# ErrorTzy/unpaper-gpu

Hardware: AMD Instinct MI355X
Metric: pages/sec + Mpixel/s, 1000-page GRAY8 A4@300dpi batch, 1/2/4/8 GPU (higher is better)
Workload: dtype u8; 1 GPU; 1000 synthetic GRAY8 A4@300dpi pages (2480x3508) per GPU, default pipeline, inputs and outputs resident in HBM; pages_per_gpu=1000, sheets_per_batch=64, streams=16, hw_queues=24, parallelism=one runner thread per device, pages sharded, no collective

## Files before the change

unpaper-gpu_amd/csrc/common.h:

```cpp
#pragma once

#include <hip/hip_runtime.h>
#include <stdint.h>
#include <stdlib.h>

#include <mutex>
#include <set>
#include <utility>

#include "unpaper_hip.h"

#define UPH_HD __host__ __device__ __forceinline__

namespace uph {

inline void allow_dynamic_lds(const void* kernel, size_t bytes) {
  if (bytes <= 64 * 1024) return;
  static std::mutex mu;
  static std::set<std::pair<int, const void*>> done;
  int dev = 0;
  (void)hipGetDevice(&dev);
  std::lock_guard<std::mutex> lk(mu);
  if (done.insert({dev, kernel}).second)
    (void)hipFuncSetAttribute(kernel, hipFuncAttributeMaxDynamicSharedMemorySize, 160 * 1024);
}


enum Fmt : int32_t {
  F_GRAY8 = UPHIP_FMT_GRAY8,
  F_Y400A = UPHIP_FMT_Y400A,
  F_RGB24 = UPHIP_FMT_RGB24,
  F_MONOWHITE = UPHIP_FMT_MONOWHITE,
  F_MONOBLACK = UPHIP_FMT_MONOBLACK,
};

UPH_HD int bytes_per_pixel(int fmt) {
  return fmt == F_GRAY8 ? 1 : fmt == F_Y400A ? 2 : fmt == F_RGB24 ? 3 : 0;
}
UPH_HD bool is_mono(int fmt) { return fmt == F_MONOWHITE || fmt == F_MONOBLACK; }
UPH_HD int64_t row_bytes(int32_t w, int fmt) {
  return is_mono(fmt) ? ((int64_t)w + 7) / 8 : (int64_t)w * bytes_per_pixel(fmt);
}
UPH_HD int64_t round_pitch(int64_t bytes) { return (bytes + 255) & ~(int64_t)255; }

struct Rect {
  int32_t x0, y0, x1, y1;
};

UPH_HD Rect to_rect(UphipRectangle r) {
  return Rect{r.vertex[0].x, r.vertex[0].y, r.vertex[1].x, r.vertex[1].y};
}
UPH_HD UphipRectangle from_rect(Rect r) {
  UphipRectangle o;
  o.vertex[0].x = r.x0;
  o.vertex[0].y = r.y0;
  o.vertex[1].x = r.x1;
  o.vertex[1].y = r.y1;
  return o;
}
UPH_HD int32_t imin(int32_t a, int32_t b) { return a < b ? a : b; }
UPH_HD int32_t imax(int32_t a, int32_t b) { return a > b ? a : b; }
UPH_HD int32_t iabs(int32_t a) { return a < 0 ? -a : a; }
UPH_HD Rect normalize(Rect r) {
  return Rect{imin(r.x0, r.x1), imin(r.y0, r.y1), imax(r.x0, r.x1), imax(r.y0, r.y1)};
}
UPH_HD Rect clip(Rect r, int32_t W, int32_t H) {
  Rect n = normalize(r);
  return Rect{imax(n.x0, 0), imax(n.y0, 0), imin(n.x1, W - 1), imin(n.y1, H - 1)};
}
UPH_HD uint64_t count_pixels(Rect r) {
  return (uint64_t)(uint32_t)((iabs(r.x0 - r.x1) + 1) * (iabs(r.y0 - r.y1) + 1));
}
UPH_HD bool point_in(int32_t x, int32_t y, Rect in) {
  Rect a = normalize(in);
  return x >= a.x0 && x <= a.x1 && y >= a.y0 && y <= a.y1;
}
UPH_HD Rect rect_from_size(int32_t x, int32_t y, int32_t w, int32_t h) {
  return Rect{x, y, x + w - 1, y + h - 1};
}
UPH_HD bool rects_overlap(Rect a_in, Rect b_in) {
  Rect a = normalize(a_in), b = normalize(b_in);
  return point_in(a.x0, a.y0, b) || point_in(a.x1, a.y1, b);
}

struct Px {
  uint8_t r, g, b;
};
UPH_HD uint8_t gray_of(Px p) { return (uint8_t)(((int)p.r + p.g + p.b) / 3); }
UPH_HD uint8_t light_of(Px p) {
  uint8_t m = p.r < p.g ? p.r : p.g;
  return m < p.b ? m : p.b;
}
UPH_HD uint8_t dark_of(Px p) {
  uint8_t m = p.r > p.g ? p.r : p.g;
  return m > p.b ? m : p.b;
}

template <int FMT>
__device__ __forceinline__ Px load_px_row(const uint8_t* row, int32_t x) {
  if (FMT == F_GRAY8) {
    uint8_t v = row[x];
    return Px{v, v, v};
  } else if (FMT == F_Y400A) {
    uint8_t v = row[2 * x];
    return Px{v, v, v};
  } else {
    const uint8_t* q = row + 3 * x;
    return Px{q[0], q[1], q[2]};
  }
}

template <int FMT>
__device__ __forceinline__ void store_px_row(uint8_t* row, int32_t x, Px p) {
  if (FMT == F_GRAY8) {
    row[x] = gray_of(p);
  } else if (FMT == F_Y400A) {
    row[2 * x] = gray_of(p);
    row[2 * x + 1] = 0xFF;
  } else {
    uint8_t* q = row + 3 * x;
    q[0] = p.r;
    q[1] = p.g;
    q[2] = p.b;
  }
}

__device__ __forceinline__ Px load_px_any(const uint8_t* base, int64_t pitch, int fmt,
                                          int32_t W, int32_t H, int32_t x, int32_t y) {
  if (x < 0 || y < 0 || x >= W || y >= H) return Px{255, 255, 255};
  const uint8_t* row = base + (int64_t)y * pitch;
  switch (fmt) {
    case F_GRAY8: return load_px_row<F_GRAY8>(row, x);
    case F_Y400A: return load_px_row<F_Y400A>(row, x);
    case F_RGB24: return load_px_row<F_RGB24>(row, x);
    case F_MONOWHITE: return (row[x >> 3] & (128 >> (x & 7))) ? Px{0, 0, 0} : Px{255, 255, 255};
    default: return (row[x >> 3] & (128 >> (x & 7))) ? Px{255, 255, 255} : Px{0, 0, 0};
  }
}

__device__ __forceinline__ void xcd_block(int* bx, int* by, int* bz) {
  const int gx = gridDim.x, gy = gridDim.y;
  const int nblk = gx * gy * gridDim.z;
  const int lin = blockIdx.x + gx * (blockIdx.y + gy * blockIdx.z);
  const int q = nblk >> 3, rr = nblk & 7, xcd = lin & 7;
  const int t = xcd * q + (xcd < rr ? xcd : rr) + (lin >> 3);
  *bz = t / (gx * gy);
  const int rem = t - *bz * gx * gy;
  *by = rem / gx;
  *bx = rem - *by * gx;
}

inline uint32_t div_magic(uint32_t d) { return d > 1 ? (uint32_t)(0xFFFFFFFFull / d + 1) : 0u; }
__device__ __forceinline__ int div_by_magic(int n, uint32_t m) {
  return m ? (int)__umulhi((uint32_t)n, m) : n;
}
__device__ __forceinline__ void xcd_block_m(uint32_t m_gxy, uint32_t m_gx, int* bx, int* by,
                                            int* bz) {
  const int gx = gridDim.x, gy = gridDim.y;
  const int nblk = gx * gy * gridDim.z;
  const int lin = blockIdx.x + gx * (blockIdx.y + gy * blockIdx.z);
  const int q = nblk >> 3, rr = nblk & 7, xcd = lin & 7;
  const int t = xcd * q + (xcd < rr ? xcd : rr) + (lin >> 3);
  *bz = div_by_magic(t, m_gxy);
  const int rem = t - *bz * gx * gy;
  *by = div_by_magic(rem, m_gx);
  *bx = rem - *by * gx;
}

struct Planes {
  uint8_t* base[2];
  int64_t pitch;
  int64_t stride;
  int32_t W, H;
  int32_t fmt;
  int32_t count;
};

struct SheetCtl {
  int32_t cur;
  int32_t status;
  int32_t point_count;
  int32_t mask_count;
  UphipPoint points[UPHIP_MAX_POINTS];
  UphipRectangle masks[UPHIP_MAX_POINTS];
  UphipRectangle border_masks[UPHIP_MAX_PAGES];
  float rotation[UPHIP_MAX_PAGES];
  int32_t rot_index[UPHIP_MAX_PAGES][4];
  int32_t op_active;
  int32_t op_i[8];
  float op_f[4];
  UphipRectangle op_rect[4];
};

enum : int32_t {
  STATUS_FLOOD_OVERFLOW = 1 << 0,
  STATUS_NOISE_OVERFLOW = 1 << 1,
  STATUS_EDGE_GUARD = 1 << 2,
  STATUS_SORT_OVERFLOW = 1 << 3,
};

__device__ __forceinline__ uint8_t* sheet_plane(const Planes& P, int s, int k) {
  return P.base[k] + (int64_t)s * P.stride;
}

#ifdef UPHIP_DIAG
inline int diag_env(const char* name) {
  const char* v = getenv(name);
  return v ? atoi(v) : 0;
}
inline int diag_skip() {
  static const int v = diag_env("UPHIP_DIAG_SKIP");
  return v;
}
inline int diag_double() {
  static const int v = diag_env("UPHIP_DIAG_DOUBLE");
  return v;
}
inline int diag_noise() {
  static const int v = diag_env("UPHIP_DIAG_NOISE");
  return v;
}
#define UPH_DIAG_BITS(d, m) ((d) & (m))
#define UPH_LAUNCH_DIAG(bit, ...)                              \
  do {                                                         \
    hipLaunchKernelGGL(__VA_ARGS__);                           \
    if (::uph::diag_double() & (bit)) hipLaunchKernelGGL(__VA_ARGS__); \
  } while (0)
#else
constexpr int diag_skip() { return 0; }
constexpr int diag_double() { return 0; }
constexpr int diag_noise() { return 0; }
#define UPH_DIAG_BITS(d, m) 0
#define UPH_LAUNCH_DIAG(bit, ...) hipLaunchKernelGGL(__VA_ARGS__)
#endif

}
```

unpaper-gpu_amd/csrc/kernels.h:

```cpp
#pragma once

#include "common.h"

namespace uph {

struct PlaneRef {
  Planes P;
  const SheetCtl* ctl;
  int32_t which;
};

__device__ __forceinline__ uint8_t* plane_ptr(const PlaneRef& R, int s) {
  int k = R.which;
  if (R.ctl) k = R.which ? 1 - R.ctl[s].cur : R.ctl[s].cur;
  return R.P.base[k] + (int64_t)s * R.P.stride;
}

inline PlaneRef cur_ref(const Planes& P, const SheetCtl* ctl) { return PlaneRef{P, ctl, 0}; }
inline PlaneRef other_ref(const Planes& P, const SheetCtl* ctl) { return PlaneRef{P, ctl, 1}; }
inline PlaneRef fixed_ref(const Planes& P, int k) { return PlaneRef{P, nullptr, k}; }

struct FillArgs {
  Rect r;
  uint8_t color[3];
  int32_t active;
};

struct CopyArgs {
  Rect a;
  int32_t tx, ty;
  int32_t active;
};

struct MaskArgs {
  int32_t n;
  uint8_t color[3];
  Rect m[UPHIP_MAX_MASKS];
};

struct MoveArgs {
  Rect area;
  int32_t tx, ty;
  uint8_t bg[3];
  int32_t active;
};

struct RotateArgs {
  Rect mask;
  float sinval, cosval;
  int32_t active;
};

void launch_fill_thr(const PlaneRef& dst, const FillArgs* args, int count, int rows_hint,
                     uint8_t thr, hipStream_t st);
void launch_copy_thr(const PlaneRef& src, const PlaneRef& dst, const CopyArgs* args, int count,
                     int rows_hint, uint8_t thr, hipStream_t st);
void launch_apply_masks_thr(const PlaneRef& dst, const MaskArgs* args, int count, uint8_t thr,
                            hipStream_t st);
void launch_mirror_oop(const PlaneRef& src, const PlaneRef& dst, bool h, bool v, uint8_t thr,
                       int count, hipStream_t st);
void launch_rotate90_thr(const PlaneRef& src, const PlaneRef& dst, int direction, uint8_t thr,
                         int count, hipStream_t st);
void launch_stretch_thr(const PlaneRef& src, const PlaneRef& dst, int interp, uint8_t thr,
                        int count, hipStream_t st);
void launch_shift(const PlaneRef& src, const PlaneRef& dst, int dx, int dy, const uint8_t bg[3],
                  uint8_t thr, int count, hipStream_t st);
void launch_flip_if_active(SheetCtl* ctl, const int32_t* active, int64_t stride_bytes,
                           int count, hipStream_t st);

void launch_move_rect(const PlaneRef& src, const PlaneRef& dst, const MoveArgs* args,
                      int count, hipStream_t st);
struct MoveExtra {
  const MaskArgs* masks;
  uint32_t* rows;
  int64_t rows_stride;
  int32_t rx0, rx1;
  uint8_t thr;
  bool dry;
  int32_t ya0, ya1, yb0, yb1;
  const int32_t* only;
};
bool launch_move_chain(const PlaneRef& src, const PlaneRef& dst, const MoveArgs* center,
                       const MaskArgs* masks, const MoveArgs* align, int count, hipStream_t st);
bool launch_move_rect_fused(const PlaneRef& src, const PlaneRef& dst, const MoveArgs* args,
                            const MoveExtra& x, int count, hipStream_t st);

bool launch_rotate_mask(const PlaneRef& src, const PlaneRef& dst, const RotateArgs* args,
                        int interp, int count, hipStream_t st, float max_abs_angle,
                        uint32_t* colsum = nullptr, int64_t cs_stride = 0);
struct LinWindow {
  int32_t cols, rows, stride;
};
bool launch_rotate_linear(const PlaneRef& src, const PlaneRef& dst, const RotateArgs* args,
                          int nmask, int64_t mstride, const int32_t* indep, int count,
                          hipStream_t st, float max_abs_angle);

}
```

unpaper-gpu_amd/csrc/kernels_rotate.hip:

```cpp
#include <type_traits>

#include "blit_common.h"
#include "interp.h"
#include "kernels.h"

namespace uph {

constexpr int kRotTW = 64, kRotTH = 16;
constexpr int kRotCap = 4096;

template <int FMT>
struct LdsSrc {
  const uint8_t* lds;
  int32_t x0, y0, w, h;
  int32_t W, H;
  Src<FMT> g;
  __device__ __forceinline__ Px at(int32_t x, int32_t y) const {
    const int32_t u = x - x0, v = y - y0;
    if (u < 0 || v < 0 || u >= w || v >= h) return g.at(x, y);
    if (FMT == F_RGB24) {
      const uint8_t* q = lds + 3 * (v * w + u);
      return Px{q[0], q[1], q[2]};
    }
    const uint8_t q = lds[v * w + u];
    return Px{q, q, q};
  }
};

template <int FMT>
__global__ void __launch_bounds__(kThreads) k_rotate_mask(PlaneRef src, PlaneRef dst,
                                                          const RotateArgs* args, int interp) {
  constexpr int CH = FMT == F_RGB24 ? 3 : 1;
  __shared__ uint8_t stage[kRotCap * CH];
  const int s = blockIdx.z;
  const RotateArgs a = args[s];
  if (!a.active) return;
  const Planes& P = src.P;
  const uint8_t* sbase = plane_ptr(src, s);
  uint8_t* dbase = plane_ptr(dst, s);
  const Rect nm = normalize(a.mask);
  const int32_t sw = nm.x1 - nm.x0 + 1, sh = nm.y1 - nm.y0 + 1;
  const float scx = nm.x0 + sw / 2.0f, scy = nm.y0 + sh / 2.0f;
  const float tcx = 0 + sw / 2.0f, tcy = 0 + sh / 2.0f;
  const Src<FMT> S{sbase, P.pitch, P.W, P.H};
  const int32_t tx0 = blockIdx.x * kRotTW, ty0 = blockIdx.y * kRotTH;
  const int32_t u0 = imax(tx0, 0) - a.mask.x0, u1 = imin(tx0 + kRotTW, P.W) - 1 - a.mask.x0;
  const int32_t v0 = imax(ty0, 0) - a.mask.y0, v1 = imin(ty0 + kRotTH, P.H) - 1 - a.mask.y0;
  const int32_t cu0 = imax(u0, 0), cu1 = imin(u1, sw - 1);
  const int32_t cv0 = imax(v0, 0), cv1 = imin(v1, sh - 1);
  const bool any_in = cu0 <= cu1 && cv0 <= cv1;
  int32_t bx0 = 0, by0 = 0, bw = 0, bh = 0;
  bool staged = false;
  if (any_in) {
    float mnx = 3.0e38f, mxx = -3.0e38f, mny = 3.0e38f, mxy = -3.0e38f;
#pragma unroll
    for (int c = 0; c < 4; c++) {
      const int32_t u = c & 1 ? cu1 : cu0, v = c & 2 ? cv1 : cv0;
      const float X = scx + (u - tcx) * a.cosval + (v - tcy) * a.sinval;
      const float Y = scy + (v - tcy) * a.cosval - (u - tcx) * a.sinval;
      mnx = fminf(mnx, X);
      mxx = fmaxf(mxx, X);
      mny = fminf(mny, Y);
      mxy = fmaxf(mxy, Y);
    }
    bx0 = (int32_t)floorf(mnx) - 3;
    by0 = (int32_t)floorf(mny) - 3;
    bw = (int32_t)floorf(mxx) + 4 - bx0 + 1;
    bh = (int32_t)floorf(mxy) + 4 - by0 + 1;
    staged = bw > 0 && bh > 0 && (int64_t)bw * bh <= kRotCap;
  }
  if (staged) {
    const int n = bw * bh;
    for (int base = 0; base < n; base += 8 * kThreads) {
      uint8_t v[8][CH];
#pragma unroll
      for (int k = 0; k < 8; k++) {
        const int i = base + k * kThreads + threadIdx.x;
        const int32_t x = bx0 + i % bw, y = by0 + i / bw;
#pragma unroll
        for (int c = 0; c < CH; c++) v[k][c] = 255;
        if (i < n && x >= 0 && y >= 0 && x < P.W && y < P.H) {
          const Px p = load_px_row<FMT>(sbase + (int64_t)y * P.pitch, x);
          v[k][0] = p.r;
          if (CH == 3) {
            v[k][1] = p.g;
            v[k][2] = p.b;
          }
        }
      }
#pragma unroll
      for (int k = 0; k < 8; k++) {
        const int i = base + k * kThreads + threadIdx.x;
        if (i < n) {
#pragma unroll
          for (int c = 0; c < CH; c++) stage[i * CH + c] = v[k][c];
        }
      }
    }
  }
  __syncthreads();
  const LdsSrc<FMT> L{stage, bx0, by0, bw, bh, P.W, P.H, S};
  const int lane = threadIdx.x & 63, w = threadIdx.x >> 6;
  const int32_t x = tx0 + lane;
  if (x >= P.W) return;
  const int32_t u = x - a.mask.x0;
#pragma unroll
  for (int k = 0; k < kRotTH / 4; k++) {
    const int32_t y = ty0 + w + 4 * k;
    if (y >= P.H) break;
    uint8_t* drow = dbase + (int64_t)y * P.pitch;
    const int32_t v = y - a.mask.y0;
    if (u >= 0 && u < sw && v >= 0 && v < sh) {
      const float srcX = scx + (u - tcx) * a.cosval + (v - tcy) * a.sinval;
      const float srcY = scy + (v - tcy) * a.cosval - (u - tcx) * a.sinval;
      if (FMT != F_RGB24 && staged && interp == UPHIP_INTERP_CUBIC) {
        const int ix = (int)srcX, iy = (int)srcY;
        const uint8_t* t = stage + (iy - 1 - by0) * bw + (ix - 1 - bx0);
        const float fx = srcX - ix;
        uint8_t col[4];
#pragma unroll
        for (int r = 0; r < 4; r++, t += bw) col[r] = cubic_scale(fx, t[0], t[1], t[2], t[3]);
        const uint8_t o = cubic_scale(srcY - iy, col[0], col[1], col[2], col[3]);
        store_px_row<FMT>(drow, x, Px{o, o, o});
        continue;
      }
      const Px o = staged ? interpolate<FMT>(L, srcX, srcY, interp)
                          : interpolate<FMT>(S, srcX, srcY, interp);
      store_px_row<FMT>(drow, x, o);
    } else {
      copy_px_raw<FMT>(drow, x, sbase + (int64_t)y * P.pitch, x);
    }
  }
}

__device__ __forceinline__ uint8_t cubic_int(float f, float h, int a, int b, int c, int d) {
  const float s2 = (float)(3 * (b - c) + d - a);
  const float s1 = (float)(2 * a - 5 * b + 4 * c - d);
  const float u = s1 + f * s2;
  const float v = (float)(c - a) + f * u;
  const int r = (int)((float)b + h * v);
  return (uint8_t)(r < 0 ? 0 : (r > 255 ? 255 : r));
}

constexpr int kRotGH = 32;
constexpr int kRotGCap = 6144;

template <int FMT>
__global__ void __launch_bounds__(kThreads) k_rotate_cubic_gray(PlaneRef src, PlaneRef dst,
                                                                const RotateArgs* args) {
  __shared__ uint32_t stage32[kRotGCap / 4];
  uint8_t* stage = reinterpret_cast<uint8_t*>(stage32);
  int txi, tyi, s;
  xcd_block(&txi, &tyi, &s);
  const RotateArgs a = args[s];
  if (!a.active) return;
  const Planes& P = src.P;
  const uint8_t* sbase = plane_ptr(src, s);
  uint8_t* dbase = plane_ptr(dst, s);
  const Rect nm = normalize(a.mask);
  const int32_t sw = nm.x1 - nm.x0 + 1, sh = nm.y1 - nm.y0 + 1;
  const float scx = nm.x0 + sw / 2.0f, scy = nm.y0 + sh / 2.0f;
  const float tcx = 0 + sw / 2.0f, tcy = 0 + sh / 2.0f;
  const int32_t tx0 = txi * kRotTW, ty0 = tyi * kRotGH;
  const int32_t u0 = imax(tx0, 0) - a.mask.x0, u1 = imin(tx0 + kRotTW, P.W) - 1 - a.mask.x0;
  const int32_t v0 = imax(ty0, 0) - a.mask.y0, v1 = imin(ty0 + kRotGH, P.H) - 1 - a.mask.y0;
  const int32_t cu0 = imax(u0, 0), cu1 = imin(u1, sw - 1);
  const int32_t cv0 = imax(v0, 0), cv1 = imin(v1, sh - 1);
  int32_t bx0 = 0, by0 = 0, bw = 0, bh = 0;
  bool staged = false;
  if (cu0 <= cu1 && cv0 <= cv1) {
    float mnx = 3.0e38f, mxx = -3.0e38f, mny = 3.0e38f, mxy = -3.0e38f;
#pragma unroll
    for (int c = 0; c < 4; c++) {
      const int32_t u = c & 1 ? cu1 : cu0, v = c & 2 ? cv1 : cv0;
      const float X = scx + (u - tcx) * a.cosval + (v - tcy) * a.sinval;
      const float Y = scy + (v - tcy) * a.cosval - (u - tcx) * a.sinval;
      mnx = fminf(mnx, X);
      mxx = fmaxf(mxx, X);
      mny = fminf(mny, Y);
      mxy = fmaxf(mxy, Y);
    }
    bx0 = (int32_t)floorf(mnx) - 3;
    by0 = (int32_t)floorf(mny) - 3;
    bw = (int32_t)floorf(mxx) + 4 - bx0 + 1;
    bh = (int32_t)floorf(mxy) + 4 - by0 + 1;
    staged = bw > 0 && bh > 0;
  }
  const int32_t xa = bx0 >= 0 ? (bx0 & ~3) : -((-bx0 + 3) & ~3);
  const int lead = FMT == F_GRAY8 ? bx0 - xa : 0;
  const int nd = (lead + bw + 3) >> 2;
  const int sstride = FMT == F_GRAY8 ? 4 * nd : bw;
  staged = staged && (int64_t)sstride * bh <= kRotGCap;
  if (staged && FMT == F_GRAY8) {
    const int n = nd * bh;
    for (int b0 = 0; b0 < n; b0 += 8 * kThreads) {
      uint32_t v[8];
#pragma unroll
      for (int k = 0; k < 8; k++) {
        const int i = b0 + k * kThreads + threadIdx.x;
        const int r = i / nd;
        const int32_t xd = xa + 4 * (i - r * nd), y = by0 + r;
        const bool row_ok = (y >= 0) & (y < P.H);
        const uint8_t* row = sbase + (int64_t)imin(imax(y, 0), P.H - 1) * P.pitch;
        v[k] = *reinterpret_cast<const uint32_t*>(row + imin(imax(xd, 0), (int32_t)P.pitch - 4));
        if (!row_ok) v[k] = 0xFFFFFFFFu;
      }
#pragma unroll
      for (int k = 0; k < 8; k++) {
        const int i = b0 + k * kThreads + threadIdx.x;
        if (i >= n) continue;
        const int r = i / nd;
        const int32_t xd = xa + 4 * (i - r * nd), y = by0 + r;
        uint32_t w4 = v[k];
        if ((y >= 0) & (y < P.H) & ((xd < 0) | (xd + 3 >= P.W))) {
          const uint8_t* row = sbase + (int64_t)y * P.pitch;
          w4 = 0;
#pragma unroll
          for (int j = 0; j < 4; j++) {
            const int32_t x = xd + j;
            const uint32_t b = (x >= 0 && x < P.W) ? row[x] : 255u;
            w4 |= b << (8 * j);
          }
        }
        stage32[i] = w4;
      }
    }
  } else if (staged) {
    const int n = bw * bh;
    for (int b0 = 0; b0 < n; b0 += 8 * kThreads) {
      uint8_t v[8];
#pragma unroll
      for (int k = 0; k < 8; k++) {
        const int i = b0 + k * kThreads + threadIdx.x;
        const int r = i / bw;
        const int32_t x = bx0 + (i - r * bw), y = by0 + r;
        const bool ok = (x >= 0) & (y >= 0) & (x < P.W) & (y < P.H);
        const uint8_t q = load_px_row<FMT>(sbase + (int64_t)imin(imax(y, 0), P.H - 1) * P.pitch,
                                           imin(imax(x, 0), P.W - 1)).r;
        v[k] = ok ? q : (uint8_t)255;
      }
#pragma unroll
      for (int k = 0; k < 8; k++) {
        const int i = b0 + k * kThreads + threadIdx.x;
        if (i < n) stage[i] = v[k];
      }
    }
  }
  __syncthreads();
  const Src<FMT> S{sbase, P.pitch, P.W, P.H};
  const int lane = threadIdx.x & 63, w = threadIdx.x >> 6;
  const int32_t x = tx0 + lane;
  if (x >= P.W) return;
  const int32_t u = x - a.mask.x0;
#pragma unroll
  for (int k = 0; k < kRotGH / 4; k++) {
    const int32_t y = ty0 + w + 4 * k;
    if (y >= P.H) break;
    uint8_t* drow = dbase + (int64_t)y * P.pitch;
    const int32_t v = y - a.mask.y0;
    if (u >= 0 && u < sw && v >= 0 && v < sh) {
      const float srcX = scx + (u - tcx) * a.cosval + (v - tcy) * a.sinval;
      const float srcY = scy + (v - tcy) * a.cosval - (u - tcx) * a.sinval;
      uint8_t o;
      if (staged) {
        const int ix = (int)srcX, iy = (int)srcY;
        const float fx = srcX - ix, fy = srcY - iy;
        const float hx = 0.5f * fx, hy = 0.5f * fy;
        const uint8_t* t = stage + (iy - 1 - by0) * sstride + lead + (ix - 1 - bx0);
        int col[4];
#pragma unroll
        for (int r = 0; r < 4; r++, t += sstride)
          col[r] = cubic_int(fx, hx, t[0], t[1], t[2], t[3]);
        o = cubic_int(fy, hy, col[0], col[1], col[2], col[3]);
      } else {
        o = interp_bicubic(S, srcX, srcY).r;
      }
      store_px_row<FMT>(drow, x, Px{o, o, o});
    } else {
      copy_px_raw<FMT>(drow, x, sbase + (int64_t)y * P.pitch, x);
    }
  }
}

typedef float f2 __attribute__((ext_vector_type(2)));
constexpr int kRQW = 256;
constexpr int kRQH = 32;
constexpr int kRQStride = 72;
constexpr int kRQRows = 84;
constexpr int kRQWords = kRQStride * kRQRows + 2;

__device__ __forceinline__ f2 fma2(f2 a, f2 b, f2 c) { return __builtin_elementwise_fma(a, b, c); }
__device__ __forceinline__ f2 splat2(float v) { return f2{v, v}; }

__device__ __forceinline__ void cubic_terms(f2 a, f2 b, f2 c, f2 d, f2& ca, f2& s1, f2& s2) {
  const f2 e = d - a, g = b - c;
  ca = c - a;
  s2 = fma2(splat2(3.0f), g, e);
  s1 = fma2(splat2(-5.0f), g, -(e + ca));
}

__device__ __forceinline__ f2 cubic2(f2 f, f2 h, f2 a, f2 b, f2 c, f2 d) {
  f2 ca, s1, s2;
  cubic_terms(a, b, c, d, ca, s1, s2);
  const f2 u = s1 + f * s2;
  const f2 v = ca + f * u;
  const f2 r = b + h * v;
  return f2{__builtin_amdgcn_fmed3f(__builtin_truncf(r.x), 0.0f, 255.0f),
            __builtin_amdgcn_fmed3f(__builtin_truncf(r.y), 0.0f, 255.0f)};
}

template <int K>
__device__ __forceinline__ float ubyte_f(uint32_t w) {
  float r;
  if constexpr (K == 0) asm("v_cvt_f32_ubyte0 %0, %1" : "=v"(r) : "v"(w));
  else if constexpr (K == 1) asm("v_cvt_f32_ubyte1 %0, %1" : "=v"(r) : "v"(w));
  else if constexpr (K == 2) asm("v_cvt_f32_ubyte2 %0, %1" : "=v"(r) : "v"(w));
  else asm("v_cvt_f32_ubyte3 %0, %1" : "=v"(r) : "v"(w));
  return r;
}
template <int K>
__device__ __forceinline__ f2 tap2(uint32_t p, uint32_t q) {
  return f2{ubyte_f<K>(p), ubyte_f<K>(q)};
}

__global__ void __launch_bounds__(kThreads) k_rotate_cubic_g8(PlaneRef src, PlaneRef dst,
                                                              const RotateArgs* args) {
  __shared__ uint32_t win[kRQWords];
  int txi, tyi, s;
  xcd_block(&txi, &tyi, &s);
  const RotateArgs a = args[s];
  if (!a.active) return;
  const Planes& P = src.P;
  const uint8_t* sbase = plane_ptr(src, s);
  uint8_t* dbase = plane_ptr(dst, s);
  const Rect nm = normalize(a.mask);
  const int32_t sw = nm.x1 - nm.x0 + 1, sh = nm.y1 - nm.y0 + 1;
  const float scx = nm.x0 + sw / 2.0f, scy = nm.y0 + sh / 2.0f;
  const float tcx = 0 + sw / 2.0f, tcy = 0 + sh / 2.0f;
  const int32_t tx0 = txi * kRQW, ty0 = tyi * kRQH;
  const int32_t u0 = imax(tx0, 0) - a.mask.x0, u1 = imin(tx0 + kRQW, P.W) - 1 - a.mask.x0;
  const int32_t v0 = imax(ty0, 0) - a.mask.y0, v1 = imin(ty0 + kRQH, P.H) - 1 - a.mask.y0;
  const int32_t cu0 = imax(u0, 0), cu1 = imin(u1, sw - 1);
  const int32_t cv0 = imax(v0, 0), cv1 = imin(v1, sh - 1);
  int32_t bx0 = 0, by0 = 0, bw = 0, bh = 0;
  if (cu0 <= cu1 && cv0 <= cv1) {
    float mnx = 3.0e38f, mxx = -3.0e38f, mny = 3.0e38f, mxy = -3.0e38f;
#pragma unroll
    for (int c = 0; c < 4; c++) {
      const int32_t u = c & 1 ? cu1 : cu0, v = c & 2 ? cv1 : cv0;
      const float X = scx + (u - tcx) * a.cosval + (v - tcy) * a.sinval;
      const float Y = scy + (v - tcy) * a.cosval - (u - tcx) * a.sinval;
      mnx = fminf(mnx, X);
      mxx = fmaxf(mxx, X);
      mny = fminf(mny, Y);
      mxy = fmaxf(mxy, Y);
    }
    bx0 = (int32_t)floorf(mnx) - 3;
    by0 = (int32_t)floorf(mny) - 3;
    bw = (int32_t)floorf(mxx) + 4 - bx0 + 1;
    bh = (int32_t)floorf(mxy) + 4 - by0 + 1;
  }
  const int32_t xa = bx0 >= 0 ? (bx0 & ~3) : -((-bx0 + 3) & ~3);
  const int lead = bx0 - xa;
  const int nd = (lead + bw + 3) >> 2;
  const bool staged = bw > 0 && bh > 0 && nd < kRQStride && bh <= kRQRows;
  if (staged) {
    const uint32_t m = nd > 1 ? (uint32_t)((0xFFFFFFFFull / (uint32_t)nd) + 1) : 0u;
    const int n = nd * bh;
    for (int b0 = 0; b0 < n; b0 += 8 * kThreads) {
      uint32_t v[8];
#pragma unroll
      for (int k = 0; k < 8; k++) {
        const int i = b0 + k * kThreads + threadIdx.x;
        const int r = nd > 1 ? (int)__umulhi((uint32_t)i, m) : i;
        const int32_t xd = xa + 4 * (i - r * nd), y = by0 + r;
        const uint8_t* row = sbase + (int64_t)imin(imax(y, 0), P.H - 1) * P.pitch;
        v[k] = *reinterpret_cast<const uint32_t*>(row + imin(imax(xd, 0), (int32_t)P.pitch - 4));
        if ((y < 0) | (y >= P.H)) v[k] = 0xFFFFFFFFu;
      }
#pragma unroll
      for (int k = 0; k < 8; k++) {
        const int i = b0 + k * kThreads + threadIdx.x;
        if (i >= n) continue;
        const int r = nd > 1 ? (int)__umulhi((uint32_t)i, m) : i;
        const int j = i - r * nd;
        const int32_t xd = xa + 4 * j, y = by0 + r;
        uint32_t w4 = v[k];
        if ((y >= 0) & (y < P.H) & ((xd < 0) | (xd + 3 >= P.W))) {
          const uint8_t* row = sbase + (int64_t)y * P.pitch;
          w4 = 0;
#pragma unroll
          for (int q = 0; q < 4; q++) {
            const int32_t x = xd + q;
            const uint32_t b = (x >= 0 && x < P.W) ? row[x] : 255u;
            w4 |= b << (8 * q);
          }
        }
        win[r * kRQStride + j] = w4;
      }
    }
  }
  __syncthreads();
  const int lane = threadIdx.x & 63, w = threadIdx.x >> 6;
  const int32_t xl = tx0 + 4 * lane;
  if (xl >= P.W) return;
  float ax[4], bs[4];
  bool colin[4];
#pragma unroll
  for (int j = 0; j < 4; j++) {
    const int32_t u = xl + j - a.mask.x0;
    const float cu = u - tcx;
    ax[j] = scx + cu * a.cosval;
    bs[j] = cu * a.sinval;
    colin[j] = (u >= 0) & (u < sw) & (xl + j < P.W);
  }
  const f2 AX0{ax[0], ax[1]}, AX1{ax[2], ax[3]}, BS0{bs[0], bs[1]}, BS1{bs[2], bs[3]};
  const int base_off = (-1 - by0) * (4 * kRQStride) + lead - 1 - bx0;
  const Src<F_GRAY8> S{sbase, P.pitch, P.W, P.H};
#pragma unroll 2
  for (int k = 0; k < kRQH / 4; k++) {
    const int32_t y = ty0 + w + 4 * k;
    if (y >= P.H) break;
    const int32_t v = y - a.mask.y0;
    const bool rowin = (v >= 0) & (v < sh);
    const float cv = v - tcy;
    const f2 VS = splat2(cv * a.sinval), VC = splat2(scy + cv * a.cosval);
    const f2 SX[2] = {AX0 + VS, AX1 + VS};
    const f2 SY[2] = {VC - BS0, VC - BS1};
    const uint8_t* srow = sbase + (int64_t)y * P.pitch;
    uint32_t out = 0;
    if (staged) {
#pragma unroll
      for (int pr = 0; pr < 2; pr++) {
        const int ix0 = (int)SX[pr].x, ix1 = (int)SX[pr].y;
        const int iy0 = (int)SY[pr].x, iy1 = (int)SY[pr].y;
        const f2 fx = SX[pr] - f2{(float)ix0, (float)ix1};
        const f2 fy = SY[pr] - f2{(float)iy0, (float)iy1};
        const f2 hx = 0.5f * fx, hy = 0.5f * fy;
        const bool in0 = rowin & colin[2 * pr], in1 = rowin & colin[2 * pr + 1];
        const int o0 = in0 ? base_off + iy0 * (4 * kRQStride) + ix0 : 0;
        const int o1 = in1 ? base_off + iy1 * (4 * kRQStride) + ix1 : 0;
        const uint32_t* w0 = win + (o0 >> 2);
        const uint32_t* w1 = win + (o1 >> 2);
        f2 col[4];
#pragma unroll
        for (int r = 0; r < 4; r++) {
          const uint32_t p = __builtin_amdgcn_alignbyte(w0[r * kRQStride + 1], w0[r * kRQStride], o0);
          const uint32_t q = __builtin_amdgcn_alignbyte(w1[r * kRQStride + 1], w1[r * kRQStride], o1);
          col[r] = cubic2(fx, hx, tap2<0>(p, q), tap2<1>(p, q), tap2<2>(p, q), tap2<3>(p, q));
        }
        const f2 o = cubic2(fy, hy, col[0], col[1], col[2], col[3]);
        out = __builtin_amdgcn_cvt_pk_u8_f32(o.x, 2 * pr, out);
        out = __builtin_amdgcn_cvt_pk_u8_f32(o.y, 2 * pr + 1, out);
      }
    } else {
#pragma unroll
      for (int j = 0; j < 4; j++) {
        const f2 sx = SX[j >> 1], sy = SY[j >> 1];
        const float fx = (j & 1) ? sx.y : sx.x, fy = (j & 1) ? sy.y : sy.x;
        if (rowin & colin[j]) out |= (uint32_t)interp_bicubic(S, fx, fy).r << (8 * j);
      }
    }
    uint32_t inmask = 0;
#pragma unroll
    for (int j = 0; j < 4; j++) inmask |= (rowin & colin[j]) ? 0xFFu << (8 * j) : 0u;
    uint8_t* drow = dbase + (int64_t)y * P.pitch;
    if (xl + 3 < P.W) {
      if (inmask != 0xFFFFFFFFu)
        out = (out & inmask) | (*reinterpret_cast<const uint32_t*>(srow + xl) & ~inmask);
      *reinterpret_cast<uint32_t*>(drow + xl) = out;
    } else {
      for (int j = 0; xl + j < P.W; j++)
        drow[xl + j] = (inmask >> (8 * j)) & 1 ? (uint8_t)(out >> (8 * j)) : srow[xl + j];
    }
  }
}

constexpr int kRFW = 128;
constexpr int kRFH = 48;
constexpr int kRFS = 144;
constexpr int kRFT = 512;
constexpr int kRFWaves = kRFT / 64;

#define UPH_TAP_PAIR(o, b, k) \
  "ds_read2_b32 %" #o ", %" #b " offset0:" #k " offset1:" UPH_STR(UPH_ROWOFF_##k) "\n\t"
#define UPH_STR2(x) #x
#define UPH_STR(x) UPH_STR2(x)
#define UPH_ROWOFF_0 144
#define UPH_ROWOFF_1 145
#define UPH_ROWOFF_2 146
#define UPH_ROWOFF_3 147
static_assert(kRFS == 144, "tap pair offsets are spelled out for a 144-float row stride");
__device__ __forceinline__ void lds_taps16(const uint32_t (&a)[4], f2 (&t)[4][4]) {
  asm volatile(UPH_TAP_PAIR(0, 16, 0) UPH_TAP_PAIR(1, 16, 1) UPH_TAP_PAIR(2, 16, 2)
               UPH_TAP_PAIR(3, 16, 3) UPH_TAP_PAIR(4, 17, 0) UPH_TAP_PAIR(5, 17, 1)
               UPH_TAP_PAIR(6, 17, 2) UPH_TAP_PAIR(7, 17, 3) UPH_TAP_PAIR(8, 18, 0)
               UPH_TAP_PAIR(9, 18, 1) UPH_TAP_PAIR(10, 18, 2) UPH_TAP_PAIR(11, 18, 3)
               UPH_TAP_PAIR(12, 19, 0) UPH_TAP_PAIR(13, 19, 1) UPH_TAP_PAIR(14, 19, 2)
               UPH_TAP_PAIR(15, 19, 3)
               : "=&v"(t[0][0]), "=&v"(t[0][1]), "=&v"(t[0][2]), "=&v"(t[0][3]),
                 "=&v"(t[1][0]), "=&v"(t[1][1]), "=&v"(t[1][2]), "=&v"(t[1][3]),
                 "=&v"(t[2][0]), "=&v"(t[2][1]), "=&v"(t[2][2]), "=&v"(t[2][3]),
                 "=&v"(t[3][0]), "=&v"(t[3][1]), "=&v"(t[3][2]), "=&v"(t[3][3])
               : "v"(a[0]), "v"(a[1]), "v"(a[2]), "v"(a[3])
               : "memory");
}
template <int N>
__device__ __forceinline__ void lds_wait_pair(f2 (&t)[4]) {
  asm volatile("s_waitcnt lgkmcnt(%4)"
               : "+v"(t[0]), "+v"(t[1]), "+v"(t[2]), "+v"(t[3])
               : "n"(N)
               : "memory");
}
template <int N>
__device__ __forceinline__ void lds_wait_pair_after(f2 (&t)[4], f2& prev) {
  asm volatile("s_waitcnt lgkmcnt(%5)"
               : "+v"(t[0]), "+v"(t[1]), "+v"(t[2]), "+v"(t[3]), "+v"(prev)
               : "n"(N)
               : "memory");
}

__device__ __forceinline__ f2 cubic2_row_u(f2 f, f2 h, const f2 (&t)[4]) {
  f2 ca, s1, s2;
  cubic_terms(t[0], t[1], t[2], t[3], ca, s1, s2);
  f2 u = f * s2;
  u = s1 + u;
  u = f * u;
  u = ca + u;
  u = h * u;
  return t[1] + u;
}
__device__ __forceinline__ float clamp_t255(float u) {
  return __builtin_amdgcn_fmed3f(__builtin_truncf(u), 0.0f, 255.0f);
}

template <int CTRL>
__device__ __forceinline__ float dpp_f(float v) {
  return __int_as_float(__builtin_amdgcn_mov_dpp(__float_as_int(v), CTRL, 0xF, 0xF, false));
}

__device__ __forceinline__ uint32_t row_off(int32_t y, int64_t pitch) {
  return (uint32_t)y * (uint32_t)pitch;
}

#ifndef UPH_ROT_MINB
#define UPH_ROT_MINB 8
#endif
#ifdef UPHIP_DIAG
__device__ unsigned long long g_rot_phase[1024 * 8];
#define UPH_ROT_T(k)                                                         \
  if (UPH_DIAG_BITS(diag, 65536) && threadIdx.x == 0) {                     \
    const unsigned long long tn = wall_clock64();                            \
    atomicAdd(&g_rot_phase[8 * (blockIdx.x & 1023) + (k)], tn - tprev);      \
    tprev = tn;                                                              \
  }
#else
#define UPH_ROT_T(k)
#endif
template <bool LOOP>
__global__ void __launch_bounds__(kRFT, UPH_ROT_MINB) k_rotate_cubic_g8f(PlaneRef src, PlaneRef dst,
                                                               const RotateArgs* args,
                                                               int max_rows, int cls_rows,
                                                               int diag,
                                                               uint32_t m_gxy, uint32_t m_gx,
                                                               int loop_count, int tgx, int tgy,
                                                               uint32_t* colsum, int64_t cs_stride) {
  extern __shared__ __attribute__((aligned(16))) float winf[];
  __shared__ int32_t win_s[4];
  __shared__ uint32_t csum_s[kRFW];
  auto tile = [&](int txi, int tyi, int s) {
#ifdef UPHIP_DIAG
  unsigned long long tprev = wall_clock64();
#endif
  const uint8_t* sbase = plane_ptr(src, s);
  uint8_t* dbase = plane_ptr(dst, s);
  const RotateArgs a = args[s];
  if (!a.active) return;
  if (cls_rows != 0) {
    const int need = kRFH + (int)ceilf((kRFW - 1) * fabsf(a.sinval)) + 5;
    if (cls_rows > 0 ? need > cls_rows : need <= -cls_rows) return;
  }
  const Planes& P = src.P;
  const Rect nm = normalize(a.mask);
  const int32_t sw = nm.x1 - nm.x0 + 1, sh = nm.y1 - nm.y0 + 1;
  const float scx = nm.x0 + sw / 2.0f, scy = nm.y0 + sh / 2.0f;
  const float tcx = 0 + sw / 2.0f, tcy = 0 + sh / 2.0f;
  const int32_t tx0 = txi * kRFW, ty0 = tyi * kRFH;
  const int32_t u0 = imax(tx0, 0) - a.mask.x0, u1 = imin(tx0 + kRFW, P.W) - 1 - a.mask.x0;
  const int32_t v0 = imax(ty0, 0) - a.mask.y0, v1 = imin(ty0 + kRFH, P.H) - 1 - a.mask.y0;
  const int32_t cu0 = imax(u0, 0), cu1 = imin(u1, sw - 1);
  const int32_t cv0 = imax(v0, 0), cv1 = imin(v1, sh - 1);
  auto csum_flush = [&]() {
    __syncthreads();
    if (threadIdx.x < kRFW && tx0 + (int)threadIdx.x < P.W)
      atomicAdd(colsum + s * cs_stride + tx0 + threadIdx.x, csum_s[threadIdx.x]);
  };
  const bool outside_tile = !(cu0 <= cu1 && cv0 <= cv1);
  if (colsum) {
    if (threadIdx.x < kRFW) csum_s[threadIdx.x] = 0;
    if (outside_tile) __syncthreads();
  }
  if (!(cu0 <= cu1 && cv0 <= cv1)) {
    const int cb = 8 * (threadIdx.x & 15);
    const int32_t x = tx0 + cb;
    uint32_t cs8[8] = {0, 0, 0, 0, 0, 0, 0, 0};
    for (int r = threadIdx.x >> 4; r < kRFH; r += kRFT / 16) {
      const int32_t y = ty0 + r;
      if (y >= P.H || x >= P.W) continue;
      const uint8_t* sp = sbase + row_off(y, P.pitch) + x;
      uint8_t* dp = dbase + row_off(y, P.pitch) + x;
      if (x + 8 <= P.W) {
        const uint64_t q = *reinterpret_cast<const uint64_t*>(sp);
        *reinterpret_cast<uint64_t*>(dp) = q;
#pragma unroll
        for (int j = 0; j < 8; j++) cs8[j] += (uint32_t)(q >> (8 * j)) & 0xFFu;
      } else {
        for (int j = 0; x + j < P.W; j++) {
          dp[j] = sp[j];
          cs8[j & 7] += sp[j];
        }
      }
    }
    if (colsum) {
#pragma unroll
      for (int j = 0; j < 8; j++) atomicAdd(&csum_s[cb + j], cs8[j]);
      csum_flush();
    }
    return;
  }
  UPH_ROT_T(0)
  const int lane = threadIdx.x & 63;
  const int wu = __builtin_amdgcn_readfirstlane(threadIdx.x >> 6);
  if (wu == 0) {
    const int c = lane & 3;
    const int32_t u = c & 1 ? cu1 : cu0, v = c & 2 ? cv1 : cv0;
    const float X = scx + (u - tcx) * a.cosval + (v - tcy) * a.sinval;
    const float Y = scy + (v - tcy) * a.cosval - (u - tcx) * a.sinval;
    float mnx = fminf(X, dpp_f<0xB1>(X)), mxx = fmaxf(X, dpp_f<0xB1>(X));
    float mny = fminf(Y, dpp_f<0xB1>(Y)), mxy = fmaxf(Y, dpp_f<0xB1>(Y));
    mnx = fminf(mnx, dpp_f<0x4E>(mnx));
    mxx = fmaxf(mxx, dpp_f<0x4E>(mxx));
    mny = fminf(mny, dpp_f<0x4E>(mny));
    mxy = fmaxf(mxy, dpp_f<0x4E>(mxy));
    if (lane < 4) {
      const float q = lane == 0 ? mnx : lane == 1 ? mny : lane == 2 ? mxx : mxy;
      win_s[lane] = (int32_t)floorf(q);
    }
  }
  __syncthreads();
  UPH_ROT_T(1)
  const int32_t bx0 = __builtin_amdgcn_readfirstlane(win_s[0]) - 1;
  const int32_t by0 = __builtin_amdgcn_readfirstlane(win_s[1]) - 1;
  const int32_t bw = __builtin_amdgcn_readfirstlane(win_s[2]) + 3 - bx0 + 1;
  const int32_t bh = __builtin_amdgcn_readfirstlane(win_s[3]) + 3 - by0 + 1;
  const int32_t xa = bx0 >= 0 ? (bx0 & ~3) : -((-bx0 + 3) & ~3);
  const int nd = (bx0 - xa + bw + 3) >> 2;
  const bool staged = bw > 0 && bh > 0 && 4 * nd <= kRFS && bh <= max_rows;
  uint64_t* nw = reinterpret_cast<uint64_t*>(winf + kRFS * max_rows);
  uint8_t* obuf = reinterpret_cast<uint8_t*>(nw + max_rows) + wu * (kRFH / kRFWaves * kRFW);
  if (staged && !UPH_DIAG_BITS(diag, 1024)) {
    const int rq = (lane * 57) >> 10;
    const int jq = lane - 18 * rq;
    const int nq = (nd + 1) >> 1;
    const bool qv = rq < 3 && jq < nq;
    const int32_t xd = xa + 8 * jq;
    auto stage = [&](int rb, uint32_t w0, uint32_t w1) {
      const int r = rb + rq;
      const bool valid = qv && r < bh;
      const unsigned long long m = __ballot(valid && (w0 & w1) != 0xFFFFFFFFu);
      if (lane < 3 && rb + lane < bh) nw[rb + lane] = (m >> (18 * lane)) & 0x3FFFFull;
      if (valid) {
        float4* d = reinterpret_cast<float4*>(winf + r * kRFS + 8 * jq);
        d[0] = make_float4(ubyte_f<0>(w0), ubyte_f<1>(w0), ubyte_f<2>(w0), ubyte_f<3>(w0));
        d[1] = make_float4(ubyte_f<0>(w1), ubyte_f<1>(w1), ubyte_f<2>(w1), ubyte_f<3>(w1));
      }
    };
    const bool interior = xa >= 0 && xa + 8 * nq <= P.W && by0 >= 0 && by0 + bh <= P.H;
    if (interior) {
      const uint32_t off0 = row_off(by0 + rq, P.pitch) + (uint32_t)(qv ? xd : xa);
      for (int rg = 3 * wu; rg < bh; rg += 3 * 3 * kRFWaves) {
        uint2 v[3];
#pragma unroll
        for (int g = 0; g < 3; g++) {
          const int rb = rg + 3 * kRFWaves * g;
          const uint32_t o = rb + rq < bh ? off0 + (uint32_t)rb * (uint32_t)P.pitch : off0;
          v[g] = *reinterpret_cast<const uint2*>(sbase + o);
        }
#pragma unroll
        for (int g = 0; g < 3; g++) {
          const int rb = rg + 3 * kRFWaves * g;
          if (rb >= bh) break;
          stage(rb, v[g].x, v[g].y);
        }
      }
    } else {
      const int32_t xc0 = imin(imax(xd, 0), (int32_t)P.pitch - 4);
      const int32_t xc1 = imin(imax(xd + 4, 0), (int32_t)P.pitch - 4);
      const int fs0 = imin(imax(24 + 8 * (xd - xc0), 0), 56);
      const int fs1 = imin(imax(24 + 8 * (xd + 4 - xc1), 0), 56);
      uint32_t out0 = qv ? 0u : 0xFFFFFFFFu, out1 = out0;
#pragma unroll
      for (int k = 0; k < 4; k++) {
        if (xd + k < 0 || xd + k >= P.W) out0 |= 0xFFu << (8 * k);
        if (xd + 4 + k < 0 || xd + 4 + k >= P.W) out1 |= 0xFFu << (8 * k);
      }
      for (int rg = 3 * wu; rg < bh; rg += 3 * 3 * kRFWaves) {
        uint2 v[3];
#pragma unroll
        for (int g = 0; g < 3; g++) {
          const int r = rg + 3 * kRFWaves * g + rq;
          const int32_t y = imin(imax(by0 + r, 0), P.H - 1);
          const uint8_t* row = sbase + row_off(y, P.pitch);
          v[g].x = *reinterpret_cast<const uint32_t*>(row + xc0);
          v[g].y = *reinterpret_cast<const uint32_t*>(row + xc1);
        }
#pragma unroll
        for (int g = 0; g < 3; g++) {
          const int rb = rg + 3 * kRFWaves * g;
          if (rb >= bh) break;
          const int32_t y = by0 + rb + rq;
          uint32_t w0 = (uint32_t)(((uint64_t)v[g].x << 24) >> fs0) | out0;
          uint32_t w1 = (uint32_t)(((uint64_t)v[g].y << 24) >> fs1) | out1;
          if ((y < 0) | (y >= P.H)) w0 = w1 = 0xFFFFFFFFu;
          stage(rb, w0, w1);
        }
      }
    }
  }
  __syncthreads();
  UPH_ROT_T(2)
  const int32_t xA = tx0 + lane, xB = xA + 64;
  const bool hasA = xA < P.W, hasB = xB < P.W;
  const int32_t uA = xA - a.mask.x0, uB = xB - a.mask.x0;
  const float cuA = uA - tcx, cuB = uB - tcx;
  const float axA = scx + cuA * a.cosval, bsA = cuA * a.sinval;
  const float axB = scx + cuB * a.cosval, bsB = cuB * a.sinval;
  const bool colA = hasA & (uA >= 0) & (uA < sw), colB = hasB & (uB >= 0) & (uB < sw);
  typedef __attribute__((address_space(3))) float lds_f32;
  const uint32_t lds0 = (uint32_t)(uintptr_t)(lds_f32*)winf;
  const Src<F_GRAY8> S{sbase, P.pitch, P.W, P.H};
  const float cuL = (tx0 - a.mask.x0) - tcx, cuR = (tx0 + kRFW - 1 - a.mask.x0) - tcx;
  const float bsL = cuL * a.sinval, bsR = cuR * a.sinval;
  constexpr int kRows = kRFH / kRFWaves;
  const int32_t yw = ty0 + wu * kRows;
  const int cb = 8 * (lane & 15);
  const int32_t xo = tx0 + cb;
  const bool partial = !(cu0 == u0 && cu1 == u1 && cv0 == v0 && cv1 == v1);
  if (partial) {
    constexpr int kQ = (kRows + 3) / 4;
    uint64_t q[kQ];
#pragma unroll
    for (int h = 0; h < kQ; h++) {
      q[h] = 0;
      const int rr = 4 * h + (lane >> 4);
      const int32_t y = imin(yw + rr, P.H - 1);
      const int32_t x = imin(xo, (int32_t)P.pitch - 8);
      if (rr < kRows) q[h] = *reinterpret_cast<const uint64_t*>(sbase + row_off(y, P.pitch) + x);
    }
#pragma unroll
    for (int h = 0; h < kQ; h++) {
      const int rr = 4 * h + (lane >> 4);
      if (rr < kRows) *reinterpret_cast<uint64_t*>(obuf + rr * kRFW + cb) = q[h];
    }
  }
  uint32_t white_rows = 0;
  if (staged) {
#pragma unroll
    for (int g = 0; g < kRows; g += 8) {
      const int k = g + (lane >> 3), j = lane & 7;
      bool hit = false;
      if (k < kRows) {
        const float cv = (yw + k - a.mask.y0) - tcy;
        const float VC = scy + cv * a.cosval;
        const int32_t yl = (int)(VC - bsL), yr = (int)(VC - bsR);
        const int32_t r0 = imax(imin(yl, yr) - 1 - by0, 0);
        const int32_t r1 = imin(imax(yl, yr) + 2 - by0, bh - 1);
        for (int r = r0 + j; r <= r1; r += 8) hit |= nw[r] != 0;
      }
      const uint64_t m = __ballot(hit);
#pragma unroll
      for (int q = 0; q < 8 && g + q < kRows; q++)
        if (((m >> (8 * q)) & 0xFFull) == 0) white_rows |= 1u << (g + q);
    }
    if (UPH_DIAG_BITS(diag, 2048)) white_rows = 0;
    if (UPH_DIAG_BITS(diag, 512)) white_rows = ~0u;
  }
  const bool posc = bx0 >= 0 && by0 >= 0;
  const uint32_t wbase = lds0 - 4u * (uint32_t)((1 + by0) * kRFS + 1 + xa);
  UPH_ROT_T(3)
  uint32_t fsA = 0, fsB = 0;
  auto row_loop = [&](auto full_tag) {
  constexpr bool FULL = decltype(full_tag)::value;
#pragma unroll
  for (int k = 0; k < kRows; k++) {
    const int32_t y = yw + k;
    const int32_t v = y - a.mask.y0;
    const bool rowin = FULL || ((v >= 0) & (v < sh) & (y < P.H));
    const float cv = v - tcy;
    const float VS = cv * a.sinval, VC = scy + cv * a.cosval;
    const bool inA = FULL || (rowin & colA), inB = FULL || (rowin & colB);
    uint32_t oA = 255, oB = 255;
    const bool white = (FULL || staged) && ((white_rows >> k) & 1u);
    if (!white && (FULL || staged)) {
      const float sxA = axA + VS, syA = VC - bsA, sxB = axB + VS, syB = VC - bsB;
      const int ixA = (int)sxA, iyA = (int)syA, ixB = (int)sxB, iyB = (int)syB;
      float fxA, fyA, fxB, fyB;
      if (FULL || posc) {
        fxA = __builtin_amdgcn_fractf(sxA);
        fyA = __builtin_amdgcn_fractf(syA);
        fxB = __builtin_amdgcn_fractf(sxB);
        fyB = __builtin_amdgcn_fractf(syB);
      } else {
        fxA = sxA - ixA, fyA = syA - iyA, fxB = sxB - ixB, fyB = syB - iyB;
      }
      const uint32_t pA = inA ? wbase + 4u * (uint32_t)(__mul24(iyA, kRFS) + ixA) : lds0;
      const uint32_t pB = inB ? wbase + 4u * (uint32_t)(__mul24(iyB, kRFS) + ixB) : lds0;
      const uint32_t ta[4] = {pA, pA + 8 * kRFS, pB, pB + 8 * kRFS};
      f2 t[4][4];
      lds_taps16(ta, t);
      const f2 FA = splat2(fxA), HA = splat2(0.5f * fxA);
      const f2 FB = splat2(fxB), HB = splat2(0.5f * fxB);
      f2 c[4];
      lds_wait_pair<12>(t[0]);
      c[0] = cubic2_row_u(FA, HA, t[0]);
      lds_wait_pair_after<8>(t[1], c[0]);
      c[1] = cubic2_row_u(FA, HA, t[1]);
      lds_wait_pair_after<4>(t[2], c[1]);
      c[2] = cubic2_row_u(FB, HB, t[2]);
      lds_wait_pair_after<0>(t[3], c[2]);
      c[3] = cubic2_row_u(FB, HB, t[3]);
      const f2 o = cubic2(f2{fyA, fyB}, f2{0.5f * fyA, 0.5f * fyB},
                          f2{clamp_t255(c[0].x), clamp_t255(c[2].x)},
                          f2{clamp_t255(c[0].y), clamp_t255(c[2].y)},
                          f2{clamp_t255(c[1].x), clamp_t255(c[3].x)},
                          f2{clamp_t255(c[1].y), clamp_t255(c[3].y)});
      oA = (uint32_t)o.x;
      oB = (uint32_t)o.y;
    }
#ifdef UPHIP_DIAG
    if (UPH_DIAG_BITS(diag, 131072)) {
      int32_t z = k;
      asm volatile(
          "s_add_u32 %0, %0, 1\n\ts_add_u32 %0, %0, 1\n\ts_add_u32 %0, %0, 1\n\ts_add_u32 %0, %0, 1\n\t"
          "s_add_u32 %0, %0, 1\n\ts_add_u32 %0, %0, 1\n\ts_add_u32 %0, %0, 1\n\ts_add_u32 %0, %0, 1\n\t"
          "s_add_u32 %0, %0, 1\n\ts_add_u32 %0, %0, 1\n\ts_add_u32 %0, %0, 1\n\ts_add_u32 %0, %0, 1\n\t"
          "s_add_u32 %0, %0, 1\n\ts_add_u32 %0, %0, 1\n\ts_add_u32 %0, %0, 1\n\ts_add_u32 %0, %0, 1\n\t"
          "s_add_u32 %0, %0, 1\n\ts_add_u32 %0, %0, 1\n\ts_add_u32 %0, %0, 1\n\ts_add_u32 %0, %0, 1\n\t"
          "s_add_u32 %0, %0, 1\n\ts_add_u32 %0, %0, 1\n\ts_add_u32 %0, %0, 1\n\ts_add_u32 %0, %0, 1\n\t"
          "s_add_u32 %0, %0, 1\n\ts_add_u32 %0, %0, 1\n\ts_add_u32 %0, %0, 1\n\ts_add_u32 %0, %0, 1\n\t"
          "s_add_u32 %0, %0, 1\n\ts_add_u32 %0, %0, 1\n\ts_add_u32 %0, %0, 1\n\ts_add_u32 %0, %0, 1"
          : "+s"(z));
      if (z == -1) oA = 0;
    }
#endif
    if (!FULL && !staged) break;
    if (FULL) {
      obuf[k * kRFW + lane] = (uint8_t)oA;
      obuf[k * kRFW + 64 + lane] = (uint8_t)oB;
      fsA += oA;
      fsB += oB;
    } else {
      if (inA) obuf[k * kRFW + lane] = (uint8_t)oA;
      if (inB) obuf[k * kRFW + 64 + lane] = (uint8_t)oB;
    }
  }
  };
  const bool full =
      !partial && staged && posc && tx0 + kRFW <= P.W && ty0 + kRFH <= P.H;
  if (full)
    row_loop(std::true_type{});
  else
    row_loop(std::false_type{});
  if (!staged) {
#pragma unroll 1
    for (int k = 0; k < kRows; k++) {
      const int32_t y = yw + k;
      const int32_t v = y - a.mask.y0;
      const bool rowin = (v >= 0) & (v < sh) & (y < P.H);
      const float cv = v - tcy;
      const float VS = cv * a.sinval, VC = scy + cv * a.cosval;
      if (rowin & colA) obuf[k * kRFW + lane] = interp_bicubic(S, axA + VS, VC - bsA).r;
      if (rowin & colB) obuf[k * kRFW + 64 + lane] = interp_bicubic(S, axB + VS, VC - bsB).r;
    }
  }
  UPH_ROT_T(4)
  __builtin_amdgcn_wave_barrier();
  if (full && !UPH_DIAG_BITS(diag, 8192)) {
#pragma unroll
    for (int k0 = 0; k0 < kRows; k0 += 4) {
      const int rr = k0 + (lane >> 4);
      if (rr < kRows) {
        const uint64_t q = *reinterpret_cast<const uint64_t*>(obuf + rr * kRFW + cb);
        *reinterpret_cast<uint64_t*>(dbase + row_off(yw + rr, P.pitch) + xo) = q;
      }
    }
  } else
  for (int k0 = 0; k0 < kRows && !UPH_DIAG_BITS(diag, 8192); k0 += 4) {
    const int rr = k0 + (lane >> 4);
    const int32_t y = yw + rr, x = xo;
    if (rr < kRows && y < P.H && x < P.W) {
      const uint64_t q = *reinterpret_cast<const uint64_t*>(obuf + rr * kRFW + cb);
      uint8_t* d = dbase + row_off(y, P.pitch) + x;
      if (x + 8 <= P.W) {
        *reinterpret_cast<uint64_t*>(d) = q;
      } else {
        for (int j = 0; x + j < P.W; j++) d[j] = (uint8_t)(q >> (8 * j));
      }
    }
  }
  UPH_ROT_T(5)
  if (colsum) {
    uint32_t sA = fsA, sB = fsB;
    if (!full) {
#pragma unroll
      for (int k = 0; k < kRows; k++) {
        if (yw + k >= P.H) break;
        sA += obuf[k * kRFW + lane];
        sB += obuf[k * kRFW + 64 + lane];
      }
    }
    atomicAdd(&csum_s[lane], sA);
    atomicAdd(&csum_s[64 + lane], sB);
    csum_flush();
  }
  UPH_ROT_T(6)
#ifdef UPHIP_DIAG
  if (UPH_DIAG_BITS(diag, 65536) && threadIdx.x == 0)
    atomicAdd(&g_rot_phase[8 * (blockIdx.x & 1023) + 7], 1ull);
#endif
  };
  if constexpr (!LOOP) {
    int txi, tyi, s;
    xcd_block_m(m_gxy, m_gx, &txi, &tyi, &s);
    tile(txi, tyi, s);
  } else {
  for (int s0 = 0; s0 < loop_count; s0 += 64) {
    const int l = threadIdx.x & 63;
    bool want = false;
    if (s0 + l < loop_count) {
      const RotateArgs q = args[s0 + l];
      want = q.active && kRFH + (int)ceilf((kRFW - 1) * fabsf(q.sinval)) + 5 > -cls_rows;
    }
    uint64_t m = __ballot(want);
    m = ((uint64_t)__builtin_amdgcn_readfirstlane((uint32_t)(m >> 32)) << 32) |
        __builtin_amdgcn_readfirstlane((uint32_t)m);
    while (m) {
      const int s = s0 + __ffsll((long long)m) - 1;
      m &= m - 1;
      for (int t = blockIdx.x; t < tgx * tgy; t += gridDim.x) {
        tile(t % tgx, t / tgx, s);
        __syncthreads();
      }
    }
  }
  }
}

static int rotate_window_rows(float max_abs_angle) {
  const float a = fminf(fabsf(max_abs_angle), 1.5707964f);
  return kRFH + (int)ceilf((kRFW - 1) * sinf(a)) + 5;
}

bool launch_rotate_mask(const PlaneRef& src, const PlaneRef& dst, const RotateArgs* args,
                        int interp, int count, hipStream_t st, float max_abs_angle,
                        uint32_t* colsum, int64_t cs_stride) {
  const dim3 grid((src.P.W + kRotTW - 1) / kRotTW, (src.P.H + kRotTH - 1) / kRotTH, count);
  const dim3 ggrid((src.P.W + kRotTW - 1) / kRotTW, (src.P.H + kRotGH - 1) / kRotGH, count);
  if (interp == UPHIP_INTERP_CUBIC && src.P.fmt == F_GRAY8) {
    if (diag_double() & 4096) colsum = nullptr;
    const int rows = rotate_window_rows(max_abs_angle);
    auto lds_of = [](int r) {
      return (sizeof(float) * kRFS + sizeof(uint64_t)) * (size_t)r + kRFH * kRFW;
    };
    const int rows4 = (int)((40 * 1024 - 16 - 4 * kRFW - kRFH * kRFW) /
                            (sizeof(float) * kRFS + sizeof(uint64_t)));
    if (lds_of(rows) <= 56 * 1024 &&
        src.P.pitch * (int64_t)src.P.H < (1ll << 31) && !(diag_double() & 256)) {
      const dim3 fgrid((src.P.W + kRFW - 1) / kRFW, (src.P.H + kRFH - 1) / kRFH, count);
      const uint32_t mgxy = div_magic(fgrid.x * fgrid.y), mgx = div_magic(fgrid.x);
      const int dd = diag_double() & (512 | 1024 | 2048 | 8192 | 65536 | 131072);
#ifdef UPHIP_DIAG
      struct PhasePrint {
        hipStream_t st;
        ~PhasePrint() {
          if (!(diag_double() & 65536)) return;
          static unsigned long long hh[1024 * 8], z[1024 * 8];
          unsigned long long h[8] = {0, 0, 0, 0, 0, 0, 0, 0};
          hipStreamSynchronize(st);
          hipMemcpyFromSymbol(hh, HIP_SYMBOL(g_rot_phase), sizeof(hh));
          hipMemcpyToSymbol(HIP_SYMBOL(g_rot_phase), z, sizeof(z));
          for (int i = 0; i < 1024 * 8; i++) h[i & 7] += hh[i];
          if (!h[7]) return;
          fprintf(stderr, "rotate phases (10 ns ticks/tile, %llu tiles): args %.0f corners %.0f staging %.0f "
                  "flags %.0f compute %.0f stores %.0f colsum %.0f\n", h[7], (double)h[0] / h[7],
                  (double)h[1] / h[7], (double)h[2] / h[7], (double)h[3] / h[7],
                  (double)h[4] / h[7], (double)h[5] / h[7], (double)h[6] / h[7]);
        }
      } phase_print{st};
#endif
      if (rows > rows4) {
        UPH_LAUNCH_DIAG(2, k_rotate_cubic_g8f<false>, fgrid, dim3(kRFT), lds_of(rows4), st, src, dst, args,
                        rows4, rows4, dd, mgxy, mgx, 0, 0, 0, colsum, cs_stride);
        UPH_LAUNCH_DIAG(2, k_rotate_cubic_g8f<true>, dim3(3 * 256), dim3(kRFT), lds_of(rows), st, src, dst,
                        args, rows, -rows4, dd, 0u, 0u, count, (int)fgrid.x, (int)fgrid.y, colsum,
                        cs_stride);
      } else {
        UPH_LAUNCH_DIAG(2, k_rotate_cubic_g8f<false>, fgrid, dim3(kRFT), lds_of(rows), st, src, dst, args,
                        rows, 0, dd, mgxy, mgx, 0, 0, 0, colsum, cs_stride);
      }
      return colsum != nullptr;
    }
    const dim3 qgrid((src.P.W + kRQW - 1) / kRQW, (src.P.H + kRQH - 1) / kRQH, count);
    UPH_LAUNCH_DIAG(2, k_rotate_cubic_g8, qgrid, dim3(kThreads), 0, st, src, dst, args);
    return false;
  }
  if (interp == UPHIP_INTERP_CUBIC && src.P.fmt == F_Y400A) {
    hipLaunchKernelGGL(k_rotate_cubic_gray<F_Y400A>, ggrid, dim3(kThreads), 0, st, src, dst, args);
    return false;
  }
  if (src.P.fmt == F_GRAY8)
    hipLaunchKernelGGL(k_rotate_mask<F_GRAY8>, grid, dim3(kThreads), 0, st, src, dst, args,
                       interp);
  else if (src.P.fmt == F_Y400A)
    hipLaunchKernelGGL(k_rotate_mask<F_Y400A>, grid, dim3(kThreads), 0, st, src, dst, args,
                       interp);
  else
    hipLaunchKernelGGL(k_rotate_mask<F_RGB24>, grid, dim3(kThreads), 0, st, src, dst, args,
                       interp);
  return false;
}

}
```

unpaper-gpu_amd/csrc/ops.hip:

```cpp
#include <cmath>
#include <cstdio>
#include <vector>

#include "filters.h"
#include "mono_proxy.h"
#include "runtime.h"
#include "scan.h"

namespace uph {

static bool ok_image(const UphipImage& im, const char* op) {
  if (!im.frame) return fail("%s: image has no frame", op);
  if (!runtime_ready()) return fail("%s: no HIP device", op);
  hipSetDevice(im.frame->device);
  return true;
}

static PlaneRef ref_of(const UphipFrame* f) { return fixed_ref(frame_planes(f), 0); }

static void fill_frame(UphipFrame* f, Rect clipped, Px c, uint8_t thr, hipStream_t st) {
  if (clipped.x1 < clipped.x0 || clipped.y1 < clipped.y0) return;
  FillArgs a{clipped, {c.r, c.g, c.b}, 1};
  FillArgs* d = stage_args(&a, 1, st);
  if (!d) return;
  launch_fill_thr(ref_of(f), d, 1, clipped.y1 - clipped.y0 + 1, thr, st);
  arg_fence(st);
}

static void copy_frames(const UphipFrame* src, UphipFrame* dst, Rect clipped, int32_t tx,
                        int32_t ty, uint8_t thr, hipStream_t st) {
  if (clipped.x1 < clipped.x0 || clipped.y1 < clipped.y0) return;
  CopyArgs a{clipped, tx, ty, 1};
  CopyArgs* d = stage_args(&a, 1, st);
  if (!d) return;
  launch_copy_thr(ref_of(src), ref_of(dst), d, 1, clipped.y1 - clipped.y0 + 1, thr, st);
  arg_fence(st);
}

static void adopt_storage(UphipFrame* f, UphipFrame* n) {
  hipStreamSynchronize(current_stream());
  hipFree(f->data);
  *f = *n;
  delete n;
}

}

using namespace uph;

extern "C" {

UphipImage uphip_create_image(UphipRectangleSize size, UphipPixelFormat format, bool fill,
                              UphipPixel background, uint8_t abs_black_threshold) {
  UphipImage im{nullptr, background, abs_black_threshold};
  im.frame = frame_alloc(size.width, size.height, format);
  if (im.frame && fill)
    fill_frame(im.frame, Rect{0, 0, size.width - 1, size.height - 1},
               Px{background.r, background.g, background.b}, abs_black_threshold,
               current_stream());
  return im;
}

void uphip_free_image(UphipImage* image) {
  if (!image) return;
  frame_free(image->frame);
  image->frame = nullptr;
}

void uphip_replace_image(UphipImage* image, UphipImage* new_image) {
  uphip_free_image(image);
  *image = *new_image;
  new_image->frame = nullptr;
}

UphipImage uphip_create_compatible_image(UphipImage source, UphipRectangleSize size, bool fill) {
  return uphip_create_image(size, (UphipPixelFormat)source.frame->format, fill, source.background,
                            source.abs_black_threshold);
}

UphipRectangleSize uphip_size_of_image(UphipImage image) {
  UphipRectangleSize s{0, 0};
  if (image.frame) s = UphipRectangleSize{image.frame->width, image.frame->height};
  return s;
}

UphipPixelFormat uphip_image_format(UphipImage image) {
  return image.frame ? (UphipPixelFormat)image.frame->format : UPHIP_FMT_NONE;
}

int uphip_image_upload(UphipImage image, const void* host, int64_t linesize) {
  if (!ok_image(image, "upload")) return -1;
  UphipFrame* f = image.frame;
  const int64_t rb = row_bytes(f->width, f->format);
  if (linesize < rb) return fail("upload: linesize %lld < row bytes %lld", (long long)linesize,
                                 (long long)rb), -1;
  hipStream_t st = current_stream();
  if (!UPH_HIP(hipMemcpy2DAsync(f->data, f->pitch, host, linesize, rb, f->height,
                                hipMemcpyHostToDevice, st)))
    return -1;
  return UPH_HIP(hipStreamSynchronize(st)) ? 0 : -1;
}

int uphip_image_download(UphipImage image, void* host, int64_t linesize) {
  if (!ok_image(image, "download")) return -1;
  UphipFrame* f = image.frame;
  const int64_t rb = row_bytes(f->width, f->format);
  if (linesize < rb) return fail("download: linesize too small"), -1;
  hipStream_t st = current_stream();
  if (!UPH_HIP(hipMemcpy2DAsync(host, linesize, f->data, f->pitch, rb, f->height,
                                hipMemcpyDeviceToHost, st)))
    return -1;
  return UPH_HIP(hipStreamSynchronize(st)) ? 0 : -1;
}

void* uphip_image_device_ptr(UphipImage image) { return image.frame ? image.frame->data : nullptr; }
int64_t uphip_image_device_pitch(UphipImage image) { return image.frame ? image.frame->pitch : 0; }

void uphip_wipe_rectangle(UphipImage image, UphipRectangle input_area, UphipPixel color) {
  if (!ok_image(image, "wipe_rectangle")) return;
  UphipFrame* f = image.frame;
  fill_frame(f, clip(to_rect(input_area), f->width, f->height), Px{color.r, color.g, color.b},
             image.abs_black_threshold, current_stream());
}

void uphip_copy_rectangle(UphipImage source, UphipImage target, UphipRectangle source_area,
                          UphipPoint target_coords) {
  if (!ok_image(source, "copy_rectangle") || !ok_image(target, "copy_rectangle")) return;
  if (source.frame->device != target.frame->device)
    return (void)fail("copy_rectangle: frames on different devices");
  Rect a = clip(to_rect(source_area), source.frame->width, source.frame->height);
  copy_frames(source.frame, target.frame, a, target_coords.x, target_coords.y,
              target.abs_black_threshold, current_stream());
}

void uphip_center_image(UphipImage source, UphipImage target, UphipPoint to,
                        UphipRectangleSize ts) {
  if (!ok_image(source, "center_image") || !ok_image(target, "center_image")) return;
  UphipPoint so{0, 0};
  UphipRectangleSize ss{source.frame->width, source.frame->height};
  if (ss.width < ts.width || ss.height < ts.height)
    uphip_wipe_rectangle(target, from_rect(rect_from_size(to.x, to.y, ts.width, ts.height)),
                         target.background);
  if (ss.width <= ts.width) {
    to.x += (ts.width - ss.width) / 2;
  } else {
    so.x += (ss.width - ts.width) / 2;
    ss.width = ts.width;
  }
  if (ss.height <= ts.height) {
    to.y += (ts.height - ss.height) / 2;
  } else {
    so.y += (ss.height - ts.height) / 2;
    ss.height = ts.height;
  }
  uphip_copy_rectangle(source, target, from_rect(rect_from_size(so.x, so.y, ss.width, ss.height)),
                       to);
}

static int compare_sizes(UphipRectangleSize a, UphipRectangleSize b) {
  if (a.height == b.height && a.width == b.width) return 0;
  return imin(a.height, a.width) < imin(b.height, b.width) ? -1 : 1;
}

void uphip_stretch_and_replace(UphipImage* pImage, UphipRectangleSize size,
                               UphipInterpolation interp) {
  if (!pImage || !ok_image(*pImage, "stretch_and_replace")) return;
  UphipFrame* f = pImage->frame;
  if (compare_sizes(UphipRectangleSize{f->width, f->height}, size) == 0) return;
  UphipFrame* n = frame_alloc(size.width, size.height, f->format);
  if (!n) return;
  launch_stretch_thr(ref_of(f), ref_of(n), interp, pImage->abs_black_threshold, 1,
                     current_stream());
  adopt_storage(f, n);
}

void uphip_resize_and_replace(UphipImage* pImage, UphipRectangleSize size,
                              UphipInterpolation interp) {
  if (!pImage || !ok_image(*pImage, "resize_and_replace")) return;
  UphipRectangleSize is{pImage->frame->width, pImage->frame->height};
  if (compare_sizes(is, size) == 0) return;
  const float hr = (float)size.width / (float)is.width;
  const float vr = (float)size.height / (float)is.height;
  UphipRectangleSize ss;
  if (hr < vr) {
    ss.width = size.width;
    ss.height = (int32_t)(is.height * hr);
  } else if (vr < hr) {
    ss.width = (int32_t)(is.width * vr);
    ss.height = size.height;
  } else {
    ss = size;
  }
  uphip_stretch_and_replace(pImage, ss, interp);
  if (size.width == ss.width && size.height == ss.height) return;
  UphipImage resized = uphip_create_compatible_image(*pImage, size, true);
  if (!resized.frame) return;
  uphip_center_image(*pImage, resized, UphipPoint{0, 0}, size);
  uphip_replace_image(pImage, &resized);
}

void uphip_flip_rotate_90(UphipImage* pImage, UphipRotationDirection direction) {
  if (!pImage || !ok_image(*pImage, "flip_rotate_90")) return;
  UphipFrame* f = pImage->frame;
  UphipFrame* n = frame_alloc(f->height, f->width, f->format);
  if (!n) return;
  launch_rotate90_thr(ref_of(f), ref_of(n), direction, pImage->abs_black_threshold, 1,
                      current_stream());
  adopt_storage(f, n);
}

void uphip_mirror(UphipImage image, UphipDirection direction) {
  if (!ok_image(image, "mirror")) return;
  UphipFrame* f = image.frame;
  UphipFrame* n = frame_alloc(f->width, f->height, f->format);
  if (!n) return;
  launch_mirror_oop(ref_of(f), ref_of(n), direction.horizontal, direction.vertical,
                    image.abs_black_threshold, 1, current_stream());
  adopt_storage(f, n);
}

void uphip_shift_image(UphipImage* pImage, UphipDelta d) {
  if (!pImage || !ok_image(*pImage, "shift_image")) return;
  UphipImage n = uphip_create_compatible_image(*pImage, uphip_size_of_image(*pImage), true);
  if (!n.frame) return;
  uphip_copy_rectangle(*pImage, n,
                       from_rect(Rect{0, 0, pImage->frame->width - 1, pImage->frame->height - 1}),
                       UphipPoint{d.horizontal, d.vertical});
  uphip_replace_image(pImage, &n);
}

void uphip_apply_masks(UphipImage image, const UphipRectangle masks[], size_t masks_count,
                       UphipPixel color) {
  if (masks_count <= 0) return;
  if (!ok_image(image, "apply_masks")) return;
  if (masks_count > UPHIP_MAX_MASKS) return (void)fail("apply_masks: too many masks");
  MaskArgs a;
  a.n = (int32_t)masks_count;
  a.color[0] = color.r;
  a.color[1] = color.g;
  a.color[2] = color.b;
  for (size_t i = 0; i < masks_count; i++) a.m[i] = to_rect(masks[i]);
  hipStream_t st = current_stream();
  MaskArgs* d = stage_args(&a, 1, st);
  if (!d) return;
  launch_apply_masks_thr(ref_of(image.frame), d, 1, image.abs_black_threshold, st);
  arg_fence(st);
}

void uphip_apply_wipes(UphipImage image, UphipWipes wipes, UphipPixel color) {
  if (!ok_image(image, "apply_wipes")) return;
  UphipFrame* f = image.frame;
  for (size_t i = 0; i < wipes.count && i < UPHIP_MAX_MASKS; i++) {
    Rect r = to_rect(wipes.areas[i]);
    if (r.x0 > r.x1 || r.y0 > r.y1) continue;
    fill_frame(f, clip(r, f->width, f->height), Px{color.r, color.g, color.b},
               image.abs_black_threshold, current_stream());
  }
}

static UphipRectangle border_to_mask(int32_t W, int32_t H, UphipBorder b) {
  return from_rect(Rect{b.left, b.top, W - b.right - 1, H - b.bottom - 1});
}

void uphip_apply_border(UphipImage image, const UphipBorder border, UphipPixel color) {
  if (border.left == 0 && border.top == 0 && border.right == 0 && border.bottom == 0) return;
  if (!ok_image(image, "apply_border")) return;
  UphipRectangle m = border_to_mask(image.frame->width, image.frame->height, border);
  uphip_apply_masks(image, &m, 1, color);
}

size_t uphip_detect_masks(UphipImage image0, UphipMaskDetectionParameters params,
                          const UphipPoint points[], size_t points_count,
                          UphipRectangle masks[]) {
  if (!params.scan_direction.horizontal && !params.scan_direction.vertical) return 0;
  if (points_count == 0) return 0;
  if (!ok_image(image0, "detect_masks")) return 0;
  MonoProxy mp(image0, false, "detect_masks");
  if (!mp.ok()) return 0;
  const UphipImage image = mp.image();
  UphipFrame* f = image.frame;
  const int32_t W = f->width, H = f->height;
  hipStream_t st = current_stream();
  const size_t n = points_count;
  std::vector<AxisArgs> col_args, row_args;
  std::vector<EdgeArgs> edges(4 * n);
  const int32_t stride = imax(W, H);
  uint32_t* sums = (uint32_t*)scratch(0, sizeof(uint32_t) * stride * 2 * n);
  int32_t* res = (int32_t*)scratch(1, sizeof(int32_t) * 4 * n);
  if (!sums || !res) return 0;
  UPH_HIP(hipMemsetAsync(sums, 0, sizeof(uint32_t) * stride * 2 * n, st));
  for (size_t i = 0; i < n; i++) {
    const UphipPoint o = points[i];
    EdgeArgs* e = &edges[4 * i];
    for (int k = 0; k < 4; k++) e[k].active = 0;
    if (params.scan_direction.horizontal) {
      int32_t depth = params.scan_depth.horizontal == -1 ? H : params.scan_depth.horizontal;
      const int32_t size = params.scan_size.width;
      const int32_t c0 = o.y - depth / 2, c1 = c0 + depth - 1;
      Rect reg = clip(Rect{0, c0, W - 1, c1}, W, H);
      AxisArgs aa{reg, 0, (reg.y1 >= reg.y0) ? 1 : 0};
      col_args.push_back(aa);
      for (int k = 0; k < 2; k++) {
        EdgeArgs& ea = e[k];
        ea.active = 1;
        ea.sums_offset = 0;
        ea.extent = W;
        ea.cross_extent = H;
        ea.c0 = c0;
        ea.c1 = c1;
        ea.b0 = o.x - size / 2;
        ea.step = (k == 0 ? -1 : 1) * params.scan_step.horizontal;
        ea.size = size;
        ea.threshold = params.scan_threshold.horizontal;
      }
    } else {
      col_args.push_back(AxisArgs{Rect{0, 0, -1, -1}, 0, 0});
    }
    if (params.scan_direction.vertical) {
      int32_t depth = params.scan_depth.vertical == -1 ? W : params.scan_depth.vertical;
      const int32_t size = params.scan_size.height;
      const int32_t c0 = o.x - depth / 2, c1 = c0 + depth - 1;
      Rect reg = clip(Rect{c0, 0, c1, H - 1}, W, H);
      row_args.push_back(AxisArgs{reg, 0, (reg.x1 >= reg.x0) ? 1 : 0});
      for (int k = 2; k < 4; k++) {
        EdgeArgs& ea = e[k];
        ea.active = 1;
        ea.sums_offset = 0;
        ea.extent = H;
        ea.cross_extent = W;
        ea.c0 = c0;
        ea.c1 = c1;
        ea.b0 = o.y - size / 2;
        ea.step = (k == 2 ? -1 : 1) * params.scan_step.vertical;
        ea.size = size;
        ea.threshold = params.scan_threshold.vertical;
      }
    } else {
      row_args.push_back(AxisArgs{Rect{0, 0, -1, -1}, 0, 0});
    }
  }
  for (size_t i = 0; i < n; i++) {
    AxisArgs* ca = stage_args(&col_args[i], 1, st);
    AxisArgs* ra = stage_args(&row_args[i], 1, st);
    if (!ca || !ra) return 0;
    if (col_args[i].active)
      launch_axis_reduce(ref_of(f), ca, 0, M_GRAY_SUM, W, H, sums + (2 * i) * stride, 0, 1, st);
    if (row_args[i].active)
      launch_axis_reduce(ref_of(f), ra, 1, M_GRAY_SUM, W, H, sums + (2 * i + 1) * stride, 0, 1,
                         st);
    arg_fence(st);
  }
  for (size_t i = 0; i < n; i++) {
    EdgeArgs* e = &edges[4 * i];
    e[0].sums_offset = e[1].sums_offset = (int32_t)((2 * i) * stride);
    e[2].sums_offset = e[3].sums_offset = (int32_t)((2 * i + 1) * stride);
  }
  EdgeArgs* de = stage_args(edges.data(), edges.size(), st);
  if (!de) return 0;
  launch_edge_scan(de, (int)edges.size(), sums, 0, res, 1, st, imax(W, H));
  arg_fence(st);
  std::vector<int32_t> counts(4 * n);
  UPH_HIP(hipMemcpyAsync(counts.data(), res, sizeof(int32_t) * 4 * n, hipMemcpyDeviceToHost, st));
  if (!UPH_HIP(hipStreamSynchronize(st))) return 0;
  size_t valid = 0;
  for (size_t i = 0; i < n; i++) {
    const UphipPoint o = points[i];
    Rect m;
    if (params.scan_direction.horizontal) {
      m.x0 = o.x - (params.scan_step.horizontal * counts[4 * i]) - params.scan_size.width / 2;
      m.x1 = o.x + (params.scan_step.horizontal * counts[4 * i + 1]) + params.scan_size.width / 2;
    } else {
      m.x0 = 0;
      m.x1 = W - 1;
    }
    if (params.scan_direction.vertical) {
      m.y0 = o.y - (params.scan_step.vertical * counts[4 * i + 2]) - params.scan_size.height / 2;
      m.y1 = o.y + (params.scan_step.vertical * counts[4 * i + 3]) + params.scan_size.height / 2;
    } else {
      m.y0 = 0;
      m.y1 = H - 1;
    }
    const int32_t mw = iabs(m.x0 - m.x1) + 1, mh = iabs(m.y0 - m.y1) + 1;
    if ((params.minimum_width != -1 && mw < params.minimum_width) ||
        (params.maximum_width != -1 && mw > params.maximum_width)) {
      m.x0 = o.x - params.maximum_width / 2;
      m.x1 = o.x + params.maximum_width / 2;
    }
    if ((params.minimum_height != -1 && mh < params.minimum_height) ||
        (params.maximum_height != -1 && mh > params.maximum_height)) {
      m.y0 = o.y - params.maximum_height / 2;
      m.y1 = o.y + params.maximum_height / 2;
    }
    masks[i] = from_rect(m);
    if (!(m.x0 == -1 && m.y0 == -1 && m.x1 == -1 && m.y1 == -1)) valid++;
  }
  return valid;
}

void uphip_align_mask(UphipImage image0, const UphipRectangle inside_area,
                      const UphipRectangle outside, UphipMaskAlignmentParameters params) {
  if (!ok_image(image0, "align_mask")) return;
  MonoProxy mp(image0, true, "align_mask");
  if (!mp.ok()) return;
  const UphipImage image = mp.image();
  const Rect in = to_rect(inside_area), out = to_rect(outside);
  const int32_t iw = iabs(in.x0 - in.x1) + 1, ih = iabs(in.y0 - in.y1) + 1;
  int32_t tx, ty;
  if (params.alignment.left) tx = out.x0 + params.margin.horizontal;
  else if (params.alignment.right) tx = out.x1 - iw - params.margin.horizontal;
  else tx = (out.x0 + out.x1 - iw) / 2;
  if (params.alignment.top) ty = out.y0 + params.margin.vertical;
  else if (params.alignment.bottom) ty = out.y1 - ih - params.margin.vertical;
  else ty = (out.y0 + out.y1 - ih) / 2;
  UphipFrame* f = image.frame;
  MoveArgs a{in, tx, ty, {image.background.r, image.background.g, image.background.b}, 1};
  hipStream_t st = current_stream();
  UphipFrame* n = frame_alloc(f->width, f->height, f->format);
  if (!n) return;
  MoveArgs* d = stage_args(&a, 1, st);
  if (!d) return;
  launch_move_rect(ref_of(f), ref_of(n), d, 1, st);
  arg_fence(st);
  adopt_storage(f, n);
  mp.finish();
}

UphipBorder uphip_detect_border(UphipImage image0, UphipBorderScanParameters params,
                                const UphipRectangle outside_mask) {
  UphipBorder b{0, 0, 0, 0};
  if (!ok_image(image0, "detect_border")) return b;
  MonoProxy mp(image0, false, "detect_border");
  if (!mp.ok()) return b;
  const UphipImage image = mp.image();
  UphipFrame* f = image.frame;
  const int32_t W = f->width, H = f->height;
  const Rect o = to_rect(outside_mask);
  b = UphipBorder{o.x0, o.y0, W - o.x1, H - o.y1};
  hipStream_t st = current_stream();
  const int32_t stride = imax(W, H);
  uint32_t* sums = (uint32_t*)scratch(0, sizeof(uint32_t) * stride * 2);
  int32_t* res = (int32_t*)scratch(1, sizeof(int32_t) * 4);
  if (!sums || !res) return b;
  UPH_HIP(hipMemsetAsync(sums, 0, sizeof(uint32_t) * stride * 2, st));
  const int32_t mw = iabs(o.x0 - o.x1) + 1, mh = iabs(o.y0 - o.y1) + 1;
  BorderEdgeArgs e[4];
  memset(e, 0, sizeof(e));
  if (params.scan_direction.horizontal) {
    AxisArgs aa{clip(Rect{0, o.y0, W - 1, o.y1}, W, H), image.abs_black_threshold,
                o.y0 <= o.y1 ? 1 : 0};
    AxisArgs* d = stage_args(&aa, 1, st);
    if (!d) return b;
    if (aa.active && aa.region.y1 >= aa.region.y0)
      launch_axis_reduce(ref_of(f), d, 0, M_DARK_COUNT, W, H, sums, 0, 1, st);
    const int32_t sz = params.scan_size.width, stp = params.scan_step.horizontal;
    e[0] = BorderEdgeArgs{1, 0, W, o.x0, o.x0 + sz, stp, mw, params.scan_threshold.horizontal};
    e[1] = BorderEdgeArgs{1, 0, W, o.x1 - sz, o.x1, -stp, mw, params.scan_threshold.horizontal};
  }
  if (params.scan_direction.vertical) {
    AxisArgs aa{clip(Rect{o.x0, 0, o.x1, H - 1}, W, H), image.abs_black_threshold,
                o.x0 <= o.x1 ? 1 : 0};
    AxisArgs* d = stage_args(&aa, 1, st);
    if (!d) return b;
    if (aa.active && aa.region.x1 >= aa.region.x0)
      launch_axis_reduce(ref_of(f), d, 1, M_DARK_COUNT, W, H, sums + stride, 0, 1, st);
    const int32_t sz = params.scan_size.height, stp = params.scan_step.vertical;
    e[2] = BorderEdgeArgs{1, stride, H, o.y0, o.y0 + sz, stp, mh, params.scan_threshold.vertical};
    e[3] = BorderEdgeArgs{1, stride, H, o.y1 - sz, o.y1, -stp, mh, params.scan_threshold.vertical};
  }
  BorderEdgeArgs* de = stage_args(e, 4, st);
  if (!de) return b;
  UPH_HIP(hipMemsetAsync(res, 0, sizeof(int32_t) * 4, st));
  launch_border_scan(de, 4, sums, 0, res, 1, st, imax(W, H));
  arg_fence(st);
  int32_t r[4];
  UPH_HIP(hipMemcpyAsync(r, res, sizeof(r), hipMemcpyDeviceToHost, st));
  if (!UPH_HIP(hipStreamSynchronize(st))) return b;
  if (params.scan_direction.horizontal) {
    b.left += r[0];
    b.right += r[1];
  }
  if (params.scan_direction.vertical) {
    b.top += r[2];
    b.bottom += r[3];
  }
  return b;
}

void uphip_deskew(UphipImage source0, UphipRectangle mask, float radians,
                  UphipInterpolation interp) {
  if (!ok_image(source0, "deskew")) return;
  MonoProxy mp(source0, true, "deskew");
  if (!mp.ok()) return;
  const UphipImage source = mp.image();
  UphipFrame* f = source.frame;
  RotateArgs a{to_rect(mask), sinf(-radians), cosf(-radians), 1};
  hipStream_t st = current_stream();
  UphipFrame* n = frame_alloc(f->width, f->height, f->format);
  if (!n) return;
  RotateArgs* d = stage_args(&a, 1, st);
  if (!d) return;
  if (!(interp == UPHIP_INTERP_LINEAR &&
        launch_rotate_linear(ref_of(f), ref_of(n), d, 1, 1, nullptr, 1, st, radians)))
    launch_rotate_mask(ref_of(f), ref_of(n), d, interp, 1, st, radians);
  arg_fence(st);
  adopt_storage(f, n);
  mp.finish();
}

}
```

unpaper-gpu_amd/csrc/pipeline.hip:

```cpp
#include <cstdio>
#include <cstdlib>
#include <cmath>
#include <cstring>
#include <string>
#include <vector>

#include "filters.h"
#include "jpeg_enc.h"
#include "libm_glibc.h"
#include "runtime.h"

namespace uph {

__global__ void k_ctl_init(SheetCtl* ctl, int count, int32_t npoints, UphipPoint p0, UphipPoint p1) {
  const int s = blockIdx.x * blockDim.x + threadIdx.x;
  if (s >= count) return;
  SheetCtl& c = ctl[s];
  c.cur = 0;
  c.status = 0;
  c.point_count = npoints;
  c.mask_count = 0;
  c.points[0] = p0;
  c.points[1] = p1;
  for (int i = 0; i < UPHIP_MAX_PAGES; i++) c.rotation[i] = 0.0f;
}

__global__ void k_status_fold(const SheetCtl* ctl, int count, int32_t* sticky) {
  const int s = blockIdx.x * blockDim.x + threadIdx.x;
  if (s < count && ctl[s].status) atomicOr(sticky, ctl[s].status);
}

__global__ void k_jenc_sources(const SheetCtl* ctl, const uint8_t* p0, const uint8_t* p1,
                               int64_t pitch, int64_t stride, int oc, int64_t page_bytes,
                               JencImage* out, int n) {
  const int i = blockIdx.x * blockDim.x + threadIdx.x;
  if (i >= n) return;
  const int s = i / oc, j = i - s * oc;
  const uint8_t* base = (ctl[s].cur & 1) ? p1 : p0;
  out[i] = JencImage{base + (int64_t)s * stride + (int64_t)j * page_bytes, pitch};
}

__global__ void k_flip_all(SheetCtl* ctl, int count) {
  const int s = blockIdx.x * blockDim.x + threadIdx.x;
  if (s < count) ctl[s].cur ^= 1;
}

struct MaskAssembleArgs {
  UphipMaskDetectionParameters p;
  int32_t W, H, npoints, assign;
};

__global__ void k_mask_assemble(SheetCtl* ctl, const int32_t* edges, MaskAssembleArgs a,
                                int count) {
  const int s = blockIdx.x * blockDim.x + threadIdx.x;
  if (s >= count) return;
  SheetCtl& c = ctl[s];
  const UphipMaskDetectionParameters& p = a.p;
  int32_t valid = 0;
  for (int i = 0; i < a.npoints; i++) {
    const int32_t* e = edges + ((int64_t)s * a.npoints + i) * 4;
    const UphipPoint o = c.points[i];
    Rect m;
    if (p.scan_direction.horizontal) {
      m.x0 = o.x - (p.scan_step.horizontal * e[0]) - p.scan_size.width / 2;
      m.x1 = o.x + (p.scan_step.horizontal * e[1]) + p.scan_size.width / 2;
    } else {
      m.x0 = 0;
      m.x1 = a.W - 1;
    }
    if (p.scan_direction.vertical) {
      m.y0 = o.y - (p.scan_step.vertical * e[2]) - p.scan_size.height / 2;
      m.y1 = o.y + (p.scan_step.vertical * e[3]) + p.scan_size.height / 2;
    } else {
      m.y0 = 0;
      m.y1 = a.H - 1;
    }
    const int32_t mw = iabs(m.x0 - m.x1) + 1, mh = iabs(m.y0 - m.y1) + 1;
    if ((p.minimum_width != -1 && mw < p.minimum_width) ||
        (p.maximum_width != -1 && mw > p.maximum_width)) {
      m.x0 = o.x - p.maximum_width / 2;
      m.x1 = o.x + p.maximum_width / 2;
    }
    if ((p.minimum_height != -1 && mh < p.minimum_height) ||
        (p.maximum_height != -1 && mh > p.maximum_height)) {
      m.y0 = o.y - p.maximum_height / 2;
      m.y1 = o.y + p.maximum_height / 2;
    }
    c.masks[i] = from_rect(m);
    if (!(m.x0 == -1 && m.y0 == -1 && m.x1 == -1 && m.y1 == -1)) valid++;
  }
  if (a.assign) c.mask_count = valid;
}

__global__ void k_mask_pick(const SheetCtl* ctl, int i, Rect* out, int32_t* active, int count,
                            const int32_t* only) {
  const int s = blockIdx.x * blockDim.x + threadIdx.x;
  if (s >= count) return;
  out[s] = to_rect(ctl[s].masks[i]);
  active[s] = i < ctl[s].mask_count && (!only || only[s]);
}

__global__ void k_rot_independent(const SheetCtl* ctl, const RotateArgs* args, int64_t mstride,
                                  int32_t* indep, int32_t* dep, int count) {
  const int s = blockIdx.x * blockDim.x + threadIdx.x;
  if (s >= count) return;
  const SheetCtl& c = ctl[s];
  const RotateArgs a0 = args[s], a1 = args[mstride + s];
  bool d = false;
  if (c.mask_count >= 2 && a0.active) {
    const Rect m0 = normalize(to_rect(c.masks[0])), m1 = normalize(to_rect(c.masks[1]));
    auto meets = [](const Rect& p, const Rect& q) {
      return p.x0 <= q.x1 && q.x0 <= p.x1 && p.y0 <= q.y1 && q.y0 <= p.y1;
    };
    d = meets(m0, m1);
    if (!d && a1.active) {
      const Rect nm = normalize(a1.mask);
      const int32_t sw = nm.x1 - nm.x0 + 1, sh = nm.y1 - nm.y0 + 1;
      const float scx = nm.x0 + sw / 2.0f, scy = nm.y0 + sh / 2.0f;
      const float tcx = 0 + sw / 2.0f, tcy = 0 + sh / 2.0f;
      const float cs = a1.cosval, sn = a1.sinval, mg = 4.0f;
      float mnx = 3.0e38f, mxx = -3.0e38f, mny = 3.0e38f, mxy = -3.0e38f;
      for (int k = 0; k < 4; k++) {
        const int32_t u = k & 1 ? sw - 1 : 0, v = k & 2 ? sh - 1 : 0;
        const float X = scx + (u - tcx) * cs + (v - tcy) * sn;
        const float Y = scy + (v - tcy) * cs - (u - tcx) * sn;
        mnx = fminf(mnx, X);
        mxx = fmaxf(mxx, X);
        mny = fminf(mny, Y);
        mxy = fmaxf(mxy, Y);
      }
      bool sep = mxx + mg < (float)m0.x0 || mnx - mg > (float)m0.x1 || mxy + mg < (float)m0.y0 ||
                 mny - mg > (float)m0.y1;
      if (!sep) {
        float au = 3.0e38f, bu = -3.0e38f, av = 3.0e38f, bv = -3.0e38f;
        for (int k = 0; k < 4; k++) {
          const float dx = (float)(k & 1 ? m0.x1 : m0.x0) - scx;
          const float dy = (float)(k & 2 ? m0.y1 : m0.y0) - scy;
          const float pu = dx * cs - dy * sn, pv = dx * sn + dy * cs;
          au = fminf(au, pu);
          bu = fmaxf(bu, pu);
          av = fminf(av, pv);
          bv = fmaxf(bv, pv);
        }
        sep = bu + mg < -tcx || au - mg > (sw - 1) - tcx || bv + mg < -tcy || av - mg > (sh - 1) - tcy;
      }
      d = !sep;
    }
  }
  dep[s] = d;
  indep[s] = !d;
}

__global__ void k_zero_sums_if_active(const RotateArgs* args, uint32_t* sums, int64_t stride,
                                      int32_t n) {
  const int s = blockIdx.y;
  if (!args[s].active) return;
  for (int32_t i = blockIdx.x * blockDim.x + threadIdx.x; i < n; i += gridDim.x * blockDim.x)
    sums[s * stride + i] = 0;
}

__global__ void k_flip_rot2(SheetCtl* ctl, const RotateArgs* args, int64_t mstride,
                            const int32_t* indep, int count) {
  const int s = blockIdx.x * blockDim.x + threadIdx.x;
  if (s >= count) return;
  if (args[s].active || (args[mstride + s].active && indep[s])) ctl[s].cur ^= 1;
}

struct RotCombo {
  float result, sinv, cosv;
};

struct RotSelectArgs {
  int32_t nangles, nedges;
  int32_t negate[4];
  int32_t max_masks, mask_index;
  float deviation_rad;
  UphipRectangle dummy;
};

__global__ void __launch_bounds__(64) k_rot_select(SheetCtl* ctl, const int32_t* peaks,
                                                   const RotTable* table, const RotCombo* combo,
                                                   RotSelectArgs a, RotateArgs* out, int count,
                                                   const int32_t* only, const uint32_t* pow2,
                                                   int npow2) {
  const int s = blockIdx.x, lane = threadIdx.x;
  if (s >= count) return;
  if (only && !only[s]) {
    if (lane == 0) out[s].active = 0;
    return;
  }
  SheetCtl& c = ctl[s];
  const int i = a.mask_index;
  const bool active = i < c.mask_count;
  int idx[4] = {0, 0, 0, 0};
  for (int e = 0; e < a.nedges; e++) {
    const int32_t* pk = peaks + (((int64_t)s * a.max_masks + i) * 4 + e) * a.nangles;
    int best = 0, bi = 0;
    for (int k = lane; k < a.nangles; k += 64) {
      const int v = pk[k];
      if (v > best) {
        best = v;
        bi = k;
      }
    }
    for (int o = 32; o > 0; o >>= 1) {
      const int ob = __shfl_xor(best, o, 64), oi = __shfl_xor(bi, o, 64);
      if (ob > best || (ob == best && oi < bi)) {
        best = ob;
        bi = oi;
      }
    }
    idx[e] = best > 0 ? bi : 0;
  }
  if (lane != 0) return;
  RotCombo r;
  if (a.nedges <= 2) {
    int key = 0;
    if (a.nedges >= 1) key = idx[0];
    if (a.nedges == 2) key = idx[0] * a.nangles + idx[1];
    r = combo[key];
  } else {
    float rot[4], total = 0.0f;
    for (int e = 0; e < a.nedges; e++) {
      const float v = table->angle[idx[e]];
      rot[e] = a.negate[e] ? -v : v;
      total += rot[e];
    }
    const float avg = __fdiv_rn(total, (float)a.nedges);
    float t2 = 0.0f;
    for (int e = 0; e < a.nedges; e++) t2 += glibc::pow2(rot[e] - avg, pow2, npow2);
    r.result = __fsqrt_rn(t2) <= a.deviation_rad ? avg : 0.0f;
    r.sinv = glibc::sinf(-r.result);
    r.cosv = glibc::cosf(-r.result);
  }
  if (i < UPHIP_MAX_PAGES) c.rotation[i] = active ? r.result : 0.0f;
  RotateArgs ra;
  ra.mask = to_rect(c.masks[i]);
  ra.sinval = r.sinv;
  ra.cosval = r.cosv;
  ra.active = active && r.result != 0.0f;
  out[s] = ra;
}

__global__ void k_center_args(const SheetCtl* ctl, int i, int32_t W, int32_t H, UphipPixel bg,
                              MoveArgs* out, int count) {
  const int s = blockIdx.x * blockDim.x + threadIdx.x;
  if (s >= count) return;
  const SheetCtl& c = ctl[s];
  MoveArgs m;
  m.area = to_rect(c.masks[i]);
  const int32_t sw = iabs(m.area.x0 - m.area.x1) + 1, sh = iabs(m.area.y0 - m.area.y1) + 1;
  m.tx = c.points[i].x - sw / 2;
  m.ty = c.points[i].y - sh / 2;
  m.bg[0] = bg.r;
  m.bg[1] = bg.g;
  m.bg[2] = bg.b;
  const Rect na = rect_from_size(m.tx, m.ty, sw, sh);
  const Rect img{0, 0, W - 1, H - 1};
  bool active = i < c.mask_count && point_in(na.x0, na.y0, img) && point_in(na.x1, na.y1, img);
  const Rect n = normalize(m.area);
  const Rect cl = clip(m.area, W, H);
  if (active && n.x0 == m.area.x0 && n.y0 == m.area.y0 && cl.x0 == n.x0 && cl.y0 == n.y0 &&
      cl.x1 == n.x1 && cl.y1 == n.y1 && m.tx == n.x0 && m.ty == n.y0)
    active = false;
  m.active = active;
  out[s] = m;
}

struct BorderAssembleArgs {
  int32_t W, H, nout, cap;
  Rect outside[UPHIP_MAX_PAGES];
  int32_t horizontal, vertical, align;
  UphipMaskAlignmentParameters ap;
  uint8_t mask_color[3];
  uint8_t bg[3];
};

__global__ void k_border_assemble(SheetCtl* ctl, const int32_t* res, BorderAssembleArgs a,
                                  MaskArgs* masks_out, MoveArgs* move_out, int count) {
  const int s = blockIdx.x * blockDim.x + threadIdx.x;
  if (s >= count) return;
  SheetCtl& c = ctl[s];
  MaskArgs& ma = masks_out[s];
  ma.n = a.nout;
  ma.color[0] = a.mask_color[0];
  ma.color[1] = a.mask_color[1];
  ma.color[2] = a.mask_color[2];
  for (int i = 0; i < a.nout; i++) {
    const Rect o = a.outside[i];
    const int32_t* r = res + ((int64_t)s * a.nout + i) * 4;
    int32_t left = o.x0, top = o.y0, right = a.W - o.x1, bottom = a.H - o.y1;
    if (a.horizontal) {
      left += r[0];
      right += r[1];
    }
    if (a.vertical) {
      top += r[2];
      bottom += r[3];
    }
    const Rect m{left, top, a.W - right - 1, a.H - bottom - 1};
    c.border_masks[i] = from_rect(m);
    ma.m[i] = m;
    const int32_t iw = iabs(m.x0 - m.x1) + 1, ih = iabs(m.y0 - m.y1) + 1;
    int32_t tx, ty;
    if (a.ap.alignment.left) tx = o.x0 + a.ap.margin.horizontal;
    else if (a.ap.alignment.right) tx = o.x1 - iw - a.ap.margin.horizontal;
    else tx = (o.x0 + o.x1 - iw) / 2;
    if (a.ap.alignment.top) ty = o.y0 + a.ap.margin.vertical;
    else if (a.ap.alignment.bottom) ty = o.y1 - ih - a.ap.margin.vertical;
    else ty = (o.y0 + o.y1 - ih) / 2;
    MoveArgs mv;
    mv.area = m;
    mv.tx = tx;
    mv.ty = ty;
    mv.bg[0] = a.bg[0];
    mv.bg[1] = a.bg[1];
    mv.bg[2] = a.bg[2];
    const Rect n = normalize(m);
    const Rect cl = clip(m, a.W, a.H);
    const bool identity = n.x0 == m.x0 && n.y0 == m.y0 && cl.x0 == n.x0 && cl.y0 == n.y0 &&
                          cl.x1 == n.x1 && cl.y1 == n.y1 && tx == n.x0 && ty == n.y0;
    mv.active = a.align && !identity;
    move_out[(int64_t)i * a.cap + s] = mv;
  }
}

}

using namespace uph;

struct UphipBatch {
  UphipOptions o;
  UphipBatchGeometry geo;
  int device = 0;
  hipStream_t st = nullptr;
  int cap = 0, n_in = 1;
  size_t dev_bytes = 0;
  int32_t rp_w = 0, rp_h = 0;
  int32_t sheet_w = 0, sheet_h = 0;
  int32_t W = 0, H = 0;
  int32_t out_w = 0, out_h = 0;
  int32_t work_fmt = F_GRAY8;
  int32_t out_fmt = F_GRAY8;
  int32_t max_w = 0, max_h = 0;
  int64_t in_pitch = 0, in_page_stride = 0;
  int64_t pitch = 0, plane_stride = 0;
  int64_t out_pitch = 0, out_stride = 0;
  uint8_t* inputs = nullptr;
  uint8_t* planes[2] = {nullptr, nullptr};
  uint8_t* out = nullptr;
  SheetCtl* ctl = nullptr;
  std::vector<UphipPoint> points;
  std::vector<Rect> outside;
  UphipMaskDetectionParameters mask_params;
  UphipBlackfilterParameters black_params;
  uint8_t* scr = nullptr;
  int64_t scr_stride = 0;
  uint8_t* rot_page = nullptr;
  std::vector<void*> allocs;
  std::vector<std::vector<std::pair<const char*, hipEvent_t>>> runs;
  std::vector<std::string> time_names;
  bool timing = false;
  int32_t* sticky = nullptr;
  BlackGeom bgeo{};
  BlackBar* dbars = nullptr;
  AxisArgs *black_h = nullptr, *black_v = nullptr;
  NoiseGeom ngeo{};
  BlurGeom blgeo{};
  GrayGeom ggeo{};
  RotTable table{};
  RotTable* dtable = nullptr;
  RotCombo* dcombo = nullptr;
  uint32_t* dpow2 = nullptr;
  int npow2 = 0;
  int max_scan = 0;
  float max_angle = 0.0f;
  int32_t* peaks = nullptr;
  int32_t* rot_lines = nullptr;
  Rect* pick_mask = nullptr;
  int32_t* pick_active = nullptr;
  RotateArgs* rot_args = nullptr;
  int32_t* rot_indep = nullptr;
  int32_t* rot_dep = nullptr;
  uint32_t* nbits = nullptr;
  int64_t nbits_stride = 0;
  uint32_t* bbits = nullptr;
  MoveArgs* move_args = nullptr;
  int32_t* border_need = nullptr;
  MaskArgs* border_mask_args = nullptr;
  int32_t* edge_res = nullptr;
  int32_t* border_res = nullptr;
  uint32_t* sums = nullptr;
  int64_t sums_stride = 0;
  struct Prepared;
  std::vector<std::string> names;
  std::vector<float> times;
  int last_count = 0;
  std::vector<void*> cache;
  size_t cache_pos = 0;
  JencContext* jenc = nullptr;
  int jenc_pages = 0;
};

namespace {

template <class T>
T* dalloc(UphipBatch* b, size_t n) {
  void* p = nullptr;
  if (!UPH_HIP(hipMalloc(&p, sizeof(T) * (n ? n : 1)))) return nullptr;
  b->allocs.push_back(p);
  b->dev_bytes += sizeof(T) * (n ? n : 1);
  return (T*)p;
}

void* upload_cached(UphipBatch* b, const void* host, size_t bytes) {
  if (b->cache_pos < b->cache.size()) return b->cache[b->cache_pos++];
  void* d = nullptr;
  if (!UPH_HIP(hipMalloc(&d, bytes ? bytes : 1))) return nullptr;
  b->allocs.push_back(d);
  b->dev_bytes += bytes ? bytes : 1;
  if (host) UPH_HIP(hipMemcpy(d, host, bytes, hipMemcpyHostToDevice));
  b->cache.push_back(d);
  b->cache_pos++;
  return d;
}

template <class T>
T* replicate(UphipBatch* b, const T& v) {
  std::vector<T> h((size_t)b->cap, v);
  return (T*)upload_cached(b, h.data(), sizeof(T) * h.size());
}

bool is_gray_px(UphipPixel p) { return p.r == p.g && p.g == p.b; }

int compare_sizes_h(int32_t aw, int32_t ah, int32_t bw, int32_t bh) {
  if (ah == bh && aw == bw) return 0;
  return imin(ah, aw) < imin(bh, bw) ? -1 : 1;
}

Planes planes_of(UphipBatch* b, int32_t w, int32_t h) {
  Planes P;
  P.base[0] = b->planes[0];
  P.base[1] = b->planes[1];
  P.pitch = b->pitch;
  P.stride = b->plane_stride;
  P.W = w;
  P.H = h;
  P.fmt = b->work_fmt;
  P.count = b->cap;
  return P;
}

void mark(UphipBatch* b, const char* name) {
  if (!b->timing) return;
  if (b->runs.empty()) return;
  hipEvent_t e;
  hipEventCreate(&e);
  hipEventRecord(e, b->st);
  b->runs.back().push_back({name, e});
}

void flip_all(UphipBatch* b, int count) {
  hipLaunchKernelGGL(k_flip_all, dim3((count + 255) / 256), dim3(256), 0, b->st, b->ctl, count);
}

}

static bool plan(UphipBatch* b) {
  const UphipOptions& o = b->o;
  const int n = b->n_in;
  b->rp_w = b->geo.page_width;
  b->rp_h = b->geo.page_height;
  if (o.pre_rotate != 0) std::swap(b->rp_w, b->rp_h);
  b->sheet_w = o.sheet_size.width == -1 ? b->rp_w * n : o.sheet_size.width;
  b->sheet_h = o.sheet_size.height == -1 ? b->rp_h : o.sheet_size.height;
  const bool gray_in = b->geo.page_format != UPHIP_FMT_RGB24;
  b->work_fmt = (gray_in && is_gray_px(o.sheet_background) && is_gray_px(o.mask_color)) ? F_GRAY8
                                                                                       : F_RGB24;
  int32_t w = b->sheet_w, h = b->sheet_h;
  b->max_w = w;
  b->max_h = h;
  {
    int32_t sw = o.stretch_size.width == -1 ? w : o.stretch_size.width;
    int32_t sh = o.stretch_size.height == -1 ? h : o.stretch_size.height;
    sw *= o.pre_zoom_factor;
    sh *= o.pre_zoom_factor;
    if (compare_sizes_h(w, h, sw, sh) != 0) {
      w = sw;
      h = sh;
    }
    b->max_w = imax(b->max_w, w);
    b->max_h = imax(b->max_h, h);
    if (o.page_size.width != -1 || o.page_size.height != -1) {
      const int32_t pw = o.page_size.width == -1 ? w : o.page_size.width;
      const int32_t ph = o.page_size.height == -1 ? h : o.page_size.height;
      if (compare_sizes_h(w, h, pw, ph) != 0) {
        const float hr = (float)pw / (float)w, vr = (float)ph / (float)h;
        int32_t ssw, ssh;
        if (hr < vr) {
          ssw = pw;
          ssh = (int32_t)(h * hr);
        } else if (vr < hr) {
          ssw = (int32_t)(w * vr);
          ssh = ph;
        } else {
          ssw = pw;
          ssh = ph;
        }
        b->max_w = imax(b->max_w, ssw);
        b->max_h = imax(b->max_h, ssh);
        w = pw;
        h = ph;
      }
    }
  }
  b->W = w;
  b->H = h;
  b->max_w = imax(b->max_w, w);
  b->max_h = imax(b->max_h, h);
  int32_t ow = w, oh = h;
  if (o.post_rotate != 0) std::swap(ow, oh);
  b->max_w = imax(b->max_w, ow);
  b->max_h = imax(b->max_h, oh);
  {
    int32_t sw = o.post_stretch_size.width == -1 ? ow : o.post_stretch_size.width;
    int32_t sh = o.post_stretch_size.height == -1 ? oh : o.post_stretch_size.height;
    sw *= o.post_zoom_factor;
    sh *= o.post_zoom_factor;
    if (compare_sizes_h(ow, oh, sw, sh) != 0) {
      ow = sw;
      oh = sh;
    }
    b->max_w = imax(b->max_w, ow);
    b->max_h = imax(b->max_h, oh);
    if (o.post_page_size.width != -1 || o.post_page_size.height != -1) {
      const int32_t pw = o.post_page_size.width == -1 ? ow : o.post_page_size.width;
      const int32_t ph = o.post_page_size.height == -1 ? oh : o.post_page_size.height;
      if (compare_sizes_h(ow, oh, pw, ph) != 0) {
        const float hr = (float)pw / (float)ow, vr = (float)ph / (float)oh;
        int32_t ssw, ssh;
        if (hr < vr) {
          ssw = pw;
          ssh = (int32_t)(oh * hr);
        } else if (vr < hr) {
          ssw = (int32_t)(ow * vr);
          ssh = ph;
        } else {
          ssw = pw;
          ssh = ph;
        }
        b->max_w = imax(b->max_w, ssw);
        b->max_h = imax(b->max_h, ssh);
        ow = pw;
        oh = ph;
      }
    }
  }
  b->out_w = ow;
  b->out_h = oh;
  b->max_w = imax(b->max_w, ow);
  b->max_h = imax(b->max_h, oh);
  if (b->W <= 0 || b->H <= 0 || b->out_w <= 0 || b->out_h <= 0) return fail("batch: empty sheet");
  int32_t of = o.output_pixel_format == UPHIP_FMT_NONE ? b->geo.page_format : o.output_pixel_format;
  if (of == UPHIP_FMT_Y400A) of = UPHIP_FMT_GRAY8;
  if (of == UPHIP_FMT_MONOBLACK) of = UPHIP_FMT_MONOWHITE;
  b->out_fmt = of;
  const int32_t W = b->W, H = b->H;
  b->points.assign(o.points, o.points + o.point_count);
  int32_t mmw = o.mask_detection_parameters.maximum_width;
  int32_t mmh = o.mask_detection_parameters.maximum_height;
  if (o.layout == UPHIP_LAYOUT_SINGLE) {
    if (b->points.empty()) b->points.push_back(UphipPoint{W / 2, H / 2});
    if (mmw == -1) mmw = W;
    if (mmh == -1) mmh = H;
    b->outside.push_back(Rect{0, 0, W - 1, H - 1});
  } else if (o.layout == UPHIP_LAYOUT_DOUBLE) {
    if (b->points.empty()) {
      b->points.push_back(UphipPoint{W / 4, H / 2});
      b->points.push_back(UphipPoint{W - W / 4, H / 2});
    }
    if (mmw == -1) mmw = W / 2;
    if (mmh == -1) mmh = H;
    b->outside.push_back(Rect{0, 0, W / 2, H - 1});
    b->outside.push_back(Rect{W / 2, 0, W - 1, H - 1});
  }
  if (mmw == -1) mmw = W;
  if (mmh == -1) mmh = H;
  if (b->points.size() > UPHIP_MAX_PAGES)
    return fail("batch: at most %d mask points are supported (got %zu)", UPHIP_MAX_PAGES,
                b->points.size());
  b->mask_params = o.mask_detection_parameters;
  b->mask_params.maximum_width = mmw;
  b->mask_params.maximum_height = mmh;
  b->black_params = o.blackfilter_parameters;
  if (b->black_params.exclusions_count == 0 && o.layout != UPHIP_LAYOUT_NONE) {
    UphipBlackfilterParameters& bp = b->black_params;
    if (o.layout == UPHIP_LAYOUT_SINGLE) {
      bp.exclusions[bp.exclusions_count++] = from_rect(rect_from_size(W / 4, H / 4, W / 2, H / 2));
    } else {
      const int32_t fw = W / 4, fh = H / 2;
      bp.exclusions[bp.exclusions_count++] = from_rect(rect_from_size(W / 8, H / 4, fw, fh));
      bp.exclusions[bp.exclusions_count++] =
          from_rect(rect_from_size(W / 8 + W / 2, H / 4, fw, fh));
    }
  }
  return true;
}

static bool allocate(UphipBatch* b) {
  const int cap = b->cap;
  const UphipOptions& o = b->o;
  b->in_pitch = round_pitch(row_bytes(b->geo.page_width, b->geo.page_format));
  b->in_page_stride = b->in_pitch * b->geo.page_height;
  b->inputs = dalloc<uint8_t>(b, (size_t)b->in_page_stride * cap * b->n_in);
  const int bpp = b->work_fmt == F_GRAY8 ? 1 : 3;
  b->pitch = round_pitch((int64_t)b->max_w * bpp);
  b->plane_stride = b->pitch * b->max_h;
  b->planes[0] = dalloc<uint8_t>(b, (size_t)b->plane_stride * cap);
  b->planes[1] = dalloc<uint8_t>(b, (size_t)b->plane_stride * cap);
  if (b->out_fmt != b->work_fmt) {
    b->out_pitch = round_pitch(row_bytes(b->out_w, b->out_fmt));
    b->out_stride = b->out_pitch * b->out_h;
    b->out = dalloc<uint8_t>(b, (size_t)b->out_stride * cap);
    if (b->out) UPH_HIP(hipMemset(b->out, 0, (size_t)b->out_stride * cap));
  }
  if (o.pre_rotate != 0) {
    const int64_t rp = round_pitch(row_bytes(b->rp_w, b->geo.page_format));
    b->rot_page = dalloc<uint8_t>(b, (size_t)rp * b->rp_h * cap);
  }
  b->ctl = dalloc<SheetCtl>(b, cap);
  b->sticky = dalloc<int32_t>(b, 1);
  if (!b->inputs || !b->planes[0] || !b->planes[1] || !b->ctl || !b->sticky) return false;
  if (!UPH_HIP(hipMemset(b->sticky, 0, sizeof(int32_t)))) return false;
  const int32_t W = b->W, H = b->H;
  size_t need = 0;
  std::vector<BlackBar> bars(2 * (size_t)(W + H) + 16);
  if (!(o.disable & UPHIP_NO_BLACKFILTER)) {
    if (b->work_fmt == F_GRAY8 && o.abs_black_threshold == 255)
      return fail("batch: abs_black_threshold 255 makes the reference flood fill recurse forever");
    if (!black_geometry(W, H, b->black_params, o.abs_black_threshold, &b->bgeo, bars.data(),
                        (int)bars.size()))
      return fail("batch: invalid blackfilter parameters");
    need = std::max(need, black_scratch_bytes(b->bgeo));
    if (b->bgeo.nbars) {
      b->dbars = dalloc<BlackBar>(b, b->bgeo.nbars);
      UPH_HIP(hipMemcpy(b->dbars, bars.data(), sizeof(BlackBar) * b->bgeo.nbars,
                        hipMemcpyHostToDevice));
    }
    std::vector<AxisArgs> hv((size_t)cap, AxisArgs{b->bgeo.hregion, 0, 1});
    b->black_h = dalloc<AxisArgs>(b, cap);
    UPH_HIP(hipMemcpy(b->black_h, hv.data(), sizeof(AxisArgs) * cap, hipMemcpyHostToDevice));
    hv.assign((size_t)cap, AxisArgs{b->bgeo.vregion, 0, 1});
    b->black_v = dalloc<AxisArgs>(b, cap);
    UPH_HIP(hipMemcpy(b->black_v, hv.data(), sizeof(AxisArgs) * cap, hipMemcpyHostToDevice));
  }
  if (!(o.disable & UPHIP_NO_NOISEFILTER)) {
    noise_geometry(W, H, o.noisefilter_intensity, o.abs_white_threshold, &b->ngeo);
    need = std::max(need, noise_scratch_bytes(b->ngeo));
    if (b->work_fmt == F_GRAY8) {
      b->nbits_stride = ((int64_t)noise_bit_words(W) * H + 63) & ~(int64_t)63;
      b->nbits = dalloc<uint32_t>(b, (size_t)b->nbits_stride * cap);
      if (!b->nbits) return false;
    }
  }
  if (!(o.disable & UPHIP_NO_BLURFILTER)) {
    if (!blur_geometry(W, H, o.blurfilter_parameters, o.abs_white_threshold, &b->blgeo))
      return fail("batch: invalid blurfilter parameters");
    need = std::max(need, blur_scratch_bytes(b->blgeo));
    if (blur_bits_usable(b->blgeo, b->work_fmt)) {
      b->nbits_stride = ((int64_t)noise_bit_words(W) * H + 63) & ~(int64_t)63;
      b->bbits = dalloc<uint32_t>(b, (size_t)b->nbits_stride * cap);
      if (!b->bbits) return false;
    }
  }
  if (!(o.disable & UPHIP_NO_GRAYFILTER)) {
    if (!gray_geometry(W, H, o.grayfilter_parameters, o.abs_black_threshold, &b->ggeo))
      return fail("batch: invalid grayfilter parameters");
    need = std::max(need, gray_scratch_bytes(b->ggeo));
  }
  need = (need + 255) & ~(size_t)255;
  b->scr_stride = (int64_t)need;
  if (need) {
    b->scr = dalloc<uint8_t>(b, need * cap);
    if (!b->scr) return false;
  }
  const int np = (int)b->points.size();
  const int nout = (int)b->outside.size();
  b->sums_stride = (int64_t)imax(b->max_w, b->max_h) * 2 * imax(np, nout) + 64;
  b->sums = dalloc<uint32_t>(b, (size_t)b->sums_stride * cap);
  b->edge_res = dalloc<int32_t>(b, (size_t)cap * imax(np, 1) * 4);
  b->border_res = dalloc<int32_t>(b, (size_t)cap * imax(nout, 1) * 4);
  b->move_args = dalloc<MoveArgs>(b, (size_t)cap * UPHIP_MAX_PAGES);
  b->border_need = dalloc<int32_t>(b, cap);
  b->border_mask_args = dalloc<MaskArgs>(b, cap);
  b->rot_args = dalloc<RotateArgs>(b, (size_t)cap * UPHIP_MAX_PAGES);
  b->rot_indep = dalloc<int32_t>(b, cap);
  b->rot_dep = dalloc<int32_t>(b, cap);
  b->pick_mask = dalloc<Rect>(b, cap);
  b->pick_active = dalloc<int32_t>(b, cap);
  if (!(o.disable & UPHIP_NO_DESKEW)) {
    if (rotation_angles(o.deskew_parameters, &b->table) < 0)
      return fail("batch: too many deskew angles");
    const int na = b->table.nangles;
    for (int i = 0; i < na; i++) b->max_angle = fmaxf(b->max_angle, fabsf(b->table.angle[i]));
    b->dtable = dalloc<RotTable>(b, 1);
    UPH_HIP(hipMemcpy(b->dtable, &b->table, sizeof(RotTable), hipMemcpyHostToDevice));
    int nedges = 0;
    int kinds[4];
    const UphipEdges& E = o.deskew_parameters.scan_edges;
    const bool on[4] = {E.left, E.top, E.right, E.bottom};
    for (int k = 0; k < 4; k++)
      if (on[k]) kinds[nedges++] = k;
    size_t ncombo = nedges == 2 ? (size_t)na * na : (size_t)na;
    std::vector<RotCombo> combo(ncombo);
    for (size_t key = 0; key < ncombo; key++) {
      float rot[2];
      int idx[2] = {(int)(nedges == 2 ? key / na : key), (int)(key % na)};
      for (int e = 0; e < nedges && e < 2; e++) {
        const float v = b->table.angle[idx[e]];
        rot[e] = (kinds[e] == 1 || kinds[e] == 3) ? -v : v;
      }
      RotCombo c;
      c.result = combine_edge_rotations(rot, nedges > 2 ? 2 : nedges,
                                        o.deskew_parameters.deskewScanDeviationRad);
      c.sinv = sinf(-c.result);
      c.cosv = cosf(-c.result);
      combo[key] = c;
    }
    b->dcombo = dalloc<RotCombo>(b, ncombo);
    UPH_HIP(hipMemcpy(b->dcombo, combo.data(), sizeof(RotCombo) * ncombo, hipMemcpyHostToDevice));
    if (nedges > 2) {
      const uint32_t* t = glibc_pow2_table(&b->npow2);
      if (!t) return fail("batch: this libm's powf(x, 2) is not reproducible on the device");
      b->dpow2 = dalloc<uint32_t>(b, imax(b->npow2, 1));
      UPH_HIP(hipMemcpy(b->dpow2, t, sizeof(uint32_t) * b->npow2, hipMemcpyHostToDevice));
    }
    b->peaks = dalloc<int32_t>(b, (size_t)cap * UPHIP_MAX_PAGES * 4 * (na > 0 ? na : 1));
    int ms = o.deskew_parameters.deskewScanSize;
    if (ms == -1 || ms > 10000) ms = 10000;
    b->max_scan = imin(ms, imax(W, H));
    b->rot_lines = (int32_t*)dalloc<uint8_t>(b, rotation_lines_bytes(cap, nedges, na, b->max_scan));
    if (!b->rot_lines) return false;
  }
  return true;
}

static void fill_uniform(UphipBatch* b, const Planes& P, int which, Rect clipped, UphipPixel c,
                         int count) {
  if (clipped.x1 < clipped.x0 || clipped.y1 < clipped.y0) return;
  FillArgs fa{clipped, {c.r, c.g, c.b}, 1};
  FillArgs* d = replicate(b, fa);
  launch_fill_thr(PlaneRef{P, b->ctl, which}, d, count, clipped.y1 - clipped.y0 + 1,
                  b->o.abs_black_threshold, b->st);
}

static void masks_uniform(UphipBatch* b, const Planes& P, const Rect* m, int n, UphipPixel c,
                          int count) {
  if (n <= 0) return;
  MaskArgs ma;
  memset(&ma, 0, sizeof(ma));
  ma.n = n;
  ma.color[0] = c.r;
  ma.color[1] = c.g;
  ma.color[2] = c.b;
  for (int i = 0; i < n; i++) ma.m[i] = m[i];
  MaskArgs* d = replicate(b, ma);
  launch_apply_masks_thr(cur_ref(P, b->ctl), d, count, b->o.abs_black_threshold, b->st);
}

static void wipes_uniform(UphipBatch* b, const Planes& P, const UphipWipes& w, int count) {
  for (size_t i = 0; i < w.count && i < UPHIP_MAX_MASKS; i++) {
    const Rect r = to_rect(w.areas[i]);
    if (r.x0 > r.x1 || r.y0 > r.y1) continue;
    fill_uniform(b, P, 0, clip(r, P.W, P.H), b->o.mask_color, count);
  }
}

static void border_uniform(UphipBatch* b, const Planes& P, const UphipBorder& br, int count) {
  if (br.left == 0 && br.top == 0 && br.right == 0 && br.bottom == 0) return;
  const Rect m{br.left, br.top, P.W - br.right - 1, P.H - br.bottom - 1};
  masks_uniform(b, P, &m, 1, b->o.mask_color, count);
}

static void stretch_all(UphipBatch* b, int32_t& w, int32_t& h, int32_t nw, int32_t nh,
                        int count) {
  if (compare_sizes_h(w, h, nw, nh) == 0) return;
  const Planes S = planes_of(b, w, h), D = planes_of(b, nw, nh);
  launch_stretch_thr(cur_ref(S, b->ctl), other_ref(D, b->ctl), b->o.interpolate_type,
                     b->o.abs_black_threshold, count, b->st);
  flip_all(b, count);
  w = nw;
  h = nh;
}

static void resize_all(UphipBatch* b, int32_t& w, int32_t& h, int32_t pw, int32_t ph,
                       int count) {
  if (compare_sizes_h(w, h, pw, ph) == 0) return;
  const float hr = (float)pw / (float)w, vr = (float)ph / (float)h;
  int32_t sw, sh;
  if (hr < vr) {
    sw = pw;
    sh = (int32_t)(h * hr);
  } else if (vr < hr) {
    sw = (int32_t)(w * vr);
    sh = ph;
  } else {
    sw = pw;
    sh = ph;
  }
  stretch_all(b, w, h, sw, sh, count);
  if (pw == sw && ph == sh) return;
  const Planes D = planes_of(b, pw, ph);
  fill_uniform(b, D, 1, Rect{0, 0, pw - 1, ph - 1}, b->o.sheet_background, count);
  int32_t sox = 0, soy = 0, tox = 0, toy = 0, ssw = w, ssh = h;
  if (ssw <= pw) tox += (pw - ssw) / 2;
  else {
    sox += (ssw - pw) / 2;
    ssw = pw;
  }
  if (ssh <= ph) toy += (ph - ssh) / 2;
  else {
    soy += (ssh - ph) / 2;
    ssh = ph;
  }
  CopyArgs ca{clip(rect_from_size(sox, soy, ssw, ssh), w, h), tox, toy, 1};
  CopyArgs* d = replicate(b, ca);
  launch_copy_thr(cur_ref(planes_of(b, w, h), b->ctl), other_ref(D, b->ctl), d, count, ssh,
                  b->o.abs_black_threshold, b->st);
  flip_all(b, count);
  w = pw;
  h = ph;
}

static bool mask_scan_all_rows(const UphipBatch* b) {
  const UphipMaskDetectionParameters& p = b->mask_params;
  if (b->points.size() != 1 || !p.scan_direction.horizontal || p.scan_direction.vertical) return false;
  if (b->work_fmt != F_GRAY8) return false;
  const int32_t depth = p.scan_depth.horizontal == -1 ? b->H : p.scan_depth.horizontal;
  const int32_t c0 = b->points[0].y - depth / 2, c1 = c0 + depth - 1;
  return c0 <= 0 && c1 >= b->H - 1;
}
static bool mask_sums_from_gray(const UphipBatch* b) {
  const UphipOptions& o = b->o;
  if (o.disable & (UPHIP_NO_DESKEW | UPHIP_NO_MASK_SCAN | UPHIP_NO_GRAYFILTER)) return false;
  return mask_scan_all_rows(b);
}
static bool mask_sums_from_rotate(const UphipBatch* b) {
  const UphipOptions& o = b->o;
  if (o.disable & (UPHIP_NO_DESKEW | UPHIP_NO_MASK_SCAN | UPHIP_NO_MASK_CENTER)) return false;
  return mask_scan_all_rows(b);
}

static void detect_masks_all(UphipBatch* b, int assign, int count, bool sums_ready = false) {
  const UphipMaskDetectionParameters& p = b->mask_params;
  if (!p.scan_direction.horizontal && !p.scan_direction.vertical) return;
  const int np = (int)b->points.size();
  const int32_t W = b->W, H = b->H;
  const Planes P = planes_of(b, W, H);
  if (!sums_ready)
    UPH_HIP(hipMemsetAsync(b->sums, 0, sizeof(uint32_t) * b->sums_stride * count, b->st));
  std::vector<EdgeArgs> ea((size_t)np * 4);
  for (int i = 0; i < np; i++) {
    const UphipPoint o = b->points[i];
    for (int k = 0; k < 4; k++) ea[i * 4 + k].active = 0;
    if (p.scan_direction.horizontal) {
      const int32_t depth = p.scan_depth.horizontal == -1 ? H : p.scan_depth.horizontal;
      const int32_t c0 = o.y - depth / 2, c1 = c0 + depth - 1;
      const Rect reg = clip(Rect{0, c0, W - 1, c1}, W, H);
      const int32_t off = (2 * i) * imax(W, H);
      if (reg.y1 >= reg.y0 && !(sums_ready && i == 0)) {
        AxisArgs* aa = replicate(b, AxisArgs{reg, 0, 1});
        launch_axis_reduce(cur_ref(P, b->ctl), aa, 0, M_GRAY_SUM, W, H, b->sums + off,
                           b->sums_stride, count, b->st);
      }
      for (int k = 0; k < 2; k++) {
        EdgeArgs& e = ea[i * 4 + k];
        e = EdgeArgs{1, off, W, H, c0, c1, o.x - p.scan_size.width / 2,
                     (k == 0 ? -1 : 1) * p.scan_step.horizontal, p.scan_size.width,
                     p.scan_threshold.horizontal};
      }
    }
    if (p.scan_direction.vertical) {
      const int32_t depth = p.scan_depth.vertical == -1 ? W : p.scan_depth.vertical;
      const int32_t c0 = o.x - depth / 2, c1 = c0 + depth - 1;
      const Rect reg = clip(Rect{c0, 0, c1, H - 1}, W, H);
      const int32_t off = (2 * i + 1) * imax(W, H);
      if (reg.x1 >= reg.x0) {
        AxisArgs* aa = replicate(b, AxisArgs{reg, 0, 1});
        launch_axis_reduce(cur_ref(P, b->ctl), aa, 1, M_GRAY_SUM, W, H, b->sums + off,
                           b->sums_stride, count, b->st);
      }
      for (int k = 2; k < 4; k++) {
        EdgeArgs& e = ea[i * 4 + k];
        e = EdgeArgs{1, off, H, W, c0, c1, o.y - p.scan_size.height / 2,
                     (k == 2 ? -1 : 1) * p.scan_step.vertical, p.scan_size.height,
                     p.scan_threshold.vertical};
      }
    }
  }
  std::vector<EdgeArgs> all((size_t)b->cap * np * 4);
  for (int s = 0; s < b->cap; s++)
    for (int j = 0; j < np * 4; j++) all[(size_t)s * np * 4 + j] = ea[j];
  EdgeArgs* de = (EdgeArgs*)upload_cached(b, all.data(), sizeof(EdgeArgs) * all.size());
  launch_edge_scan(de, np * 4, b->sums, b->sums_stride, b->edge_res, count, b->st, imax(W, H));
  MaskAssembleArgs ma{p, W, H, np, assign};
  hipLaunchKernelGGL(k_mask_assemble, dim3((count + 255) / 256), dim3(256), 0, b->st, b->ctl,
                     b->edge_res, ma, count);
}

static bool border_rows_from_center(const UphipBatch* b) {
  const UphipOptions& o = b->o;
  const uint32_t dis = o.disable;
  const UphipBorderScanParameters& p = o.border_scan_parameters;
  if ((dis & UPHIP_NO_MASK_CENTER) || b->points.empty()) return false;
  if ((dis & UPHIP_NO_BORDER_SCAN) || b->outside.size() != 1) return false;
  if (p.scan_direction.horizontal || !p.scan_direction.vertical) return false;
  if (b->work_fmt != F_GRAY8) return false;
  if (b->outside[0].x0 > b->outside[0].x1) return false;
  if (!(dis & UPHIP_NO_WIPE)) {
    if (o.wipes.count > 0) return false;
    if (o.layout == UPHIP_LAYOUT_DOUBLE && (o.middle_wipe[0] > 0 || o.middle_wipe[1] > 0)) return false;
  }
  if (!(dis & UPHIP_NO_BORDER) &&
      (o.border.left || o.border.top || o.border.right || o.border.bottom))
    return false;
  return true;
}

static bool chain_center_align(const UphipBatch* b) {
  if (!border_rows_from_center(b) || b->points.size() != 1) return false;
  if (b->o.disable & UPHIP_NO_BORDER_ALIGN) return false;
  return b->pitch * (int64_t)b->H < (1ll << 31) && UPHIP_MAX_PAGES >= 2;
}

constexpr int32_t kBorderEdgeRows = 320;
static bool border_edge_rows_only(const UphipBatch* b) { return b->H > 2 * kBorderEdgeRows + 64; }
static MoveExtra center_count_args(const UphipBatch* b) {
  const Rect oc = clip(b->outside[0], b->W, b->H);
  MoveExtra x{};
  x.rows = b->sums + imax(b->W, b->H);
  x.rows_stride = b->sums_stride;
  x.rx0 = oc.x0;
  x.rx1 = oc.x1;
  x.thr = b->o.abs_black_threshold;
  return x;
}

static void border_all(UphipBatch* b, int count, bool rows_ready,
                       const MoveArgs* center = nullptr) {
  const UphipBorderScanParameters& p = b->o.border_scan_parameters;
  const int nout = (int)b->outside.size();
  const int32_t W = b->W, H = b->H;
  const Planes P = planes_of(b, W, H);
  if (!rows_ready)
    UPH_HIP(hipMemsetAsync(b->sums, 0, sizeof(uint32_t) * b->sums_stride * count, b->st));
  std::vector<BorderEdgeArgs> ea((size_t)nout * 4);
  memset(ea.data(), 0, sizeof(BorderEdgeArgs) * ea.size());
  for (int i = 0; i < nout; i++) {
    const Rect o = b->outside[i];
    const int32_t mw = iabs(o.x0 - o.x1) + 1, mh = iabs(o.y0 - o.y1) + 1;
    if (p.scan_direction.horizontal) {
      const int32_t off = (2 * i) * imax(W, H);
      AxisArgs a{clip(Rect{0, o.y0, W - 1, o.y1}, W, H), b->o.abs_black_threshold,
                 o.y0 <= o.y1 ? 1 : 0};
      if (a.active && a.region.y1 >= a.region.y0)
        launch_axis_reduce(cur_ref(P, b->ctl), replicate(b, a), 0, M_DARK_COUNT, W, H,
                           b->sums + off, b->sums_stride, count, b->st);
      const int32_t sz = p.scan_size.width, stp = p.scan_step.horizontal;
      ea[i * 4 + 0] = BorderEdgeArgs{1, off, W, o.x0, o.x0 + sz, stp, mw, p.scan_threshold.horizontal};
      ea[i * 4 + 1] = BorderEdgeArgs{1, off, W, o.x1 - sz, o.x1, -stp, mw, p.scan_threshold.horizontal};
    }
    if (p.scan_direction.vertical) {
      const int32_t off = (2 * i + 1) * imax(W, H);
      AxisArgs a{clip(Rect{o.x0, 0, o.x1, H - 1}, W, H), b->o.abs_black_threshold,
                 o.x0 <= o.x1 ? 1 : 0};
      if (a.active && a.region.x1 >= a.region.x0 && !rows_ready)
        launch_axis_reduce(cur_ref(P, b->ctl), replicate(b, a), 1, M_DARK_COUNT, W, H,
                           b->sums + off, b->sums_stride, count, b->st);
      const int32_t sz = p.scan_size.height, stp = p.scan_step.vertical;
      ea[i * 4 + 2] = BorderEdgeArgs{1, off, H, o.y0, o.y0 + sz, stp, mh, p.scan_threshold.vertical};
      ea[i * 4 + 3] = BorderEdgeArgs{1, off, H, o.y1 - sz, o.y1, -stp, mh, p.scan_threshold.vertical};
    }
  }
  std::vector<BorderEdgeArgs> all((size_t)b->cap * nout * 4);
  for (int s = 0; s < b->cap; s++)
    for (int j = 0; j < nout * 4; j++) all[(size_t)s * nout * 4 + j] = ea[j];
  BorderEdgeArgs* de =
      (BorderEdgeArgs*)upload_cached(b, all.data(), sizeof(BorderEdgeArgs) * all.size());
  UPH_HIP(hipMemsetAsync(b->border_res, 0, sizeof(int32_t) * count * nout * 4, b->st));
  if (center && border_edge_rows_only(b)) {
    UPH_HIP(hipMemsetAsync(b->border_need, 0, sizeof(int32_t) * count, b->st));
    launch_border_scan(de, nout * 4, b->sums, b->sums_stride, b->border_res, count, b->st,
                       imax(W, H), kBorderEdgeRows, H - kBorderEdgeRows, b->border_need);
    MoveExtra x = center_count_args(b);
    x.dry = true;
    x.ya0 = kBorderEdgeRows;
    x.ya1 = H - kBorderEdgeRows;
    x.only = b->border_need;
    launch_move_rect_fused(cur_ref(P, b->ctl), other_ref(P, b->ctl), center, x, count, b->st);
    launch_border_scan(de, nout * 4, b->sums, b->sums_stride, b->border_res, count, b->st,
                       imax(W, H), 0, 0, nullptr, b->border_need);
  } else {
    launch_border_scan(de, nout * 4, b->sums, b->sums_stride, b->border_res, count, b->st,
                       imax(W, H));
  }
  BorderAssembleArgs ba;
  memset(&ba, 0, sizeof(ba));
  ba.W = W;
  ba.H = H;
  ba.nout = nout;
  ba.cap = b->cap;
  for (int i = 0; i < nout; i++) ba.outside[i] = b->outside[i];
  ba.horizontal = p.scan_direction.horizontal;
  ba.vertical = p.scan_direction.vertical;
  ba.align = !(b->o.disable & UPHIP_NO_BORDER_ALIGN);
  ba.ap = b->o.mask_alignment_parameters;
  ba.mask_color[0] = b->o.mask_color.r;
  ba.mask_color[1] = b->o.mask_color.g;
  ba.mask_color[2] = b->o.mask_color.b;
  ba.bg[0] = b->o.sheet_background.r;
  ba.bg[1] = b->o.sheet_background.g;
  ba.bg[2] = b->o.sheet_background.b;
  hipLaunchKernelGGL(k_border_assemble, dim3((count + 255) / 256), dim3(256), 0, b->st, b->ctl,
                     b->border_res, ba, b->border_mask_args, b->move_args, count);
  const bool align = !(b->o.disable & UPHIP_NO_BORDER_ALIGN);
  const bool fold = align && nout == 1 && P.fmt == F_GRAY8;
  if (center) {
    launch_move_chain(cur_ref(P, b->ctl), other_ref(P, b->ctl), center, b->border_mask_args,
                      b->move_args, count, b->st);
    flip_all(b, count);
    return;
  }
  if (!fold)
    launch_apply_masks_thr(cur_ref(P, b->ctl), b->border_mask_args, count,
                           b->o.abs_black_threshold, b->st);
  for (int i = 0; i < nout && align; i++) {
    MoveArgs* mv = b->move_args + (int64_t)i * b->cap;
    if (fold) {
      MoveExtra x{};
      x.masks = b->border_mask_args;
      launch_move_rect_fused(cur_ref(P, b->ctl), other_ref(P, b->ctl), mv, x, count, b->st);
    } else {
      launch_move_rect(cur_ref(P, b->ctl), other_ref(P, b->ctl), mv, count, b->st);
    }
    launch_flip_if_active(b->ctl, &mv->active, sizeof(MoveArgs), count, b->st);
  }
}

static bool decode_fused(const UphipBatch* b, const uint8_t* src, int64_t spitch,
                         int64_t sstride) {
  const UphipOptions& o = b->o;
  const uint32_t dis = o.disable;
  if (b->work_fmt != F_GRAY8 || b->geo.page_format != F_GRAY8 || b->n_in != 1) return false;
  if (b->rp_w != b->sheet_w || b->rp_h != b->sheet_h || o.pre_rotate != 0) return false;
  if (b->sheet_w != b->W || b->sheet_h != b->H) return false;
  if (((uintptr_t)src & 15) || (spitch & 15) || (sstride & 15)) return false;
  if (o.pre_mirror.horizontal || o.pre_mirror.vertical) return false;
  if (o.pre_shift.horizontal != 0 || o.pre_shift.vertical != 0 || o.pre_mask_count > 0) return false;
  if (!(dis & UPHIP_NO_WIPE) && o.pre_wipes.count > 0) return false;
  if (!(dis & UPHIP_NO_BORDER) &&
      (o.pre_border.left || o.pre_border.top || o.pre_border.right || o.pre_border.bottom))
    return false;
  return true;
}

static bool run_batch(UphipBatch* b, int count, const uint8_t* src, int64_t spitch,
                      int64_t sstride) {
  const UphipOptions& o = b->o;
  const uint32_t dis = o.disable;
  if (b->timing) b->runs.emplace_back();
  b->cache_pos = 0;
  mark(b, "start");
  const UphipPoint p0 = b->points.size() > 0 ? b->points[0] : UphipPoint{0, 0};
  const UphipPoint p1 = b->points.size() > 1 ? b->points[1] : UphipPoint{0, 0};
  hipLaunchKernelGGL(k_ctl_init, dim3((count + 255) / 256), dim3(256), 0, b->st, b->ctl, count,
                     (int32_t)b->points.size(), p0, p1);
  const int n = b->n_in;
  int32_t w = b->sheet_w, h = b->sheet_h;
  Planes S0 = planes_of(b, w, h);
  const bool covered = n == 1 && b->rp_w == w && b->rp_h == h;
  const bool fused = decode_fused(b, src, spitch, sstride);
  SheetBits bits;
  if (fused) {
    const bool black_on = !(dis & UPHIP_NO_BLACKFILTER) && b->bgeo.nbars > 0;
    bits.nbits = !(dis & UPHIP_NO_NOISEFILTER) ? b->nbits : nullptr;
    bits.bbits = !(dis & UPHIP_NO_BLURFILTER) ? b->bbits : nullptr;
    bits.stride = b->nbits_stride;
    bits.vsum = black_on && b->bgeo.vregion.x1 >= b->bgeo.vregion.x0;
    bits.rm = black_on;
    launch_decode_gray(src, spitch, sstride, cur_ref(S0, b->ctl), o.abs_white_threshold, bits,
                       b->bgeo, b->scr, b->scr_stride, count, b->st);
  }
  if (!covered) fill_uniform(b, S0, 0, Rect{0, 0, w - 1, h - 1}, o.sheet_background, count);
  for (int j = 0; j < n && !fused; j++) {
    Planes pg;
    pg.base[0] = pg.base[1] = const_cast<uint8_t*>(src) + j * sstride;
    pg.pitch = spitch;
    pg.stride = sstride * n;
    pg.W = b->geo.page_width;
    pg.H = b->geo.page_height;
    pg.fmt = b->geo.page_format;
    pg.count = count;
    if (o.pre_rotate != 0) {
      Planes rp;
      rp.base[0] = rp.base[1] = b->rot_page;
      rp.pitch = round_pitch(row_bytes(b->rp_w, pg.fmt));
      rp.stride = rp.pitch * b->rp_h;
      rp.W = b->rp_w;
      rp.H = b->rp_h;
      rp.fmt = pg.fmt;
      rp.count = count;
      launch_rotate90_thr(fixed_ref(pg, 0), fixed_ref(rp, 0), o.pre_rotate / 90,
                          o.abs_black_threshold, count, b->st);
      pg = rp;
    }
    int32_t tox = w * j / n, toy = 0, tw = w / n, th = h;
    int32_t sox = 0, soy = 0, ssw = pg.W, ssh = pg.H;
    if ((ssw < tw || ssh < th) && covered == false) {
    }
    if (ssw <= tw) tox += (tw - ssw) / 2;
    else {
      sox += (ssw - tw) / 2;
      ssw = tw;
    }
    if (ssh <= th) toy += (th - ssh) / 2;
    else {
      soy += (ssh - th) / 2;
      ssh = th;
    }
    CopyArgs ca{clip(rect_from_size(sox, soy, ssw, ssh), pg.W, pg.H), tox, toy, 1};
    launch_copy_thr(fixed_ref(pg, 0), cur_ref(S0, b->ctl), replicate(b, ca), count, ssh,
                    o.abs_black_threshold, b->st);
  }
  mark(b, "decode");
  if (o.pre_mirror.horizontal || o.pre_mirror.vertical) {
    const Planes P = planes_of(b, w, h);
    launch_mirror_oop(cur_ref(P, b->ctl), other_ref(P, b->ctl), o.pre_mirror.horizontal,
                      o.pre_mirror.vertical, o.abs_black_threshold, count, b->st);
    flip_all(b, count);
  }
  if (o.pre_shift.horizontal != 0 || o.pre_shift.vertical != 0) {
    const Planes P = planes_of(b, w, h);
    const uint8_t bg[3] = {o.sheet_background.r, o.sheet_background.g, o.sheet_background.b};
    launch_shift(cur_ref(P, b->ctl), other_ref(P, b->ctl), o.pre_shift.horizontal,
                 o.pre_shift.vertical, bg, o.abs_black_threshold, count, b->st);
    flip_all(b, count);
  }
  if (o.pre_mask_count > 0) {
    std::vector<Rect> pm(o.pre_mask_count);
    for (size_t i = 0; i < o.pre_mask_count; i++) pm[i] = to_rect(o.pre_masks[i]);
    masks_uniform(b, planes_of(b, w, h), pm.data(), (int)pm.size(), o.mask_color, count);
  }
  {
    int32_t sw = o.stretch_size.width == -1 ? w : o.stretch_size.width;
    int32_t sh = o.stretch_size.height == -1 ? h : o.stretch_size.height;
    sw *= o.pre_zoom_factor;
    sh *= o.pre_zoom_factor;
    stretch_all(b, w, h, sw, sh, count);
    if (o.page_size.width != -1 || o.page_size.height != -1)
      resize_all(b, w, h, o.page_size.width == -1 ? w : o.page_size.width,
                 o.page_size.height == -1 ? h : o.page_size.height, count);
  }
  const Planes P = planes_of(b, b->W, b->H);
  if (!(dis & UPHIP_NO_WIPE)) wipes_uniform(b, P, o.pre_wipes, count);
  if (!(dis & UPHIP_NO_BORDER)) border_uniform(b, P, o.pre_border, count);
  mark(b, "pre");
  if (!(dis & UPHIP_NO_BLACKFILTER) && b->bgeo.nbars > 0) {
    launch_blackfilter(cur_ref(P, b->ctl), b->bgeo, b->dbars, b->scr, b->scr_stride, b->ctl, count,
                       b->st, b->black_h, b->black_v, bits);
    mark(b, "blackfilter");
  }
  if (!(dis & UPHIP_NO_NOISEFILTER)) {
    launch_noisefilter(cur_ref(P, b->ctl), b->ngeo, b->scr, b->scr_stride, b->ctl, count, b->st,
                       bits);
    mark(b, "noisefilter");
  }
  if (!(dis & UPHIP_NO_BLURFILTER)) {
    launch_blurfilter(cur_ref(P, b->ctl), b->blgeo, b->scr, b->scr_stride, count, b->st, bits);
    mark(b, "blurfilter");
  }
  bool mask_sums_ready = false;
  bool center_sums_ready = false;
  if (!(dis & UPHIP_NO_GRAYFILTER)) {
    uint32_t* cs = nullptr;
    if (mask_sums_from_gray(b)) {
      UPH_HIP(hipMemsetAsync(b->sums, 0, sizeof(uint32_t) * b->sums_stride * count, b->st));
      cs = b->sums;
    }
    mask_sums_ready = launch_grayfilter(cur_ref(P, b->ctl), b->ggeo, b->scr, b->scr_stride, count,
                                        b->st, cs, b->sums_stride);
    mark(b, "grayfilter");
  }
  if (!(dis & UPHIP_NO_DESKEW)) {
    if (!(dis & UPHIP_NO_MASK_SCAN)) {
      detect_masks_all(b, 1, count, mask_sums_ready);
      mark(b, "masks_deskew");
    }
    const UphipEdges& E = o.deskew_parameters.scan_edges;
    RotGeom rg;
    memset(&rg, 0, sizeof(rg));
    rg.W = b->W;
    rg.H = b->H;
    const int shifts[4][2] = {{1, 0}, {0, 1}, {-1, 0}, {0, -1}};
    const bool on[4] = {E.left, E.top, E.right, E.bottom};
    RotSelectArgs ra;
    memset(&ra, 0, sizeof(ra));
    for (int k = 0; k < 4; k++)
      if (on[k]) {
        rg.edge_shift[rg.nedges][0] = shifts[k][0];
        rg.edge_shift[rg.nedges][1] = shifts[k][1];
        ra.negate[rg.nedges] = (k == 1 || k == 3);
        rg.nedges++;
      }
    rg.scan_size = o.deskew_parameters.deskewScanSize;
    rg.scan_depth = o.deskew_parameters.deskewScanDepth;
    rg.max_masks = UPHIP_MAX_PAGES;
    ra.nangles = b->table.nangles;
    ra.nedges = rg.nedges;
    ra.max_masks = UPHIP_MAX_PAGES;
    ra.deviation_rad = o.deskew_parameters.deskewScanDeviationRad;
    auto detect = [&](int i, const int32_t* only) {
      hipLaunchKernelGGL(k_mask_pick, dim3((count + 255) / 256), dim3(256), 0, b->st, b->ctl, i,
                         b->pick_mask, b->pick_active, count, only);
      launch_rotation_peaks(cur_ref(P, b->ctl), rg, b->dtable, b->pick_mask, b->pick_active, i,
                            b->peaks, count, b->st, b->table.nangles, b->max_scan, b->rot_lines,
                            b->max_angle);
#ifdef UPHIP_DIAG
      if (getenv("UPHIP_DIAG_ROTATION")) {
        const int nl = count * rg.nedges * b->table.nangles;
        std::vector<int32_t> fl((size_t)nl);
        UPH_HIP(hipMemcpyAsync(fl.data(), rotation_line_flags(b->rot_lines, nl, b->max_scan),
                               sizeof(int32_t) * nl, hipMemcpyDeviceToHost, b->st));
        UPH_HIP(hipStreamSynchronize(b->st));
        int nf = 0;
        for (int t = 0; t < nl; t++) nf += fl[t] != 0;
        fprintf(stderr, "uphip: batch rotation %d of %d lines walked directly\n", nf, nl);
      }
#endif
      ra.mask_index = i;
      hipLaunchKernelGGL(k_rot_select, dim3(count), dim3(64), 0, b->st, b->ctl,
                         b->peaks, b->dtable, b->dcombo, ra, b->rot_args + (int64_t)i * b->cap,
                         count, only, b->dpow2, b->npow2);
    };
    const bool linear = o.interpolate_type == UPHIP_INTERP_LINEAR &&
                        (P.fmt == F_GRAY8 || P.fmt == F_RGB24);
    auto rotate = [&](const RotateArgs* args, int nmask, const int32_t* indep,
                      uint32_t* colsum = nullptr) {
      if (linear && launch_rotate_linear(cur_ref(P, b->ctl), other_ref(P, b->ctl), args, nmask,
                                         b->cap, indep, count, b->st, b->max_angle))
        return false;
      return launch_rotate_mask(cur_ref(P, b->ctl), other_ref(P, b->ctl), args,
                                o.interpolate_type, count, b->st, b->max_angle, colsum,
                                b->sums_stride);
    };
    if (linear && b->points.size() == 2) {
      detect(0, nullptr);
      detect(1, nullptr);
      hipLaunchKernelGGL(k_rot_independent, dim3((count + 255) / 256), dim3(256), 0, b->st,
                         b->ctl, b->rot_args, (int64_t)b->cap, b->rot_indep, b->rot_dep, count);
      mark(b, "deskew_detect");
      rotate(b->rot_args, 2, b->rot_indep);
      mark(b, "deskew_rotate");
      hipLaunchKernelGGL(k_flip_rot2, dim3((count + 255) / 256), dim3(256), 0, b->st, b->ctl,
                         b->rot_args, (int64_t)b->cap, b->rot_indep, count);
      RotateArgs* a1 = b->rot_args + b->cap;
      detect(1, b->rot_dep);
      mark(b, "deskew_detect");
      rotate(a1, 1, nullptr);
      mark(b, "deskew_rotate");
      launch_flip_if_active(b->ctl, &a1->active, sizeof(RotateArgs), count, b->st);
    } else {
      for (size_t i = 0; i < b->points.size(); i++) {
        detect((int)i, nullptr);
        RotateArgs* ai = b->rot_args + (int64_t)i * b->cap;
        const bool fuse = mask_sums_from_rotate(b);
        if (fuse)
          hipLaunchKernelGGL(k_zero_sums_if_active, dim3(4, count), dim3(256), 0, b->st, ai,
                             b->sums, b->sums_stride, b->W);
        mark(b, "deskew_detect");
        center_sums_ready = rotate(ai, 1, nullptr, fuse ? b->sums : nullptr);
        mark(b, "deskew_rotate");
        launch_flip_if_active(b->ctl, &ai->active, sizeof(RotateArgs), count, b->st);
      }
    }
  }
  const bool rows_fused = border_rows_from_center(b);
  const bool chain = chain_center_align(b);
  MoveArgs* const center_mv = chain ? b->move_args + b->cap : nullptr;
  if (!(dis & UPHIP_NO_MASK_CENTER)) {
    if (!(dis & UPHIP_NO_MASK_SCAN)) {
      detect_masks_all(b, 1, count, center_sums_ready);
      mark(b, "masks_center");
    }
    for (size_t i = 0; i < b->points.size(); i++) {
      MoveArgs* mv = chain ? center_mv : b->move_args;
      hipLaunchKernelGGL(k_center_args, dim3((count + 255) / 256), dim3(256), 0, b->st, b->ctl,
                         (int)i, b->W, b->H, o.sheet_background, mv, count);
      if (rows_fused && i + 1 == b->points.size()) {
        MoveExtra x = center_count_args(b);
        x.dry = chain;
        if (chain && border_edge_rows_only(b)) {
          x.ya0 = 0;
          x.ya1 = kBorderEdgeRows;
          x.yb0 = b->H - kBorderEdgeRows;
          x.yb1 = b->H;
        }
        launch_move_rect_fused(cur_ref(P, b->ctl), other_ref(P, b->ctl), mv, x, count, b->st);
      } else {
        launch_move_rect(cur_ref(P, b->ctl), other_ref(P, b->ctl), mv, count, b->st);
      }
      if (!chain) launch_flip_if_active(b->ctl, &mv->active, sizeof(MoveArgs), count, b->st);
    }
    mark(b, "center");
  }
  if (!(dis & UPHIP_NO_WIPE)) {
    UphipWipes wp = o.wipes;
    if (o.layout == UPHIP_LAYOUT_DOUBLE && (o.middle_wipe[0] > 0 || o.middle_wipe[1] > 0) &&
        wp.count < UPHIP_MAX_MASKS) {
      wp.areas[wp.count++] = from_rect(Rect{b->W / 2 - o.middle_wipe[0], 0,
                                            b->W / 2 + o.middle_wipe[1], b->H - 1});
    }
    wipes_uniform(b, P, wp, count);
  }
  if (!(dis & UPHIP_NO_BORDER)) border_uniform(b, P, o.border, count);
  if (!(dis & UPHIP_NO_BORDER_SCAN) && !b->outside.empty()) {
    border_all(b, count, rows_fused, center_mv);
    mark(b, "border");
  }
  if (!(dis & UPHIP_NO_WIPE)) wipes_uniform(b, P, o.post_wipes, count);
  if (!(dis & UPHIP_NO_BORDER)) border_uniform(b, P, o.post_border, count);
  w = b->W;
  h = b->H;
  if (o.post_mirror.horizontal || o.post_mirror.vertical) {
    const Planes Q = planes_of(b, w, h);
    launch_mirror_oop(cur_ref(Q, b->ctl), other_ref(Q, b->ctl), o.post_mirror.horizontal,
                      o.post_mirror.vertical, o.abs_black_threshold, count, b->st);
    flip_all(b, count);
  }
  if (o.post_shift.horizontal != 0 || o.post_shift.vertical != 0) {
    const Planes Q = planes_of(b, w, h);
    const uint8_t bg[3] = {o.sheet_background.r, o.sheet_background.g, o.sheet_background.b};
    launch_shift(cur_ref(Q, b->ctl), other_ref(Q, b->ctl), o.post_shift.horizontal,
                 o.post_shift.vertical, bg, o.abs_black_threshold, count, b->st);
    flip_all(b, count);
  }
  if (o.post_rotate != 0) {
    const Planes S = planes_of(b, w, h), D = planes_of(b, h, w);
    launch_rotate90_thr(cur_ref(S, b->ctl), other_ref(D, b->ctl), o.post_rotate / 90,
                        o.abs_black_threshold, count, b->st);
    flip_all(b, count);
    std::swap(w, h);
  }
  {
    int32_t sw = o.post_stretch_size.width == -1 ? w : o.post_stretch_size.width;
    int32_t sh = o.post_stretch_size.height == -1 ? h : o.post_stretch_size.height;
    sw *= o.post_zoom_factor;
    sh *= o.post_zoom_factor;
    stretch_all(b, w, h, sw, sh, count);
    if (o.post_page_size.width != -1 || o.post_page_size.height != -1)
      resize_all(b, w, h, o.post_page_size.width == -1 ? w : o.post_page_size.width,
                 o.post_page_size.height == -1 ? h : o.post_page_size.height, count);
  }
  if (b->out) {
    Planes Q = planes_of(b, w, h);
    Planes O;
    O.base[0] = O.base[1] = b->out;
    O.pitch = b->out_pitch;
    O.stride = b->out_stride;
    O.W = w;
    O.H = h;
    O.fmt = b->out_fmt;
    O.count = count;
    CopyArgs ca{Rect{0, 0, w - 1, h - 1}, 0, 0, 1};
    launch_copy_thr(cur_ref(Q, b->ctl), fixed_ref(O, 0), replicate(b, ca), count, h,
                    o.abs_black_threshold, b->st);
  }
  mark(b, "output");
  hipLaunchKernelGGL(k_status_fold, dim3((count + 255) / 256), dim3(256), 0, b->st, b->ctl, count,
                     b->sticky);
  b->last_count = count;
  return uphip_last_error() == nullptr;
}

extern "C" {

UphipBatch* uphip_batch_create(const UphipOptions* options, const UphipBatchGeometry* geometry) {
  if (!options || !geometry) return fail("batch_create: null argument"), nullptr;
  if (!runtime_ready()) return fail("batch_create: no HIP device"), nullptr;
  if (geometry->capacity <= 0 || geometry->page_width <= 0 || geometry->page_height <= 0)
    return fail("batch_create: invalid geometry"), nullptr;
  if (options->input_count < 1 || options->input_count > UPHIP_MAX_PAGES)
    return fail("batch_create: input_count must be 1 or 2"), nullptr;
  if (geometry->page_format < UPHIP_FMT_GRAY8 || geometry->page_format > UPHIP_FMT_MONOBLACK)
    return fail("batch_create: invalid page format"), nullptr;
  UphipBatch* b = new UphipBatch();
  b->o = *options;
  b->geo = *geometry;
  b->cap = geometry->capacity;
  b->n_in = options->input_count;
  b->device = current_device();
  hipSetDevice(b->device);
  if (!UPH_HIP(hipStreamCreateWithFlags(&b->st, hipStreamNonBlocking)) || !plan(b) ||
      !allocate(b)) {
    uphip_batch_destroy(b);
    return nullptr;
  }
  return b;
}

void uphip_batch_destroy(UphipBatch* b) {
  if (!b) return;
  hipSetDevice(b->device);
  if (b->st) hipStreamSynchronize(b->st);
  for (auto& r : b->runs)
    for (auto& m : r) hipEventDestroy(m.second);
  for (void* p : b->allocs) hipFree(p);
  delete b->jenc;
  if (b->st) hipStreamDestroy(b->st);
  delete b;
}

int uphip_batch_output_info(UphipBatch* b, int32_t* width, int32_t* height, int32_t* format,
                            int64_t* bytes_per_sheet) {
  if (!b) return -1;
  if (width) *width = b->out_w;
  if (height) *height = b->out_h;
  if (format) *format = b->out_fmt;
  if (bytes_per_sheet) *bytes_per_sheet = row_bytes(b->out_w, b->out_fmt) * b->out_h;
  return 0;
}

int uphip_batch_device_bytes(UphipBatch* b, int64_t* bytes) {
  if (!b || !bytes) return fail("batch_device_bytes: null argument"), -1;
  *bytes = (int64_t)b->dev_bytes;
  return 0;
}

void* uphip_batch_input_ptr(UphipBatch* b, int32_t slot, int64_t* pitch) {
  if (!b || slot < 0 || slot >= b->cap * b->n_in) return nullptr;
  if (pitch) *pitch = b->in_pitch;
  return b->inputs + (int64_t)slot * b->in_page_stride;
}

int uphip_batch_set_input(UphipBatch* b, int32_t slot, const void* host, int64_t linesize) {
  if (!b || slot < 0 || slot >= b->cap * b->n_in) return fail("batch_set_input: bad slot"), -1;
  hipSetDevice(b->device);
  const int64_t rb = row_bytes(b->geo.page_width, b->geo.page_format);
  return UPH_HIP(hipMemcpy2DAsync(b->inputs + (int64_t)slot * b->in_page_stride, b->in_pitch, host,
                                  linesize, rb, b->geo.page_height, hipMemcpyHostToDevice, b->st))
             ? 0
             : -1;
}

int uphip_batch_run(UphipBatch* b, int32_t count) {
  if (!b || count <= 0 || count > b->cap) return fail("batch_run: bad count"), -1;
  hipSetDevice(b->device);
  return run_batch(b, count, b->inputs, b->in_pitch, b->in_page_stride) ? 0 : -1;
}

int uphip_batch_run_device(UphipBatch* b, int32_t count, const void* pages, int64_t pitch,
                           int64_t page_stride) {
  if (!b || count <= 0 || count > b->cap || !pages)
    return fail("batch_run_device: bad arguments"), -1;
  if (pitch < row_bytes(b->geo.page_width, b->geo.page_format))
    return fail("batch_run_device: pitch too small"), -1;
  hipSetDevice(b->device);
  return run_batch(b, count, (const uint8_t*)pages, pitch, page_stride) ? 0 : -1;
}

int uphip_batch_wait(UphipBatch* b) {
  if (!b) return -1;
  hipSetDevice(b->device);
  if (!UPH_HIP(hipStreamSynchronize(b->st))) return -1;
  int32_t any = 0;
  if (!UPH_HIP(hipMemcpy(&any, b->sticky, sizeof(any), hipMemcpyDeviceToHost))) return -1;
  if (!any) return 0;
  UPH_HIP(hipMemset(b->sticky, 0, sizeof(int32_t)));
  std::vector<SheetCtl> c(b->last_count > 0 ? b->last_count : 1);
  if (b->last_count > 0) {
    UPH_HIP(hipMemcpy(c.data(), b->ctl, sizeof(SheetCtl) * b->last_count,
                      hipMemcpyDeviceToHost));
    for (int s = 0; s < b->last_count; s++)
      if (c[s].status)
        return fail("batch: sheet %d failed on the device (status 0x%x)", s, c[s].status), -1;
  }
  return fail("batch: a sheet of an earlier run since the last wait failed on the device "
              "(status 0x%x)", any), -1;
}

void* uphip_batch_output_ptr(UphipBatch* b, int32_t sheet, int64_t* pitch) {
  if (!b || sheet < 0 || sheet >= b->cap) return nullptr;
  hipSetDevice(b->device);
  if (!UPH_HIP(hipStreamSynchronize(b->st))) return nullptr;
  if (b->out) {
    if (pitch) *pitch = b->out_pitch;
    return b->out + (int64_t)sheet * b->out_stride;
  }
  int32_t cur = 0;
  hipMemcpy(&cur, &b->ctl[sheet].cur, 4, hipMemcpyDeviceToHost);
  if (pitch) *pitch = b->pitch;
  return b->planes[cur] + (int64_t)sheet * b->plane_stride;
}

int uphip_batch_get_output(UphipBatch* b, int32_t sheet, void* host, int64_t linesize) {
  int64_t pitch = 0;
  void* p = uphip_batch_output_ptr(b, sheet, &pitch);
  if (!p) return fail("batch_get_output: bad sheet"), -1;
  const int64_t rb = row_bytes(b->out_w, b->out_fmt);
  if (linesize < rb) return fail("batch_get_output: linesize too small"), -1;
  if (!UPH_HIP(hipMemcpy2DAsync(host, linesize, p, pitch, rb, b->out_h, hipMemcpyDeviceToHost,
                                b->st)))
    return -1;
  return UPH_HIP(hipStreamSynchronize(b->st)) ? 0 : -1;
}

int uphip_batch_get_report(UphipBatch* b, int32_t sheet, UphipSheetReport* r) {
  if (!b || !r || sheet < 0 || sheet >= b->cap) return -1;
  SheetCtl c;
  hipSetDevice(b->device);
  hipStreamSynchronize(b->st);
  if (!UPH_HIP(hipMemcpy(&c, &b->ctl[sheet], sizeof(c), hipMemcpyDeviceToHost))) return -1;
  memset(r, 0, sizeof(*r));
  r->mask_count = c.mask_count;
  for (int i = 0; i < UPHIP_MAX_PAGES; i++) {
    r->masks[i] = c.masks[i];
    r->rotation[i] = c.rotation[i];
    r->border_masks[i] = c.border_masks[i];
  }
  r->width = b->out_w;
  r->height = b->out_h;
  r->flags = (uint32_t)c.status;
  return 0;
}

void* uphip_batch_stream(UphipBatch* b) { return b ? (void*)b->st : nullptr; }

int uphip_batch_output_pitch(UphipBatch* b, int64_t* pitch) {
  if (!b || !pitch) return -1;
  *pitch = b->out ? b->out_pitch : b->pitch;
  return 0;
}

int uphip_batch_query(UphipBatch* b) {
  if (!b) return -1;
  hipSetDevice(b->device);
  const hipError_t e = hipStreamQuery(b->st);
  if (e == hipSuccess) return 1;
  if (e == hipErrorNotReady) return 0;
  return check_hip(e, "hipStreamQuery"), -1;
}

int uphip_batch_upload_async(UphipBatch* b, int32_t count, const void* host, int64_t linesize,
                             int64_t page_stride) {
  if (!b || !host || count <= 0 || count > b->cap)
    return fail("batch_upload_async: bad arguments"), -1;
  const int64_t rb = row_bytes(b->geo.page_width, b->geo.page_format);
  if (linesize < rb) return fail("batch_upload_async: linesize too small"), -1;
  hipSetDevice(b->device);
  const int64_t n = (int64_t)count * b->n_in;
  const uint8_t* h = (const uint8_t*)host;
  if (linesize == b->in_pitch && page_stride == b->in_page_stride)
    return UPH_HIP(hipMemcpyAsync(b->inputs, h, (size_t)(n * page_stride), hipMemcpyHostToDevice,
                                  b->st))
               ? 0
               : -1;
  for (int64_t i = 0; i < n; i++)
    if (!UPH_HIP(hipMemcpy2DAsync(b->inputs + i * b->in_page_stride, b->in_pitch,
                                  h + i * page_stride, linesize, rb, b->geo.page_height,
                                  hipMemcpyHostToDevice, b->st)))
      return -1;
  return 0;
}

int uphip_batch_download_async(UphipBatch* b, void* host, int64_t linesize, int64_t sheet_stride) {
  if (!b || !host || b->last_count <= 0) return fail("batch_download_async: nothing to download"), -1;
  const int64_t rb = row_bytes(b->out_w, b->out_fmt);
  if (linesize < rb) return fail("batch_download_async: linesize too small"), -1;
  hipSetDevice(b->device);
  const hipError_t q = hipStreamQuery(b->st);
  if (q == hipErrorNotReady) return fail("batch_download_async: the run has not finished"), -1;
  if (!check_hip(q, "hipStreamQuery")) return -1;
  const int n = b->last_count;
  std::vector<int32_t> cur((size_t)n, 0);
  if (!b->out &&
      !UPH_HIP(hipMemcpy2D(cur.data(), sizeof(int32_t), &b->ctl[0].cur, sizeof(SheetCtl),
                           sizeof(int32_t), n, hipMemcpyDeviceToHost)))
    return -1;
  uint8_t* h = (uint8_t*)host;
  const int64_t sp = b->out ? b->out_pitch : b->pitch;
  const int64_t ss = b->out ? b->out_stride : b->plane_stride;
  auto src_of = [&](int s) -> const uint8_t* {
    return b->out ? b->out + (int64_t)s * ss : b->planes[cur[s] & 1] + (int64_t)s * ss;
  };
  if (linesize == sp && sheet_stride == sp * b->out_h && ss == sheet_stride) {
    const int64_t extent = (int64_t)(b->out_h - 1) * sp + rb;
    for (int s = 0; s < n;) {
      int e = s + 1;
      while (e < n && (b->out || (cur[e] & 1) == (cur[s] & 1))) e++;
      if (!UPH_HIP(hipMemcpyAsync(h + s * sheet_stride, src_of(s), (size_t)((e - s - 1) * ss + extent),
                                  hipMemcpyDeviceToHost, b->st)))
        return -1;
      s = e;
    }
    return 0;
  }
  for (int s = 0; s < n; s++)
    if (!UPH_HIP(hipMemcpy2DAsync(h + s * sheet_stride, linesize, src_of(s), sp, rb, b->out_h,
                                  hipMemcpyDeviceToHost, b->st)))
      return -1;
  return 0;
}

int uphip_batch_encode_jpeg_async(UphipBatch* b, int32_t quality, int32_t sampling) {
  if (!b || b->last_count <= 0) return fail("batch_encode_jpeg: nothing to encode"), -1;
  if (quality == 0) quality = UPHIP_JPEG_DEFAULT_QUALITY;
  hipSetDevice(b->device);
  const int oc = b->o.output_count < 1 ? 1 : b->o.output_count;
  const int n = b->last_count * oc;
  const int bpp = b->work_fmt == F_GRAY8 ? 1 : 3;
  const int32_t pw = b->out_w / oc;
  const int64_t page = (int64_t)pw * b->out_h * bpp + (64 << 10);
  if (!b->jenc) b->jenc = new JencContext();
  JencContext& c = *b->jenc;
  if (!c.setup(pw, b->out_h, b->work_fmt == F_GRAY8 ? UPHIP_FMT_GRAY8 : UPHIP_FMT_RGB24, sampling,
               quality, n, page / 4, page * n, b->st))
    return -1;
  hipLaunchKernelGGL(k_jenc_sources, dim3((n + 255) / 256), dim3(256), 0, b->st, b->ctl,
                     b->planes[0], b->planes[1], b->pitch, b->plane_stride, oc,
                     (int64_t)pw * bpp, c.B.images, n);
  if (!c.encode_async(b->st)) return -1;
  b->jenc_pages = n;
  return 0;
}

int64_t uphip_batch_jpeg_sizes(UphipBatch* b, int64_t* sizes, int32_t max_pages) {
  if (!b || !b->jenc || b->jenc_pages <= 0) return fail("batch_jpeg_sizes: no encode"), -1;
  if (uphip_batch_query(b) != 1) return fail("batch_jpeg_sizes: the encode has not finished"), -1;
  int64_t total = 0;
  for (int i = 0; i < b->jenc_pages; i++) {
    const int64_t s = b->jenc->host_sizes[i];
    if (sizes && i < max_pages) sizes[i] = s < 0 ? -1 : s;
    if (s > 0) total += s;
  }
  return total;
}

int uphip_batch_jpeg_download_async(UphipBatch* b, void* host, int64_t capacity) {
  const int64_t total = uphip_batch_jpeg_sizes(b, nullptr, 0);
  if (total < 0) return -1;
  if (!host || capacity < total) return fail("batch_jpeg_download: buffer too small"), -1;
  if (total == 0) return 0;
  hipSetDevice(b->device);
  return UPH_HIP(hipMemcpyAsync(host, b->jenc->out, (size_t)total, hipMemcpyDeviceToHost, b->st))
             ? 0
             : -1;
}

int uphip_batch_jpeg_page(UphipBatch* b, int32_t page, const void** device_src, int64_t* pitch,
                          int32_t* width, int32_t* height, int32_t* format) {
  const int oc = b && b->o.output_count > 1 ? b->o.output_count : 1;
  if (!b || page < 0 || page >= b->last_count * oc) return fail("batch_jpeg_page: bad page"), -1;
  hipSetDevice(b->device);
  if (!UPH_HIP(hipStreamSynchronize(b->st))) return -1;
  const int s = page / oc, j = page % oc;
  int32_t cur = 0;
  if (!UPH_HIP(hipMemcpy(&cur, &b->ctl[s].cur, 4, hipMemcpyDeviceToHost))) return -1;
  const int bpp = b->work_fmt == F_GRAY8 ? 1 : 3;
  const int32_t pw = b->out_w / oc;
  if (device_src)
    *device_src = b->planes[cur & 1] + (int64_t)s * b->plane_stride + (int64_t)j * pw * bpp;
  if (pitch) *pitch = b->pitch;
  if (width) *width = pw;
  if (height) *height = b->out_h;
  if (format) *format = b->work_fmt == F_GRAY8 ? UPHIP_FMT_GRAY8 : UPHIP_FMT_RGB24;
  return 0;
}

int uphip_batch_set_timing(UphipBatch* b, int32_t enable) {
  if (!b) return -1;
  b->timing = enable != 0;
  return 0;
}

int uphip_batch_kernel_times(UphipBatch* b, const char** names, float* ms, int max_entries) {
  if (!b) return -1;
  hipSetDevice(b->device);
  if (!UPH_HIP(hipStreamSynchronize(b->st))) return -1;
  std::vector<std::string> order;
  std::vector<double> tot;
  for (auto& r : b->runs) {
    for (size_t i = 1; i < r.size(); i++) {
      float t = 0.0f;
      hipEventElapsedTime(&t, r[i - 1].second, r[i].second);
      size_t k = 0;
      while (k < order.size() && order[k] != r[i].first) k++;
      if (k == order.size()) {
        order.push_back(r[i].first);
        tot.push_back(0.0);
      }
      tot[k] += t;
    }
    for (auto& m : r) hipEventDestroy(m.second);
  }
  b->runs.clear();
  b->time_names = order;
  int k = 0;
  for (; k < (int)order.size() && k < max_entries; k++) {
    if (names) names[k] = b->time_names[k].c_str();
    if (ms) ms[k] = (float)tot[k];
  }
  return k;
}

}
```

Measured before the change: 28420 pages/s.

## Precompute per-tile rotation windows and flags in a separate planning kernel

Adds a k_rot_tiles pre-pass that computes, once per sheet and tile, the rotated source window, its staging, interior, partial and full flags, and the large-angle classification, writing them to a scratch buffer. The cubic GRAY8 rotate kernel then reads these records instead of computing corner transforms with a DPP reduction and an LDS barrier per tile. The large-sheet loop kernel can also exit early when no sheet is large. Global loads and stores are made explicitly global-address-space. The cost is an extra kernel launch and extra scratch memory traffic per rotate.

```diff
diff --git a/unpaper-gpu_amd/csrc/common.h b/unpaper-gpu_amd/csrc/common.h
--- a/unpaper-gpu_amd/csrc/common.h
+++ b/unpaper-gpu_amd/csrc/common.h
@@ -155,16 +155,22 @@
   return m ? (int)__umulhi((uint32_t)n, m) : n;
 }
 __device__ __forceinline__ void xcd_block_m(uint32_t m_gxy, uint32_t m_gx, int* bx, int* by,
-                                            int* bz) {
+                                            int* bz, int* lin_t) {
   const int gx = gridDim.x, gy = gridDim.y;
   const int nblk = gx * gy * gridDim.z;
   const int lin = blockIdx.x + gx * (blockIdx.y + gy * blockIdx.z);
   const int q = nblk >> 3, rr = nblk & 7, xcd = lin & 7;
   const int t = xcd * q + (xcd < rr ? xcd : rr) + (lin >> 3);
+  *lin_t = t;
   *bz = div_by_magic(t, m_gxy);
   const int rem = t - *bz * gx * gy;
   *by = div_by_magic(rem, m_gx);
   *bx = rem - *by * gx;
+}
+__device__ __forceinline__ void xcd_block_m(uint32_t m_gxy, uint32_t m_gx, int* bx, int* by,
+                                            int* bz) {
+  int t;
+  xcd_block_m(m_gxy, m_gx, bx, by, bz, &t);
 }
 
 struct Planes {
diff --git a/unpaper-gpu_amd/csrc/kernels.h b/unpaper-gpu_amd/csrc/kernels.h
--- a/unpaper-gpu_amd/csrc/kernels.h
+++ b/unpaper-gpu_amd/csrc/kernels.h
@@ -85,9 +85,10 @@
 bool launch_move_rect_fused(const PlaneRef& src, const PlaneRef& dst, const MoveArgs* args,
                             const MoveExtra& x, int count, hipStream_t st);
 
+size_t rotate_scratch_bytes(int32_t W, int32_t H, int count);
 bool launch_rotate_mask(const PlaneRef& src, const PlaneRef& dst, const RotateArgs* args,
                         int interp, int count, hipStream_t st, float max_abs_angle,
-                        uint32_t* colsum = nullptr, int64_t cs_stride = 0);
+                        void* scratch, uint32_t* colsum = nullptr, int64_t cs_stride = 0);
 struct LinWindow {
   int32_t cols, rows, stride;
 };
diff --git a/unpaper-gpu_amd/csrc/kernels_rotate.hip b/unpaper-gpu_amd/csrc/kernels_rotate.hip
--- a/unpaper-gpu_amd/csrc/kernels_rotate.hip
+++ b/unpaper-gpu_amd/csrc/kernels_rotate.hip
@@ -3,6 +3,7 @@
 #include "blit_common.h"
 #include "interp.h"
 #include "kernels.h"
+#include "rot_tiles.h"
 
 namespace uph {
 
@@ -476,9 +477,6 @@
   }
 }
 
-constexpr int kRFW = 128;
-constexpr int kRFH = 48;
-constexpr int kRFS = 144;
 constexpr int kRFT = 512;
 constexpr int kRFWaves = kRFT / 64;
 
@@ -557,50 +555,91 @@
 #else
 #define UPH_ROT_T(k)
 #endif
+template <class T>
+__device__ __forceinline__ T gload(const uint8_t* p) {
+  return *(const __attribute__((address_space(1))) T*)p;
+}
+template <class T>
+__device__ __forceinline__ void gstore(uint8_t* p, T v) {
+  *(__attribute__((address_space(1))) T*)p = v;
+}
+
+struct RotPlane {
+  int32_t W, H;
+  uint32_t pitch;
+};
+
+__global__ void __launch_bounds__(256) k_rot_tiles(PlaneRef src, PlaneRef dst, const RotateArgs* args,
+                                                   int count, int tgx, int tgy, int rows_small,
+                                                   int rows_large, int cls_rows, RotSheet* sheets,
+                                                   RotTile* tiles, uint32_t* nlarge) {
+  const int s = blockIdx.y;
+  if (blockIdx.x == 0 && s == 0) {
+    __shared__ uint32_t n_s;
+    if (threadIdx.x == 0) n_s = 0;
+    __syncthreads();
+    uint32_t c = 0;
+    if (cls_rows)
+      for (int q = threadIdx.x; q < count; q += blockDim.x)
+        c += args[q].active && rot_need_rows(args[q].sinval) > cls_rows;
+    if (c) atomicAdd(&n_s, c);
+    __syncthreads();
+    if (threadIdx.x == 0) *nlarge = n_s;
+  }
+  const RotateArgs a = args[s];
+  const bool first = blockIdx.x == 0 && threadIdx.x == 0;
+  if (!a.active) {
+    if (first) sheets[s].active = 0, sheets[s].large = 0;
+    return;
+  }
+  RotSheet g;
+  rot_sheet_geom(a.mask.x0, a.mask.y0, a.mask.x1, a.mask.y1, a.sinval, a.cosval, &g);
+  g.src = plane_ptr(src, s);
+  g.dst = plane_ptr(dst, s);
+  g.active = 1;
+  g.large = cls_rows && rot_need_rows(a.sinval) > cls_rows;
+  if (first) sheets[s] = g;
+  const int ti = blockIdx.x * blockDim.x + threadIdx.x;
+  if (ti >= tgx * tgy) return;
+  const int tyi = ti / tgx;
+  tiles[(int64_t)s * (tgx * tgy) + ti] =
+      rot_tile(&g, src.P.W, src.P.H, ti - tyi * tgx, tyi, g.large ? rows_large : rows_small);
+}
+
 template <bool LOOP>
-__global__ void __launch_bounds__(kRFT, UPH_ROT_MINB) k_rotate_cubic_g8f(PlaneRef src, PlaneRef dst,
-                                                               const RotateArgs* args,
-                                                               int max_rows, int cls_rows,
-                                                               int diag,
-                                                               uint32_t m_gxy, uint32_t m_gx,
-                                                               int loop_count, int tgx, int tgy,
-                                                               uint32_t* colsum, int64_t cs_stride) {
+__global__ void __launch_bounds__(kRFT, UPH_ROT_MINB) k_rotate_cubic_g8f(
+    const RotSheet* __restrict__ sheets, const RotTile* __restrict__ tiles,
+    const uint32_t* __restrict__ nlarge, RotPlane P, int max_rows, int diag, uint32_t m_gxy,
+    uint32_t m_gx, int loop_count, int tgx, int tgy, uint32_t* colsum, int64_t cs_stride) {
   extern __shared__ __attribute__((aligned(16))) float winf[];
-  __shared__ int32_t win_s[4];
   __shared__ uint32_t csum_s[kRFW];
-  auto tile = [&](int txi, int tyi, int s) {
+  auto tile = [&](int txi, int tyi, int s, int ti) {
 #ifdef UPHIP_DIAG
   unsigned long long tprev = wall_clock64();
 #endif
-  const uint8_t* sbase = plane_ptr(src, s);
-  uint8_t* dbase = plane_ptr(dst, s);
-  const RotateArgs a = args[s];
-  if (!a.active) return;
-  if (cls_rows != 0) {
-    const int need = kRFH + (int)ceilf((kRFW - 1) * fabsf(a.sinval)) + 5;
-    if (cls_rows > 0 ? need > cls_rows : need <= -cls_rows) return;
-  }
-  const Planes& P = src.P;
-  const Rect nm = normalize(a.mask);
-  const int32_t sw = nm.x1 - nm.x0 + 1, sh = nm.y1 - nm.y0 + 1;
-  const float scx = nm.x0 + sw / 2.0f, scy = nm.y0 + sh / 2.0f;
-  const float tcx = 0 + sw / 2.0f, tcy = 0 + sh / 2.0f;
+  const RotTile T = tiles[ti];
+  const RotSheet a = sheets[s];
+  UPH_ROT_T(0)
+  asm volatile("" ::"s"(T.bx0), "s"((uint32_t)T.bw), "s"(T.flags), "s"(a.src), "s"(a.dst),
+               "s"(a.mx0), "s"(a.sw), "s"(a.scx), "s"(a.tcx), "s"(a.sinval), "s"(a.active),
+               "s"(P.W), "s"(P.H), "s"(P.pitch), "s"(colsum), "s"(cs_stride));
+  if (!a.active || (a.large != 0) != LOOP) return;
+  const uint8_t* sbase = a.src;
+  uint8_t* dbase = a.dst;
+  const int32_t sw = a.sw, sh = a.sh;
+  const float scx = a.scx, scy = a.scy, tcx = a.tcx, tcy = a.tcy;
   const int32_t tx0 = txi * kRFW, ty0 = tyi * kRFH;
-  const int32_t u0 = imax(tx0, 0) - a.mask.x0, u1 = imin(tx0 + kRFW, P.W) - 1 - a.mask.x0;
-  const int32_t v0 = imax(ty0, 0) - a.mask.y0, v1 = imin(ty0 + kRFH, P.H) - 1 - a.mask.y0;
-  const int32_t cu0 = imax(u0, 0), cu1 = imin(u1, sw - 1);
-  const int32_t cv0 = imax(v0, 0), cv1 = imin(v1, sh - 1);
   auto csum_flush = [&]() {
     __syncthreads();
     if (threadIdx.x < kRFW && tx0 + (int)threadIdx.x < P.W)
       atomicAdd(colsum + s * cs_stride + tx0 + threadIdx.x, csum_s[threadIdx.x]);
   };
-  const bool outside_tile = !(cu0 <= cu1 && cv0 <= cv1);
+  const bool outside_tile = T.flags & ROT_T_OUTSIDE;
   if (colsum) {
     if (threadIdx.x < kRFW) csum_s[threadIdx.x] = 0;
     if (outside_tile) __syncthreads();
   }
-  if (!(cu0 <= cu1 && cv0 <= cv1)) {
+  if (outside_tile) {
     const int cb = 8 * (threadIdx.x & 15);
     const int32_t x = tx0 + cb;
     uint32_t cs8[8] = {0, 0, 0, 0, 0, 0, 0, 0};
@@ -610,14 +649,15 @@
       const uint8_t* sp = sbase + row_off(y, P.pitch) + x;
       uint8_t* dp = dbase + row_off(y, P.pitch) + x;
       if (x + 8 <= P.W) {
-        const uint64_t q = *reinterpret_cast<const uint64_t*>(sp);
-        *reinterpret_cast<uint64_t*>(dp) = q;
+        const uint64_t q = gload<uint64_t>(sp);
+        gstore<uint64_t>(dp, q);
 #pragma unroll
         for (int j = 0; j < 8; j++) cs8[j] += (uint32_t)(q >> (8 * j)) & 0xFFu;
       } else {
         for (int j = 0; x + j < P.W; j++) {
-          dp[j] = sp[j];
-          cs8[j & 7] += sp[j];
+          const uint8_t q = gload<uint8_t>(sp + j);
+          gstore<uint8_t>(dp + j, q);
+          cs8[j & 7] += q;
         }
       }
     }
@@ -628,34 +668,13 @@
     }
     return;
   }
-  UPH_ROT_T(0)
+  UPH_ROT_T(1)
   const int lane = threadIdx.x & 63;
   const int wu = __builtin_amdgcn_readfirstlane(threadIdx.x >> 6);
-  if (wu == 0) {
-    const int c = lane & 3;
-    const int32_t u = c & 1 ? cu1 : cu0, v = c & 2 ? cv1 : cv0;
-    const float X = scx + (u - tcx) * a.cosval + (v - tcy) * a.sinval;
-    const float Y = scy + (v - tcy) * a.cosval - (u - tcx) * a.sinval;
-    float mnx = fminf(X, dpp_f<0xB1>(X)), mxx = fmaxf(X, dpp_f<0xB1>(X));
-    float mny = fminf(Y, dpp_f<0xB1>(Y)), mxy = fmaxf(Y, dpp_f<0xB1>(Y));
-    mnx = fminf(mnx, dpp_f<0x4E>(mnx));
-    mxx = fmaxf(mxx, dpp_f<0x4E>(mxx));
-    mny = fminf(mny, dpp_f<0x4E>(mny));
-    mxy = fmaxf(mxy, dpp_f<0x4E>(mxy));
-    if (lane < 4) {
-      const float q = lane == 0 ? mnx : lane == 1 ? mny : lane == 2 ? mxx : mxy;
-      win_s[lane] = (int32_t)floorf(q);
-    }
-  }
-  __syncthreads();
-  UPH_ROT_T(1)
-  const int32_t bx0 = __builtin_amdgcn_readfirstlane(win_s[0]) - 1;
-  const int32_t by0 = __builtin_amdgcn_readfirstlane(win_s[1]) - 1;
-  const int32_t bw = __builtin_amdgcn_readfirstlane(win_s[2]) + 3 - bx0 + 1;
-  const int32_t bh = __builtin_amdgcn_readfirstlane(win_s[3]) + 3 - by0 + 1;
-  const int32_t xa = bx0 >= 0 ? (bx0 & ~3) : -((-bx0 + 3) & ~3);
-  const int nd = (bx0 - xa + bw + 3) >> 2;
-  const bool staged = bw > 0 && bh > 0 && 4 * nd <= kRFS && bh <= max_rows;
+  const int32_t bx0 = T.bx0, by0 = T.by0, bw = T.bw, bh = T.bh;
+  const int32_t xa = rot_window_xa(bx0);
+  const int nd = rot_window_nd(bx0, bw);
+  const bool staged = (T.flags & ROT_T_STAGED) && bh <= max_rows;
   uint64_t* nw = reinterpret_cast<uint64_t*>(winf + kRFS * max_rows);
   uint8_t* obuf = reinterpret_cast<uint8_t*>(nw + max_rows) + wu * (kRFH / kRFWaves * kRFW);
   if (staged && !UPH_DIAG_BITS(diag, 1024)) {
@@ -675,7 +694,7 @@
         d[1] = make_float4(ubyte_f<0>(w1), ubyte_f<1>(w1), ubyte_f<2>(w1), ubyte_f<3>(w1));
       }
     };
-    const bool interior = xa >= 0 && xa + 8 * nq <= P.W && by0 >= 0 && by0 + bh <= P.H;
+    const bool interior = T.flags & ROT_T_INTERIOR;
     if (interior) {
       const uint32_t off0 = row_off(by0 + rq, P.pitch) + (uint32_t)(qv ? xd : xa);
       for (int rg = 3 * wu; rg < bh; rg += 3 * 3 * kRFWaves) {
@@ -684,7 +703,8 @@
         for (int g = 0; g < 3; g++) {
           const int rb = rg + 3 * kRFWaves * g;
           const uint32_t o = rb + rq < bh ? off0 + (uint32_t)rb * (uint32_t)P.pitch : off0;
-          v[g] = *reinterpret_cast<const uint2*>(sbase + o);
+          const uint64_t q = gload<uint64_t>(sbase + o);
+          v[g] = make_uint2((uint32_t)q, (uint32_t)(q >> 32));
         }
 #pragma unroll
         for (int g = 0; g < 3; g++) {
@@ -711,8 +731,8 @@
           const int r = rg + 3 * kRFWaves * g + rq;
           const int32_t y = imin(imax(by0 + r, 0), P.H - 1);
           const uint8_t* row = sbase + row_off(y, P.pitch);
-          v[g].x = *reinterpret_cast<const uint32_t*>(row + xc0);
-          v[g].y = *reinterpret_cast<const uint32_t*>(row + xc1);
+          v[g].x = gload<uint32_t>(row + xc0);
+          v[g].y = gload<uint32_t>(row + xc1);
         }
 #pragma unroll
         for (int g = 0; g < 3; g++) {
@@ -731,7 +751,7 @@
   UPH_ROT_T(2)
   const int32_t xA = tx0 + lane, xB = xA + 64;
   const bool hasA = xA < P.W, hasB = xB < P.W;
-  const int32_t uA = xA - a.mask.x0, uB = xB - a.mask.x0;
+  const int32_t uA = xA - a.mx0, uB = xB - a.mx0;
   const float cuA = uA - tcx, cuB = uB - tcx;
   const float axA = scx + cuA * a.cosval, bsA = cuA * a.sinval;
   const float axB = scx + cuB * a.cosval, bsB = cuB * a.sinval;
@@ -739,13 +759,13 @@
   typedef __attribute__((address_space(3))) float lds_f32;
   const uint32_t lds0 = (uint32_t)(uintptr_t)(lds_f32*)winf;
   const Src<F_GRAY8> S{sbase, P.pitch, P.W, P.H};
-  const float cuL = (tx0 - a.mask.x0) - tcx, cuR = (tx0 + kRFW - 1 - a.mask.x0) - tcx;
+  const float cuL = (tx0 - a.mx0) - tcx, cuR = (tx0 + kRFW - 1 - a.mx0) - tcx;
   const float bsL = cuL * a.sinval, bsR = cuR * a.sinval;
   constexpr int kRows = kRFH / kRFWaves;
   const int32_t yw = ty0 + wu * kRows;
   const int cb = 8 * (lane & 15);
   const int32_t xo = tx0 + cb;
-  const bool partial = !(cu0 == u0 && cu1 == u1 && cv0 == v0 && cv1 == v1);
+  const bool partial = T.flags & ROT_T_PARTIAL;
   if (partial) {
     constexpr int kQ = (kRows + 3) / 4;
     uint64_t q[kQ];
@@ -755,7 +775,7 @@
       const int rr = 4 * h + (lane >> 4);
       const int32_t y = imin(yw + rr, P.H - 1);
       const int32_t x = imin(xo, (int32_t)P.pitch - 8);
-      if (rr < kRows) q[h] = *reinterpret_cast<const uint64_t*>(sbase + row_off(y, P.pitch) + x);
+      if (rr < kRows) q[h] = gload<uint64_t>(sbase + row_off(y, P.pitch) + x);
     }
 #pragma unroll
     for (int h = 0; h < kQ; h++) {
@@ -770,7 +790,7 @@
       const int k = g + (lane >> 3), j = lane & 7;
       bool hit = false;
       if (k < kRows) {
-        const float cv = (yw + k - a.mask.y0) - tcy;
+        const float cv = (yw + k - a.my0) - tcy;
         const float VC = scy + cv * a.cosval;
         const int32_t yl = (int)(VC - bsL), yr = (int)(VC - bsR);
         const int32_t r0 = imax(imin(yl, yr) - 1 - by0, 0);
@@ -785,7 +805,7 @@
     if (UPH_DIAG_BITS(diag, 2048)) white_rows = 0;
     if (UPH_DIAG_BITS(diag, 512)) white_rows = ~0u;
   }
-  const bool posc = bx0 >= 0 && by0 >= 0;
+  const bool posc = T.flags & ROT_T_POSC;
   const uint32_t wbase = lds0 - 4u * (uint32_t)((1 + by0) * kRFS + 1 + xa);
   UPH_ROT_T(3)
   uint32_t fsA = 0, fsB = 0;
@@ -794,7 +814,7 @@
 #pragma unroll
   for (int k = 0; k < kRows; k++) {
     const int32_t y = yw + k;
-    const int32_t v = y - a.mask.y0;
+    const int32_t v = y - a.my0;
     const bool rowin = FULL || ((v >= 0) & (v < sh) & (y < P.H));
     const float cv = v - tcy;
     const float VS = cv * a.sinval, VC = scy + cv * a.cosval;
@@ -865,8 +885,7 @@
     }
   }
   };
-  const bool full =
-      !partial && staged && posc && tx0 + kRFW <= P.W && ty0 + kRFH <= P.H;
+  const bool full = (T.flags & ROT_T_FULL) && staged;
   if (full)
     row_loop(std::true_type{});
   else
@@ -875,7 +894,7 @@
 #pragma unroll 1
     for (int k = 0; k < kRows; k++) {
       const int32_t y = yw + k;
-      const int32_t v = y - a.mask.y0;
+      const int32_t v = y - a.my0;
       const bool rowin = (v >= 0) & (v < sh) & (y < P.H);
       const float cv = v - tcy;
       const float VS = cv * a.sinval, VC = scy + cv * a.cosval;
@@ -891,7 +910,7 @@
       const int rr = k0 + (lane >> 4);
       if (rr < kRows) {
         const uint64_t q = *reinterpret_cast<const uint64_t*>(obuf + rr * kRFW + cb);
-        *reinterpret_cast<uint64_t*>(dbase + row_off(yw + rr, P.pitch) + xo) = q;
+        gstore<uint64_t>(dbase + row_off(yw + rr, P.pitch) + xo, q);
       }
     }
   } else
@@ -902,9 +921,9 @@
       const uint64_t q = *reinterpret_cast<const uint64_t*>(obuf + rr * kRFW + cb);
       uint8_t* d = dbase + row_off(y, P.pitch) + x;
       if (x + 8 <= P.W) {
-        *reinterpret_cast<uint64_t*>(d) = q;
+        gstore<uint64_t>(d, q);
       } else {
-        for (int j = 0; x + j < P.W; j++) d[j] = (uint8_t)(q >> (8 * j));
+        for (int j = 0; x + j < P.W; j++) gstore<uint8_t>(d + j, (uint8_t)(q >> (8 * j)));
       }
     }
   }
@@ -930,17 +949,15 @@
 #endif
   };
   if constexpr (!LOOP) {
-    int txi, tyi, s;
-    xcd_block_m(m_gxy, m_gx, &txi, &tyi, &s);
-    tile(txi, tyi, s);
+    int txi, tyi, s, ti;
+    xcd_block_m(m_gxy, m_gx, &txi, &tyi, &s, &ti);
+    tile(txi, tyi, s, ti);
   } else {
+  if (*nlarge == 0) return;
   for (int s0 = 0; s0 < loop_count; s0 += 64) {
     const int l = threadIdx.x & 63;
     bool want = false;
-    if (s0 + l < loop_count) {
-      const RotateArgs q = args[s0 + l];
-      want = q.active && kRFH + (int)ceilf((kRFW - 1) * fabsf(q.sinval)) + 5 > -cls_rows;
-    }
+    if (s0 + l < loop_count) want = sheets[s0 + l].active && sheets[s0 + l].large;
     uint64_t m = __ballot(want);
     m = ((uint64_t)__builtin_amdgcn_readfirstlane((uint32_t)(m >> 32)) << 32) |
         __builtin_amdgcn_readfirstlane((uint32_t)m);
@@ -948,7 +965,7 @@
       const int s = s0 + __ffsll((long long)m) - 1;
       m &= m - 1;
       for (int t = blockIdx.x; t < tgx * tgy; t += gridDim.x) {
-        tile(t % tgx, t / tgx, s);
+        tile(t % tgx, t / tgx, s, s * (tgx * tgy) + t);
         __syncthreads();
       }
     }
@@ -961,9 +978,17 @@
   return kRFH + (int)ceilf((kRFW - 1) * sinf(a)) + 5;
 }
 
+static size_t rot_tiles_per_sheet(int32_t W, int32_t H) {
+  return (size_t)((W + kRFW - 1) / kRFW) * (size_t)((H + kRFH - 1) / kRFH);
+}
+size_t rotate_scratch_bytes(int32_t W, int32_t H, int count) {
+  return 64 + (sizeof(RotSheet) + sizeof(RotTile) * rot_tiles_per_sheet(W, H)) * (size_t)count;
+}
+static_assert(sizeof(RotSheet) == 64 && sizeof(RotTile) == 16, "records are read as whole dwords");
+
 bool launch_rotate_mask(const PlaneRef& src, const PlaneRef& dst, const RotateArgs* args,
                         int interp, int count, hipStream_t st, float max_abs_angle,
-                        uint32_t* colsum, int64_t cs_stride) {
+                        void* scratch, uint32_t* colsum, int64_t cs_stride) {
   const dim3 grid((src.P.W + kRotTW - 1) / kRotTW, (src.P.H + kRotTH - 1) / kRotTH, count);
   const dim3 ggrid((src.P.W + kRotTW - 1) / kRotTW, (src.P.H + kRotGH - 1) / kRotGH, count);
   if (interp == UPHIP_INTERP_CUBIC && src.P.fmt == F_GRAY8) {
@@ -991,22 +1016,31 @@
           hipMemcpyToSymbol(HIP_SYMBOL(g_rot_phase), z, sizeof(z));
           for (int i = 0; i < 1024 * 8; i++) h[i & 7] += hh[i];
           if (!h[7]) return;
-          fprintf(stderr, "rotate phases (10 ns ticks/tile, %llu tiles): args %.0f corners %.0f staging %.0f "
+          fprintf(stderr, "rotate phases (10 ns ticks/tile, %llu tiles): index %.0f records %.0f staging %.0f "
                   "flags %.0f compute %.0f stores %.0f colsum %.0f\n", h[7], (double)h[0] / h[7],
                   (double)h[1] / h[7], (double)h[2] / h[7], (double)h[3] / h[7],
                   (double)h[4] / h[7], (double)h[5] / h[7], (double)h[6] / h[7]);
         }
       } phase_print{st};
 #endif
-      if (rows > rows4) {
-        UPH_LAUNCH_DIAG(2, k_rotate_cubic_g8f<false>, fgrid, dim3(kRFT), lds_of(rows4), st, src, dst, args,
-                        rows4, rows4, dd, mgxy, mgx, 0, 0, 0, colsum, cs_stride);
-        UPH_LAUNCH_DIAG(2, k_rotate_cubic_g8f<true>, dim3(3 * 256), dim3(kRFT), lds_of(rows), st, src, dst,
-                        args, rows, -rows4, dd, 0u, 0u, count, (int)fgrid.x, (int)fgrid.y, colsum,
+      uint32_t* nlarge = static_cast<uint32_t*>(scratch);
+      RotSheet* sheets = reinterpret_cast<RotSheet*>(static_cast<uint8_t*>(scratch) + 64);
+      RotTile* tiles = reinterpret_cast<RotTile*>(sheets + count);
+      const RotPlane rp{src.P.W, src.P.H, (uint32_t)src.P.pitch};
+      const int tgx = (int)fgrid.x, tgy = (int)fgrid.y;
+      const bool split = rows > rows4;
+      hipLaunchKernelGGL(k_rot_tiles, dim3((tgx * tgy + 255) / 256, count), dim3(256), 0, st, src,
+                         dst, args, count, tgx, tgy, split ? rows4 : rows, rows, split ? rows4 : 0,
+                         sheets, tiles, nlarge);
+      if (split) {
+        UPH_LAUNCH_DIAG(2, k_rotate_cubic_g8f<false>, fgrid, dim3(kRFT), lds_of(rows4), st, sheets,
+                        tiles, nlarge, rp, rows4, dd, mgxy, mgx, 0, 0, 0, colsum, cs_stride);
+        UPH_LAUNCH_DIAG(2, k_rotate_cubic_g8f<true>, dim3(3 * 256), dim3(kRFT), lds_of(rows), st,
+                        sheets, tiles, nlarge, rp, rows, dd, 0u, 0u, count, tgx, tgy, colsum,
                         cs_stride);
       } else {
-        UPH_LAUNCH_DIAG(2, k_rotate_cubic_g8f<false>, fgrid, dim3(kRFT), lds_of(rows), st, src, dst, args,
-                        rows, 0, dd, mgxy, mgx, 0, 0, 0, colsum, cs_stride);
+        UPH_LAUNCH_DIAG(2, k_rotate_cubic_g8f<false>, fgrid, dim3(kRFT), lds_of(rows), st, sheets,
+                        tiles, nlarge, rp, rows, dd, mgxy, mgx, 0, 0, 0, colsum, cs_stride);
       }
       return colsum != nullptr;
     }
diff --git a/unpaper-gpu_amd/csrc/ops.hip b/unpaper-gpu_amd/csrc/ops.hip
--- a/unpaper-gpu_amd/csrc/ops.hip
+++ b/unpaper-gpu_amd/csrc/ops.hip
@@ -498,10 +498,11 @@
   UphipFrame* n = frame_alloc(f->width, f->height, f->format);
   if (!n) return;
   RotateArgs* d = stage_args(&a, 1, st);
-  if (!d) return;
+  void* rs = scratch(0, rotate_scratch_bytes(f->width, f->height, 1));
+  if (!d || !rs) return;
   if (!(interp == UPHIP_INTERP_LINEAR &&
         launch_rotate_linear(ref_of(f), ref_of(n), d, 1, 1, nullptr, 1, st, radians)))
-    launch_rotate_mask(ref_of(f), ref_of(n), d, interp, 1, st, radians);
+    launch_rotate_mask(ref_of(f), ref_of(n), d, interp, 1, st, radians, rs);
   arg_fence(st);
   adopt_storage(f, n);
   mp.finish();
diff --git a/unpaper-gpu_amd/csrc/pipeline.hip b/unpaper-gpu_amd/csrc/pipeline.hip
--- a/unpaper-gpu_amd/csrc/pipeline.hip
+++ b/unpaper-gpu_amd/csrc/pipeline.hip
@@ -380,6 +380,7 @@
   Rect* pick_mask = nullptr;
   int32_t* pick_active = nullptr;
   RotateArgs* rot_args = nullptr;
+  uint8_t* rot_scratch = nullptr;
   int32_t* rot_indep = nullptr;
   int32_t* rot_dep = nullptr;
   uint32_t* nbits = nullptr;
@@ -694,6 +695,8 @@
   b->border_need = dalloc<int32_t>(b, cap);
   b->border_mask_args = dalloc<MaskArgs>(b, cap);
   b->rot_args = dalloc<RotateArgs>(b, (size_t)cap * UPHIP_MAX_PAGES);
+  b->rot_scratch = dalloc<uint8_t>(b, rotate_scratch_bytes(b->max_w, b->max_h, cap));
+  if (!b->rot_scratch) return false;
   b->rot_indep = dalloc<int32_t>(b, cap);
   b->rot_dep = dalloc<int32_t>(b, cap);
   b->pick_mask = dalloc<Rect>(b, cap);
@@ -1250,8 +1253,8 @@
                                          b->cap, indep, count, b->st, b->max_angle))
         return false;
       return launch_rotate_mask(cur_ref(P, b->ctl), other_ref(P, b->ctl), args,
-                                o.interpolate_type, count, b->st, b->max_angle, colsum,
-                                b->sums_stride);
+                                o.interpolate_type, count, b->st, b->max_angle, b->rot_scratch,
+                                colsum, b->sums_stride);
     };
     if (linear && b->points.size() == 2) {
       detect(0, nullptr);
diff --git a/unpaper-gpu_amd/csrc/rot_tiles.h b/unpaper-gpu_amd/csrc/rot_tiles.h
--- /dev/null
+++ b/unpaper-gpu_amd/csrc/rot_tiles.h
@@ -0,0 +1,112 @@
+#ifndef UNPAPER_HIP_ROT_TILES_H
+#define UNPAPER_HIP_ROT_TILES_H
+
+#include <math.h>
+#include <stdint.h>
+
+#ifdef __HIPCC__
+#define ROT_FN __host__ __device__ static inline
+#else
+#define ROT_FN static inline
+#endif
+
+enum {
+  kRFW = 128,
+  kRFH = 48,
+  kRFS = 144
+};
+
+enum {
+  ROT_T_OUTSIDE = 1,
+  ROT_T_PARTIAL = 2,
+  ROT_T_STAGED = 4,
+  ROT_T_INTERIOR = 8,
+  ROT_T_POSC = 16,
+  ROT_T_FULL = 32
+};
+
+typedef struct RotSheet {
+  const uint8_t* src;
+  uint8_t* dst;
+  int32_t mx0, my0;
+  int32_t sw, sh;
+  float scx, scy, tcx, tcy;
+  float sinval, cosval;
+  int32_t active;
+  int32_t large;
+} RotSheet;
+
+typedef struct RotTile {
+  int32_t bx0, by0;
+  uint16_t bw, bh;
+  uint32_t flags;
+} RotTile;
+
+ROT_FN int32_t rot_imin(int32_t a, int32_t b) { return a < b ? a : b; }
+ROT_FN int32_t rot_imax(int32_t a, int32_t b) { return a > b ? a : b; }
+
+ROT_FN int rot_need_rows(float sinval) { return kRFH + (int)ceilf((kRFW - 1) * fabsf(sinval)) + 5; }
+
+ROT_FN void rot_sheet_geom(int32_t x0, int32_t y0, int32_t x1, int32_t y1, float sinval,
+                           float cosval, RotSheet* g) {
+  const int32_t nx0 = rot_imin(x0, x1), ny0 = rot_imin(y0, y1);
+  const int32_t nx1 = rot_imax(x0, x1), ny1 = rot_imax(y0, y1);
+  const int32_t sw = nx1 - nx0 + 1, sh = ny1 - ny0 + 1;
+  g->mx0 = x0;
+  g->my0 = y0;
+  g->sw = sw;
+  g->sh = sh;
+  g->scx = nx0 + sw / 2.0f;
+  g->scy = ny0 + sh / 2.0f;
+  g->tcx = 0 + sw / 2.0f;
+  g->tcy = 0 + sh / 2.0f;
+  g->sinval = sinval;
+  g->cosval = cosval;
+}
+
+ROT_FN int32_t rot_window_xa(int32_t bx0) { return bx0 >= 0 ? (bx0 & ~3) : -((-bx0 + 3) & ~3); }
+ROT_FN int rot_window_nd(int32_t bx0, int32_t bw) { return (bx0 - rot_window_xa(bx0) + bw + 3) >> 2; }
+
+ROT_FN RotTile rot_tile(const RotSheet* g, int32_t W, int32_t H, int txi, int tyi, int max_rows) {
+  RotTile t;
+  const int32_t tx0 = txi * kRFW, ty0 = tyi * kRFH;
+  const int32_t u0 = rot_imax(tx0, 0) - g->mx0, u1 = rot_imin(tx0 + kRFW, W) - 1 - g->mx0;
+  const int32_t v0 = rot_imax(ty0, 0) - g->my0, v1 = rot_imin(ty0 + kRFH, H) - 1 - g->my0;
+  const int32_t cu0 = rot_imax(u0, 0), cu1 = rot_imin(u1, g->sw - 1);
+  const int32_t cv0 = rot_imax(v0, 0), cv1 = rot_imin(v1, g->sh - 1);
+  if (!(cu0 <= cu1 && cv0 <= cv1)) {
+    t.bx0 = t.by0 = 0;
+    t.bw = t.bh = 0;
+    t.flags = ROT_T_OUTSIDE;
+    return t;
+  }
+  float mnx = 0, mny = 0, mxx = 0, mxy = 0;
+  for (int c = 0; c < 4; c++) {
+    const int32_t u = c & 1 ? cu1 : cu0, v = c & 2 ? cv1 : cv0;
+    const float X = g->scx + (u - g->tcx) * g->cosval + (v - g->tcy) * g->sinval;
+    const float Y = g->scy + (v - g->tcy) * g->cosval - (u - g->tcx) * g->sinval;
+    mnx = c ? fminf(mnx, X) : X;
+    mxx = c ? fmaxf(mxx, X) : X;
+    mny = c ? fminf(mny, Y) : Y;
+    mxy = c ? fmaxf(mxy, Y) : Y;
+  }
+  const int32_t bx0 = (int32_t)floorf(mnx) - 1, by0 = (int32_t)floorf(mny) - 1;
+  const int32_t bw = (int32_t)floorf(mxx) + 3 - bx0 + 1, bh = (int32_t)floorf(mxy) + 3 - by0 + 1;
+  const int32_t xa = rot_window_xa(bx0);
+  const int nd = rot_window_nd(bx0, bw);
+  const int nq = (nd + 1) >> 1;
+  const int staged = bw > 0 && bh > 0 && 4 * nd <= kRFS && bh <= max_rows;
+  const int interior = xa >= 0 && xa + 8 * nq <= W && by0 >= 0 && by0 + bh <= H;
+  const int partial = !(cu0 == u0 && cu1 == u1 && cv0 == v0 && cv1 == v1);
+  const int posc = bx0 >= 0 && by0 >= 0;
+  const int full = !partial && staged && posc && tx0 + kRFW <= W && ty0 + kRFH <= H;
+  t.bx0 = bx0;
+  t.by0 = by0;
+  t.bw = (uint16_t)rot_imin(rot_imax(bw, 0), 0xFFFF);
+  t.bh = (uint16_t)rot_imin(rot_imax(bh, 0), 0xFFFF);
+  t.flags = (partial ? ROT_T_PARTIAL : 0) | (staged ? ROT_T_STAGED : 0) |
+            (interior ? ROT_T_INTERIOR : 0) | (posc ? ROT_T_POSC : 0) | (full ? ROT_T_FULL : 0);
+  return t;
+}
+
+#endif
```

New measurement: 29480 pages/s, median of 6. 3.8% higher.
